# mulns/AccFlow

Hardware: AMD Instinct MI355X
Metric: frame-pairs/s (estimator pair-evals/s), AccFlow(RAFT) 7-frame 480x1024 backward accumulation (higher is better)
Workload: dtype f32 (direct-kernel operands split into 2 fp16 terms - activations kept pre-split in HBM as fp16 hi+lo, 4 B per element; other kernels 3 bf16 terms; f32 accumulate); 1 GPU; AccFlow(RAFT) 7-frame 480x1024, 12 GRU iters, 1 sequence(s)/GPU/step (BASELINE.json configs[2]; configs[3] when n_gpus=8); parallelism=1 rank, no process group: no collective runs, weights=deterministic random init (no checkpoints offline)

## Files before the change

accflow_amd/_lib.py:

```python
import ctypes
import os
import threading

_HERE = os.path.dirname(os.path.abspath(__file__))
LIB_PATH = os.environ.get("ACCFLOW_HIP_LIB") or os.path.join(_HERE, "lib", "libaccflow_hip.so")

ABI_VERSION = 20
c_f = ctypes.c_void_p
c_ll = ctypes.c_longlong
c_i = ctypes.c_int


class ConvSrc(ctypes.Structure):
    _fields_ = [
        ("ptr", c_f), ("bs", c_ll),
        ("C", c_i), ("Hs", c_i), ("Ws", c_i),
        ("step", c_i), ("oy", c_i), ("ox", c_i),
        ("KH", c_i), ("KW", c_i), ("padH", c_i), ("padW", c_i),
        ("reserved", c_i),
    ]


MAX_SRC = 4


class ConvDesc(ctypes.Structure):
    _fields_ = [
        ("in0", c_f), ("in1", c_f),
        ("in0_bs", c_ll), ("in1_bs", c_ll),
        ("C0", c_i), ("C1", c_i),
        ("B", c_i), ("H", c_i), ("W", c_i),
        ("OH", c_i), ("OW", c_i),
        ("KH", c_i), ("KW", c_i), ("stride", c_i), ("padH", c_i), ("padW", c_i),
        ("Cout", c_i),
        ("wpack", c_f), ("ktab", c_f),
        ("Kpad", c_i), ("CoutPad", c_i),
        ("bias", c_f),
        ("out", c_f), ("out_bs", c_ll),
        ("act", c_i), ("epi", c_i),
        ("e0", c_f), ("e0_bs", c_ll),
        ("e1", c_f), ("e1_bs", c_ll),
        ("out2", c_f), ("out2_bs", c_ll),
        ("offset", c_f), ("offset_bs", c_ll),
        ("dmask", c_f), ("dmask_bs", c_ll),
        ("wsplit", c_f), ("mode", c_i),
        ("wpatch", c_f),
        ("wsplit_bs", c_ll),
        ("kws", c_f), ("kws_elems", c_ll),
        ("wpatch16", c_f), ("guard", c_f),
        ("wscale16", c_f), ("wsplit16", c_f), 
        ("stats", c_f), ("stat_slots", c_i), ("pre", c_f), ("pre_bs", c_ll), ("in_norm", c_f), ("acc_scale", ctypes.c_float),
        ("in_fmt", c_i), ("out16", c_f), ("out16_bs", c_ll),
        ("cb", c_i), ("out_cbs", c_ll), ("e0_cbs", c_ll), ("out16_cbs", c_ll),
        ("nsrc", c_i), ("src", ConvSrc * MAX_SRC),
        ("e0_fmt", c_i),
        ("tg_w16", c_f), ("tg_scale", c_f), ("tg_out", c_f), ("tg_out_bs", c_ll), ("tg_out_ps", c_ll),
        ("tg_rows", c_i), ("tg_coutpad", c_i),
        ("split_c0", c_i), ("p32", c_i),
    ]


SIGNATURES = {
    "accflow_abi_version": [],
    "accflow_conv_desc_bytes": [],
    "accflow_conv_src_bytes": [],
    "accflow_s16_item_words": [c_i, c_i, c_i],
    "accflow_to_s16_f32": [c_f, c_ll, c_f, c_ll, c_f, c_i, c_i, c_i, c_f],
    "accflow_conv_kpad": [c_i, c_i, c_i],
    "accflow_conv_coutpad": [c_i],
    "accflow_conv_pack_f32": [c_f, c_f, c_i, c_i, c_i, c_i, c_i, c_i, c_f, c_f, c_f],
    "accflow_conv_pack_bf16s": [c_f, c_f, c_i, c_i, c_i, c_i, c_f, c_f],
    "accflow_conv_patch_elems": [c_i, c_i, c_i, c_i],
    "accflow_conv_pack_patch": [c_f, c_f, c_i, c_i, c_i, c_i, c_f, c_f],
    "accflow_conv_pack_patch16": [c_f, c_f, c_i, c_i, c_i, c_i, c_f, c_f, c_f],
    "accflow_conv_pack_split16": [c_f, c_f, c_i, c_i, c_i, c_i, c_f, c_f, c_f],
    "accflow_conv_multi_pack_elems": [c_i, c_i, ctypes.POINTER(c_i), ctypes.POINTER(c_i), ctypes.POINTER(c_i)],
    "accflow_conv_pack_multi16": [ctypes.POINTER(c_f), c_f, c_i, c_i, ctypes.POINTER(c_i), ctypes.POINTER(c_i), ctypes.POINTER(c_i),
                                  c_f, c_f, c_f],
    "accflow_conv2d_f32": [ctypes.POINTER(ConvDesc), c_f],
    "accflow_conv_stat_slots": [ctypes.POINTER(ConvDesc)],
    "accflow_conv_in_norm_supported": [ctypes.POINTER(ConvDesc)],
    "accflow_conv_plan_query": [ctypes.POINTER(ConvDesc), ctypes.POINTER(c_i), c_i],
    "accflow_conv_gru16_supported": [],
    "accflow_instance_stats_finalize_f32": [c_f, c_i, c_f, c_i, c_i, ctypes.c_float, c_f],
    "accflow_instance_norm_apply_f32": [c_f, c_f, c_i, c_f, c_f, c_f, c_i, c_i, c_i, ctypes.c_float, c_i, c_f],
    "accflow_instance_norm_apply_s16_f32": [c_f, c_f, c_i, c_f, c_f, c_f, c_f, c_ll, c_f, c_i, c_i, c_i, ctypes.c_float, c_i, c_f],
    "accflow_instance_norm_apply_s16res_f32": [c_f, c_f, c_i, c_f, c_f, c_ll, c_f, c_f, c_ll, c_f, c_i, c_i, c_i, ctypes.c_float, c_f],
    "accflow_instance_stats_finalize_sub_f32": [c_f, c_i, c_i, c_i, c_f, c_i, c_i, ctypes.c_float, c_f],
    "accflow_instance_norm_apply_s16proj_f32": [c_f, c_f, c_i, c_f, c_ll, c_f, c_i, c_i, c_i, c_f, c_f, c_ll, c_f, c_i, c_i, c_i,
                                                ctypes.c_float, c_f],
    "accflow_get_occ_s16": [c_f, c_ll, c_f, c_ll, c_f, c_ll, c_f, c_ll, c_f, c_i, c_i, c_i, c_i, c_i, c_f],
    "accflow_blend_s16": [c_f, c_f, c_f, c_f, c_ll, c_f, c_i, c_i, c_i, c_f],
    "accflow_deform_columns_s16": [c_f, c_ll, c_f, c_ll, c_f, c_ll, c_i, c_f, c_ll, c_f, c_i, c_i, c_i, c_i, c_i, c_i, c_i, c_i, c_f],
    "accflow_corr_volume_f32": [c_f, c_f, c_f, c_f, c_f, c_f, c_i, c_i, c_i, c_i, c_f],
    "accflow_corr_volume_ws_bytes": [c_i, c_i, c_i],
    "accflow_corr_volume_split_f32": [c_f, c_f, c_f, c_f, c_f, c_f, c_f, c_i, c_i, c_i, c_i, c_i, c_f],
    "accflow_corr_lookup_f32": [c_f, c_f, c_f, c_f, c_f, c_f, c_ll, c_i, c_i, c_i, c_f],
    "accflow_corr_disp_supported": [c_i, c_i],
    "accflow_corr_disp_level_elems": [c_i, c_i, c_i],
    "accflow_corr_volume_disp_f32": [c_f, c_f, c_f, c_f, c_f, c_f, c_f, c_i, c_f, c_i, c_i, c_i, c_i, c_f],
    "accflow_corr_pack_bytes": [c_i, c_i, c_i],
    "accflow_corr_pack_f32": [c_f, c_f, c_i, c_f, c_i, c_i, c_i, c_i, c_f],
    "accflow_corr_volume_disp_packed_f32": [c_f, c_i, ctypes.POINTER(c_i), ctypes.POINTER(c_i), c_f, c_f, c_f, c_f, c_i, c_f, c_i, c_i, c_i,
                                            c_i, c_f],
    "accflow_corr_disp_pool_f32": [c_f, c_f, c_f, c_f, c_i, c_i, c_i, c_f],
    "accflow_corr_lookup_disp_f32": [c_f, c_f, c_f, c_f, c_f, c_f, c_ll, c_i, c_i, c_i, c_f],
    "accflow_corr_lookup_disp_s16": [c_f, c_f, c_f, c_f, c_f, c_f, c_ll, c_f, c_i, c_i, c_i, c_f],
    "accflow_corr_alt_pyramid_elems": [c_i, c_i, c_i],
    "accflow_corr_alt_pyramid_f32": [c_f, c_f, c_i, c_i, c_i, c_i, c_f],
    "accflow_corr_lookup_alt_f32": [c_f, c_i, c_f, c_f, c_f, c_ll, c_i, c_i, c_i, c_i, c_f],
    "accflow_corr_lookup_alt_s16": [c_f, c_i, c_f, c_f, c_f, c_ll, c_f, c_i, c_i, c_i, c_i, c_f],
    "accflow_corr_lookup_convc1_kpad": [],
    "accflow_corr_lookup_convc1_s16": [c_f, c_f, c_f, c_f, c_f, c_f, c_f, c_f, c_f, c_ll, c_f, c_ll, c_i, c_f, c_i, c_i, c_i, c_i, c_f],
    "accflow_flow_from_coords_s16": [c_f, c_f, c_ll, c_f, c_ll, c_f, c_ll, c_f, c_ll, c_i, c_f, c_i, c_i, c_i, c_i, c_f],
    "accflow_convex_upsample_f32": [c_f, c_ll, c_f, c_ll, c_f, c_i, c_i, c_i, c_f],
    "accflow_backwarp_f32": [c_f, c_ll, c_f, c_ll, c_f, c_ll, c_i, c_i, c_i, c_i, c_f],
    "accflow_compose_flow_f32": [c_f, c_ll, c_f, c_ll, c_f, c_ll, c_i, c_i, c_i, c_f],
    "accflow_get_occ_f32": [c_f, c_ll, c_f, c_ll, c_f, c_ll, c_f, c_ll, c_i, c_i, c_i, c_i, c_i, c_f],
    "accflow_downflow8_f32": [c_f, c_f, c_i, c_i, c_i, c_i, c_f],
    "accflow_forward_interpolate_f32": [c_f, c_f, c_i, c_i, c_i, c_f],
    "accflow_instance_norm_f32": [c_f, c_f, c_f, c_i, c_i, c_i, ctypes.c_float, c_i, c_f],
    "accflow_split_tanh_relu_f32": [c_f, c_f, c_ll, c_f, c_ll, c_i, c_i, c_i, c_i, c_f],
    "accflow_split_tanh_relu_idx_f32": [c_f, c_i, ctypes.POINTER(c_i), c_f, c_ll, c_f, c_ll, c_i, c_i, c_i, c_i, c_f],
    "accflow_coords_grid_f32": [c_f, c_f, c_i, c_i, c_i, c_f],
    "accflow_flow_from_coords_f32": [c_f, c_f, c_ll, c_f, c_ll, c_f, c_i, c_i, c_i, c_i, c_f],
    "accflow_deform_columns_f32": [c_f, c_ll, c_f, c_ll, c_f, c_ll, c_f, c_i, c_i, c_i, c_i, c_i, c_i, c_i, c_i, c_f],
    "accflow_conv_pack_all_f32": [c_f, c_f, c_i, c_i, c_i, c_i, c_i, c_i, c_i, c_f, c_f, c_f, c_f, c_f, c_f, c_f, c_f],
    "accflow_tap_sum_f32": [c_f, c_f, c_f, c_ll, c_f, c_ll, c_i, c_i, c_i, c_i, c_i, c_i, c_i, c_i, c_i, c_i, c_f],
    "accflow_tap_sum_parts_f32": [c_f, c_i, c_ll, c_ll, c_f, c_f, c_ll, c_f, c_ll, c_i, c_i, c_i, c_i, c_i, c_i, c_i, c_i, c_i, c_i, c_f],
    "accflow_blend_f32": [c_f, c_f, c_f, c_f, c_i, c_i, c_i, c_f],
    "accflow_activation_f32": [c_f, c_ll, c_i, c_i, c_i, c_i, c_f],
    "accflow_copy_f32": [c_f, c_ll, c_f, c_ll, c_i, c_i, c_i, c_f],
    "accflow_gma_attention_f32": [c_f, c_f, c_i, c_i, c_i, ctypes.c_float, c_f],
    "accflow_gma_attention_ws_bytes": [c_i, c_i, c_i],
    "accflow_gma_attention_t_f32": [c_f, c_f, c_f, c_i, c_i, c_i, c_i, c_i, ctypes.c_float, c_f],
    "accflow_gma_aggregate_ws_bytes": [c_i, c_i, c_i],
    "accflow_gma_attention_s16_ws_bytes": [c_i, c_i, c_i],
    "accflow_gma_attention_s16": [c_f, c_f, c_f, c_f, c_i, c_i, c_i, c_i, ctypes.c_float, c_f],
    "accflow_gma_aggregate_s16_ws_bytes": [c_i, c_i, c_i],
    "accflow_gma_aggregate_s16": [c_f, c_f, c_f, c_ll, c_f, c_f, c_ll, c_f, c_ll, c_f, c_f, c_i, c_i, c_i, c_i, c_f],
    "accflow_gma_attention_alt_ws_bytes": [c_i, c_i, c_i],
    "accflow_gma_attention_alt": [c_f, c_f, c_f, c_f, c_f, c_f, c_i, c_i, c_i, c_i, ctypes.c_float, c_f],
    "accflow_gma_aggregate_alt_ws_bytes": [c_i, c_i, c_i],
    "accflow_gma_aggregate_alt": [c_f, c_f, c_f, c_f, c_f, c_ll, c_f, c_f, c_ll, c_f, c_ll, c_f, c_f, c_i, c_i, c_i, c_i, c_f],
    "accflow_gma_aggregate_t_f32": [c_f, c_f, c_f, c_f, c_f, c_ll, c_f, c_i, c_f, c_i, c_i, c_i, c_i, c_f],
    "accflow_gma_aggregate_f32": [c_f, c_f, c_f, c_f, c_f, c_ll, c_i, c_i, c_i, c_f],
    "accflow_act_backward_f32": [c_f, c_ll, c_f, c_ll, c_f, c_ll, c_i, c_ll, c_i, c_f],
    "accflow_add_f32": [c_f, c_ll, c_f, c_ll, c_i, c_ll, c_f],
    "accflow_l1_grad_f32": [c_f, c_f, c_f, c_ll, ctypes.c_float, c_f],
    "accflow_dilate_f32": [c_f, c_ll, c_f, c_i, c_i, c_i, c_i, c_i, c_i, c_i, c_f],
    "accflow_blend_backward_f32": [c_f, c_f, c_f, c_f, c_f, c_f, c_f, c_i, c_i, c_i, c_f],
    "accflow_convex_upsample_backward_f32": [c_f, c_f, c_f, c_f, c_f, c_i, c_i, c_i, c_f],
    "accflow_conv_wgrad_f32": [c_f, c_ll, c_f, c_ll, c_f, c_f, c_i, c_i, c_i, c_i, c_i, c_i, c_i, c_i, c_i, c_i, c_f],
    "accflow_deform_conv_backward_f32": [c_f, c_ll, c_f, c_ll, c_f, c_ll, c_f, c_f, c_ll, c_f, c_f, c_i, c_i, c_i, c_i, c_i, c_i, c_i,
                                         c_i, c_f],
}

_lock = threading.Lock()
_lib = None


def _promote_hip_runtime():
    import torch
    cand = os.path.join(os.path.dirname(torch.__file__), "lib", "libamdhip64.so")
    if os.path.exists(cand):
        ctypes.CDLL(cand, mode=ctypes.RTLD_GLOBAL)
    else:
        ctypes.CDLL("libamdhip64.so", mode=ctypes.RTLD_GLOBAL)


def load():
    global _lib
    if _lib is not None:
        return _lib
    with _lock:
        if _lib is not None:
            return _lib
        if not os.path.exists(LIB_PATH):
            raise RuntimeError(
                "accflow_amd: %s not found - run `python -m accflow_amd.build` (hipcc, gfx950). "
                "There is no non-HIP fallback." % LIB_PATH)
        _promote_hip_runtime()
        lib = ctypes.CDLL(LIB_PATH)
        for name, argtypes in SIGNATURES.items():
            fn = getattr(lib, name)
            fn.argtypes = argtypes
            fn.restype = ctypes.c_longlong if name in ("accflow_conv_patch_elems", "accflow_conv_multi_pack_elems", "accflow_corr_pack_bytes", "accflow_corr_volume_ws_bytes",
                                                    "accflow_gma_aggregate_ws_bytes", "accflow_gma_attention_ws_bytes", "accflow_gma_aggregate_s16_ws_bytes", "accflow_gma_attention_s16_ws_bytes", "accflow_gma_attention_alt_ws_bytes", "accflow_gma_aggregate_alt_ws_bytes", "accflow_corr_disp_level_elems", "accflow_corr_alt_pyramid_elems",
                                                    "accflow_s16_item_words") else ctypes.c_int
        if lib.accflow_abi_version() != ABI_VERSION:
            raise RuntimeError("accflow_amd: ABI version mismatch")
        if (lib.accflow_conv_desc_bytes() != ctypes.sizeof(ConvDesc) or lib.accflow_conv_src_bytes() != ctypes.sizeof(ConvSrc)):
            raise RuntimeError("accflow_amd: accflow_conv_desc is %d / %d bytes in the library, %d / %d in _lib.py's mirror" % (
                lib.accflow_conv_desc_bytes(), lib.accflow_conv_src_bytes(), ctypes.sizeof(ConvDesc), ctypes.sizeof(ConvSrc)))
        _lib = lib
    return _lib
```

accflow_amd/csrc/misc.hip:

```cpp
#include "common.h"

namespace {

__device__ __forceinline__ double block_sum(double v, double* red) {
#pragma unroll
  for (int o = 32; o > 0; o >>= 1) v += __shfl_xor(v, o, 64);
  const int lane = threadIdx.x & 63, wave = threadIdx.x >> 6, nw = blockDim.x >> 6;
  __syncthreads();
  if (lane == 0) red[wave] = v;
  __syncthreads();
  double t = 0.0;
  for (int i = 0; i < nw; ++i) t += red[i];
  return t;
}

__global__ __launch_bounds__(512) void instance_norm_kernel(const float* x, const float* res,
                                                            float* out, int HW, float eps, int mode) {
  __shared__ double red[8];
  const long long base = (long long)blockIdx.x * HW;
  const float* p = x + base;
  const bool vec = (HW & 3) == 0;
  double s = 0.0;
  if (vec) {
    const float4* p4 = reinterpret_cast<const float4*>(p);
// ... 112 lines not shown
      for (int k = 0; k < 4; ++k) o[k] = fmaxf(o[k], 0.0f);
    if (mode == 2) {
      const float4 r = *reinterpret_cast<const float4*>(res + i4);
      o[0] = fmaxf(r.x + o[0], 0.0f); o[1] = fmaxf(r.y + o[1], 0.0f); o[2] = fmaxf(r.z + o[2], 0.0f); o[3] = fmaxf(r.w + o[3], 0.0f);
    }
    *reinterpret_cast<float4*>(out + i4) = make_float4(o[0], o[1], o[2], o[3]);
  } else {
    for (long long i = i4; i < i4 + 4 && i < total; ++i) {
      const long long plane = i / HW;
      float v = (x[i] - meanrstd[2 * plane]) * meanrstd[2 * plane + 1];
      if (mode >= 1) v = fmaxf(v, 0.0f);
      if (mode == 2) v = fmaxf(res[i] + v, 0.0f);
      out[i] = v;
    }
  }
}

__global__ void split_tanh_relu_kernel(const float* __restrict__ cnet, float* __restrict__ net, long long net_bs,
                                       float* __restrict__ inp, long long inp_bs, int B, int hd, int cd, int HW) {
  const long long per = (long long)(hd + cd) * HW;
  const long long g = (long long)blockIdx.x * blockDim.x + threadIdx.x;
  if (g >= B * per) return;
  const int b = (int)(g / per);
  const long long r = g - b * per;
  const int c = (int)(r / HW), pix = (int)(r - (long long)c * HW);
  const float v = cnet[g];
  if (c < hd) net[b * net_bs + (long long)c * HW + pix] = tanhf(v);
  else inp[b * inp_bs + (long long)(c - hd) * HW + pix] = fmaxf(v, 0.0f);
}

struct split_idx { int v[64]; };
__global__ void split_tanh_relu_idx_kernel(const float* __restrict__ cnet, split_idx idx, float* __restrict__ net,
                                           long long net_bs, float* __restrict__ inp, long long inp_bs, int B, int hd, int cd,
                                           int HW) {
  const long long per = (long long)(hd + cd) * HW;
  const long long g = (long long)blockIdx.x * blockDim.x + threadIdx.x;
  if (g >= B * per) return;
  const int b = (int)(g / per);
  const long long r = g - b * per;
  const int c = (int)(r / HW), pix = (int)(r - (long long)c * HW);
  const float v = cnet[(long long)idx.v[b] * per + r];
  if (c < hd) net[b * net_bs + (long long)c * HW + pix] = tanhf(v);
  else inp[b * inp_bs + (long long)(c - hd) * HW + pix] = fmaxf(v, 0.0f);
}

__global__ void coords_grid_kernel(float* __restrict__ coords, const float* __restrict__ flow_init, int B, int H8,
                                   int W8) {
  const int P = H8 * W8;
  const long long g = (long long)blockIdx.x * blockDim.x + threadIdx.x;
  if (g >= (long long)B * 2 * P) return;
  const int pix = (int)(g % P), ch = (int)((g / P) & 1);
  const int y = pix / W8, x = pix - y * W8;
  float v = ch == 0 ? (float)x : (float)y;
  if (flow_init) v += flow_init[g];
  coords[g] = v;
}

__global__ void flow_from_coords_kernel(const float* __restrict__ coords1, float* __restrict__ dst0,
                                        long long dst0_bs, float* __restrict__ dst1, long long dst1_bs,
                                        float* __restrict__ stack, int B, int H8, int W8, int is_flow) {
  const int P = H8 * W8;
  const long long g = (long long)blockIdx.x * blockDim.x + threadIdx.x;
  if (g >= (long long)B * 2 * P) return;
  const int b = (int)(g / (2 * P));
  const int r = (int)(g - (long long)b * 2 * P);
  const int ch = r / P, pix = r - ch * P;
  const int y = pix / W8, x = pix - y * W8;
  const float v = is_flow ? coords1[g] : coords1[g] - (ch == 0 ? (float)x : (float)y);
  if (dst0) dst0[b * dst0_bs + r] = v;
  if (dst1) dst1[b * dst1_bs + r] = v;
  if (stack) {
    float* s = stack + (long long)b * 16 * P + pix;
#pragma unroll
    for (int ky = 0; ky < 7; ++ky) {
      const int ys = y + ky - 3;
      const bool ok = (unsigned)ys < (unsigned)H8;
      const float c = ok ? coords1[g + (long long)(ky - 3) * W8] : 0.0f;
      const float u = (ok && !is_flow) ? c - (ch == 0 ? (float)x : (float)ys) : c;
      s[(long long)(ch * 7 + ky) * P] = u;
    }
    s[(long long)(14 + ch) * P] = 0.0f;
  }
}

__global__ __launch_bounds__(256) void flow_from_coords_s16_kernel(const float* __restrict__ coords1, float* __restrict__ dst0,
                                                                   long long dst0_bs, float* __restrict__ dst1, long long dst1_bs,
                                                                   mu32x4* __restrict__ stack, long long stack_bs,
                                                                   unsigned* __restrict__ motion, long long motion_bs, int motion_ch,
                                                                   int* guard, int B, int H8, int W8, int is_flow) {
  const int P = H8 * W8;
  const long long g = (long long)blockIdx.x * 256 + threadIdx.x;
  if (g >= (long long)B * P) return;
  const int b = (int)(g / P), pix = (int)(g - (long long)b * P);
  const int y = pix / W8, x = pix - y * W8;
  const float* c = coords1 + (long long)b * 2 * P + pix;
  float st[16];
#pragma unroll
  for (int ch = 0; ch < 2; ++ch)
#pragma unroll
    for (int ky = 0; ky < 7; ++ky) {
      const int ys = y + ky - 3;
      const bool ok = (unsigned)ys < (unsigned)H8;
      const float cv = ok ? c[(long long)ch * P + (long long)(ky - 3) * W8] : 0.0f;
      st[ch * 7 + ky] = (ok && !is_flow) ? cv - (ch == 0 ? (float)x : (float)ys) : cv;
    }
  st[14] = 0.0f; st[15] = 0.0f;
  const float fx = st[3], fy = st[10];
  if (dst0) { dst0[b * dst0_bs + pix] = fx; dst0[b * dst0_bs + P + pix] = fy; }
  if (dst1) { dst1[b * dst1_bs + pix] = fx; dst1[b * dst1_bs + P + pix] = fy; }
  bool bad = false;
  if (stack) {
    mu32x4* sb = stack + (b * stack_bs) / 4;
#pragma unroll
    for (int o = 0; o < 2; ++o) {
      float v[8];
#pragma unroll
      for (int j = 0; j < 8; ++j) v[j] = st[o * 8 + j];
      mu32x4 hi, lo;
      s16_split8(v, hi, lo, bad);
      sb[((long long)(o * 2 + 0)) * P + pix] = hi;
      sb[((long long)(o * 2 + 1)) * P + pix] = lo;
    }
  }
  if (motion) {
    float v[8] = {fx, fy, 0.0f, 0.0f, 0.0f, 0.0f, 0.0f, 0.0f};
    mu32x4 hi, lo;
    s16_split8(v, hi, lo, bad);
    const int oct = motion_ch >> 3, word = (motion_ch & 7) >> 1;
    unsigned* mb = motion + b * motion_bs;
    mb[(((long long)(oct * 2 + 0)) * P + pix) * 4 + word] = hi[0];
    mb[(((long long)(oct * 2 + 1)) * P + pix) * 4 + word] = lo[0];
  }
  if (bad && guard) atomicOr(guard, 1);
}

__global__ __launch_bounds__(256) void to_s16_kernel(const float* __restrict__ src, long long src_bs, mu32x4* __restrict__ dst,
                                                     long long dst_bs, int* guard, int B, int C, int HW) {
  const int O = (C + 7) >> 3;
  const long long g = (long long)blockIdx.x * 256 + threadIdx.x;
  if (g >= (long long)B * O * HW) return;
  const int pix = (int)(g % HW), o = (int)((g / HW) % O), b = (int)(g / ((long long)HW * O));
  float v[8];
#pragma unroll
  for (int j = 0; j < 8; ++j) v[j] = (o * 8 + j < C) ? src[b * src_bs + (long long)(o * 8 + j) * HW + pix] : 0.0f;
  mu32x4 hi, lo;
  bool bad = false;
  s16_split8(v, hi, lo, bad);
  mu32x4* d = dst + (b * dst_bs) / 4;
  d[(long long)(o * 2 + 0) * HW + pix] = hi;
  d[(long long)(o * 2 + 1) * HW + pix] = lo;
  if (bad && guard) atomicOr(guard, 1);
}

__global__ __launch_bounds__(256) void instance_norm_apply_s16_kernel(const float* __restrict__ x, const float* __restrict__ meanrstd,
                                                                      const float* __restrict__ res, float* __restrict__ out,
                                                                      mu32x4* __restrict__ dst, long long dst_bs, int* guard,
                                                                      int B, int C, int HW, int mode) {
  const int O = (C + 7) >> 3;
  const long long g = (long long)blockIdx.x * 256 + threadIdx.x;
  if (g >= (long long)B * O * HW) return;
  const int pix = (int)(g % HW), o = (int)((g / HW) % O), b = (int)(g / ((long long)HW * O));
  float v[8];
#pragma unroll
  for (int j = 0; j < 8; ++j) {
    const int c = o * 8 + j;
    v[j] = 0.0f;
    if (c < C) {
      const long long plane = (long long)b * C + c, e = plane * HW + pix;
      float t = (x[e] - meanrstd[2 * plane]) * meanrstd[2 * plane + 1];
      if (mode >= 1) t = fmaxf(t, 0.0f);
      if (mode == 2) t = fmaxf(res[e] + t, 0.0f);
      if (out) out[e] = t;
      v[j] = t;
    }
  }
  mu32x4 hi, lo;
  bool bad = false;
  s16_split8(v, hi, lo, bad);
  mu32x4* d = dst + (b * dst_bs) / 4;
  d[(long long)(o * 2 + 0) * HW + pix] = hi;
  d[(long long)(o * 2 + 1) * HW + pix] = lo;
  if (bad && guard) atomicOr(guard, 1);
}

__global__ __launch_bounds__(256) void instance_norm_apply_s16res_kernel(const float* __restrict__ x, const float* __restrict__ meanrstd,
                                                                         const mu32x4* __restrict__ res, long long res_bs,
                                                                         float* __restrict__ out, mu32x4* __restrict__ dst,
                                                                         long long dst_bs, int* guard, int B, int C, int HW) {
  const int O = (C + 7) >> 3;
  const long long g = (long long)blockIdx.x * 256 + threadIdx.x;
  if (g >= (long long)B * O * HW) return;
  const int pix = (int)(g % HW), o = (int)((g / HW) % O), b = (int)(g / ((long long)HW * O));
  const mu32x4* rp = res + (b * res_bs) / 4;
  const mu32x4 rh = rp[(long long)(o * 2 + 0) * HW + pix], rl = rp[(long long)(o * 2 + 1) * HW + pix];
  const unsigned hw[4] = {rh.x, rh.y, rh.z, rh.w}, lw[4] = {rl.x, rl.y, rl.z, rl.w};
  float v[8];
#pragma unroll
  for (int j = 0; j < 8; ++j) {
    const int c = o * 8 + j;
    v[j] = 0.0f;
    if (c < C) {
      const long long plane = (long long)b * C + c, e = plane * HW + pix;
      const _Float16 hh = __builtin_bit_cast(_Float16, (unsigned short)((hw[j >> 1] >> (16 * (j & 1))) & 0xFFFFu));
      const _Float16 ll = __builtin_bit_cast(_Float16, (unsigned short)((lw[j >> 1] >> (16 * (j & 1))) & 0xFFFFu));
      const float r = ((float)hh + (float)ll) * (1.0f / (float)(1 << ACCFLOW_F16_ASHIFT));
      float t = fmaxf((x[e] - meanrstd[2 * plane]) * meanrstd[2 * plane + 1], 0.0f);
      t = fmaxf(r + t, 0.0f);
      if (out) out[e] = t;
      v[j] = t;
    }
  }
  mu32x4 hi, lo;
  bool bad = false;
  s16_split8(v, hi, lo, bad);
  mu32x4* d = dst + (b * dst_bs) / 4;
  d[(long long)(o * 2 + 0) * HW + pix] = hi;
  d[(long long)(o * 2 + 1) * HW + pix] = lo;
  if (bad && guard) atomicOr(guard, 1);
}

__global__ __launch_bounds__(256) void instance_norm_apply_s16proj_kernel(const float* __restrict__ x, const float* __restrict__ mr2,
                                                                          const float* __restrict__ res, long long res_bs,
                                                                          const float* __restrict__ mr3, mu32x4* __restrict__ dst,
                                                                          long long dst_bs, int* guard, int B, int C, int HW) {
  const int O = (C + 7) >> 3;
  const long long g = (long long)blockIdx.x * 256 + threadIdx.x;
  if (g >= (long long)B * O * HW) return;
  const int pix = (int)(g % HW), o = (int)((g / HW) % O), b = (int)(g / ((long long)HW * O));
  float v[8];
#pragma unroll
  for (int j = 0; j < 8; ++j) {
    const int c = o * 8 + j;
    v[j] = 0.0f;
    if (c < C) {
      const long long plane = (long long)b * C + c;
      const float t = fmaxf((x[plane * HW + pix] - mr2[2 * plane]) * mr2[2 * plane + 1], 0.0f);
      const float r = (res[b * res_bs + (long long)c * HW + pix] - mr3[2 * plane]) * mr3[2 * plane + 1];
      v[j] = fmaxf(r + t, 0.0f);
    }
  }
  mu32x4 hi, lo;
  bool bad = false;
  s16_split8(v, hi, lo, bad);
  mu32x4* d = dst + (b * dst_bs) / 4;
  d[(long long)(o * 2 + 0) * HW + pix] = hi;
  d[(long long)(o * 2 + 1) * HW + pix] = lo;
  if (bad && guard) atomicOr(guard, 1);
}

__global__ void blend_kernel(const float* __restrict__ f1, const float* __restrict__ f2, const float* __restrict__ m,
                             float* __restrict__ out, int B, int C, int HW) {
  const long long g = (long long)blockIdx.x * blockDim.x + threadIdx.x;
  if (g >= (long long)B * C * HW) return;
  const int b = (int)(g / ((long long)C * HW));
  const int pix = (int)(g % HW);
  const float mm = m[(long long)b * HW + pix];
  out[g] = f1[g] * mm + (1.0f - mm) * f2[g];
}

__global__ __launch_bounds__(256) void blend_s16_kernel(const float* __restrict__ f1, const float* __restrict__ f2,
                                                        const float* __restrict__ m, mu32x4* __restrict__ dst, long long dst_bs,
                                                        int* guard, int B, int C, int HW) {
  const int O = (C + 7) >> 3;
  const long long g = (long long)blockIdx.x * 256 + threadIdx.x;
  if (g >= (long long)B * O * HW) return;
  const int pix = (int)(g % HW), o = (int)((g / HW) % O), b = (int)(g / ((long long)HW * O));
  const float mm = m[(long long)b * HW + pix];
  float v[8];
#pragma unroll
  for (int j = 0; j < 8; ++j) {
    const int c = o * 8 + j;
    const long long e = ((long long)b * C + c) * HW + pix;
    v[j] = c < C ? f1[e] * mm + (1.0f - mm) * f2[e] : 0.0f;
  }
  mu32x4 hi, lo;
  bool bad = false;
  s16_split8(v, hi, lo, bad);
  mu32x4* d = dst + (b * dst_bs) / 4;
  d[(long long)(o * 2 + 0) * HW + pix] = hi;
  d[(long long)(o * 2 + 1) * HW + pix] = lo;
  if (bad && guard) atomicOr(guard, 1);
}

__global__ void copy_kernel(const float* __restrict__ src, long long src_bs, float* __restrict__ dst, long long dst_bs,
                            int B, long long per) {
  const long long g = (long long)blockIdx.x * blockDim.x + threadIdx.x;
  if (g >= B * per) return;
  const int b = (int)(g / per);
  const long long r = g - b * per;
  dst[b * dst_bs + r] = src[b * src_bs + r];
}

__global__ void act_kernel(float* __restrict__ x, long long x_bs, int B, long long per, int act) {
  const long long g = (long long)blockIdx.x * blockDim.x + threadIdx.x;
  if (g >= B * per) return;
  const int b = (int)(g / per);
  const long long r = g - b * per;
  x[b * x_bs + r] = apply_act(x[b * x_bs + r], act);
}

}

extern "C" int accflow_activation_f32(float* x, long long x_bs, int B, int C, int HW, int act, void* stream) {
  if (!x || B <= 0 || C <= 0 || HW <= 0) return 1;
  const long long per = (long long)C * HW;
  hipLaunchKernelGGL(act_kernel, dim3(cdiv(B * per, 256)), dim3(256), 0, as_stream(stream), x, x_bs, B, per, act);
  ACCFLOW_RETURN_LAUNCH_STATUS();
}

extern "C" int accflow_instance_norm_f32(const float* x, const float* res, float* out, int B, int C, int HW, float eps,
                                         int mode, void* stream) {
  if (!x || !out || B <= 0 || C <= 0 || HW <= 0 || mode < 0 || mode > 2 || (mode == 2 && !res)) return 1;
  hipLaunchKernelGGL(instance_norm_kernel, dim3((unsigned)((long long)B * C)), dim3(512), 0, as_stream(stream), x, res,
                     out, HW, eps, mode);
  ACCFLOW_RETURN_LAUNCH_STATUS();
}

extern "C" int accflow_instance_stats_finalize_f32(const float* stats, int slots, float* meanrstd, int B, int C, float eps,
                                                   void* stream) {
  if (!stats || !meanrstd || slots <= 0 || B <= 0 || C <= 0) return 1;
  launch_finalize(stats, slots, C, 0, meanrstd, B, C, eps, as_stream(stream));
  ACCFLOW_RETURN_LAUNCH_STATUS();
}

extern "C" int accflow_instance_stats_finalize_sub_f32(const float* stats, int slots, int Ctot, int c0, float* meanrstd, int B,
                                                       int C, float eps, void* stream) {
  if (!stats || !meanrstd || slots <= 0 || B <= 0 || C <= 0 || c0 < 0 || c0 + C > Ctot) return 1;
  launch_finalize(stats, slots, Ctot, c0, meanrstd, B, C, eps, as_stream(stream));
  ACCFLOW_RETURN_LAUNCH_STATUS();
}

extern "C" int accflow_instance_norm_apply_s16proj_f32(const float* x, const float* stats, int slots, const float* res,
                                                       long long res_bs, const float* res_stats, int res_slots, int res_ctot,
                                                       int res_c0, float* meanrstd, void* out16, long long out16_bs, int* guard,
                                                       int B, int C, int HW, float eps, void* stream) {
  if (!x || !stats || !res || !res_stats || !meanrstd || !out16 || slots <= 0 || res_slots <= 0 || B <= 0 || C <= 0 || HW <= 0 ||
      res_c0 < 0 || res_c0 + C > res_ctot)
    return 1;
  hipStream_t st = as_stream(stream);
  float* mr3 = meanrstd + 2LL * B * C;
  launch_finalize(stats, slots, C, 0, meanrstd, B, C, eps, st, res_stats, res_slots, res_ctot, res_c0, mr3);
  const long long n = (long long)B * ((C + 7) / 8) * HW;
  hipLaunchKernelGGL(instance_norm_apply_s16proj_kernel, dim3(cdiv(n, 256)), dim3(256), 0, st, x, meanrstd, res, res_bs, mr3,
                     reinterpret_cast<mu32x4*>(out16), out16_bs, guard, B, C, HW);
  ACCFLOW_RETURN_LAUNCH_STATUS();
}

extern "C" int accflow_instance_norm_apply_f32(const float* x, const float* stats, int slots, float* meanrstd,
                                               const float* res, float* out, int B, int C, int HW, float eps, int mode,
                                               void* stream) {
  if (!x || !stats || !meanrstd || !out || slots <= 0 || B <= 0 || C <= 0 || HW <= 0 || mode < 0 || mode > 2 ||
      (mode == 2 && !res))
    return 1;
  const long long total = (long long)B * C * HW;
  launch_finalize(stats, slots, C, 0, meanrstd, B, C, eps, as_stream(stream));
  hipLaunchKernelGGL(instance_norm_apply_kernel, dim3(cdiv(cdiv(total, 4), 256)), dim3(256), 0, as_stream(stream), x,
                     meanrstd, res, out, HW, total, mode);
  ACCFLOW_RETURN_LAUNCH_STATUS();
}

extern "C" int accflow_instance_norm_apply_s16_f32(const float* x, const float* stats, int slots, float* meanrstd,
                                                   const float* res, float* out, void* out16, long long out16_bs, int* guard,
                                                   int B, int C, int HW, float eps, int mode, void* stream) {
  if (!x || !stats || !meanrstd || !out16 || slots <= 0 || B <= 0 || C <= 0 || HW <= 0 || mode < 0 || mode > 2 ||
      (mode == 2 && !res))
    return 1;
  launch_finalize(stats, slots, C, 0, meanrstd, B, C, eps, as_stream(stream));
  const long long n = (long long)B * ((C + 7) / 8) * HW;
  hipLaunchKernelGGL(instance_norm_apply_s16_kernel, dim3(cdiv(n, 256)), dim3(256), 0, as_stream(stream), x, meanrstd, res,
                     out, reinterpret_cast<mu32x4*>(out16), out16_bs, guard, B, C, HW, mode);
  ACCFLOW_RETURN_LAUNCH_STATUS();
}

extern "C" int accflow_instance_norm_apply_s16res_f32(const float* x, const float* stats, int slots, float* meanrstd,
                                                      const void* res16, long long res16_bs, float* out, void* out16,
                                                      long long out16_bs, int* guard, int B, int C, int HW, float eps,
                                                      void* stream) {
  if (!x || !stats || !meanrstd || !res16 || !out16 || slots <= 0 || B <= 0 || C <= 0 || HW <= 0) return 1;
  launch_finalize(stats, slots, C, 0, meanrstd, B, C, eps, as_stream(stream));
  const long long n = (long long)B * ((C + 7) / 8) * HW;
  hipLaunchKernelGGL(instance_norm_apply_s16res_kernel, dim3(cdiv(n, 256)), dim3(256), 0, as_stream(stream), x, meanrstd,
                     reinterpret_cast<const mu32x4*>(res16), res16_bs, out, reinterpret_cast<mu32x4*>(out16), out16_bs, guard,
                     B, C, HW);
  ACCFLOW_RETURN_LAUNCH_STATUS();
}

extern "C" int accflow_split_tanh_relu_f32(const float* cnet, float* net, long long net_bs, float* inp,
                                           long long inp_bs, int B, int hd, int cd, int HW, void* stream) {
  if (!cnet || !net || !inp || B <= 0 || hd <= 0 || cd <= 0 || HW <= 0) return 1;
  const long long n = (long long)B * (hd + cd) * HW;
  hipLaunchKernelGGL(split_tanh_relu_kernel, dim3(cdiv(n, 256)), dim3(256), 0, as_stream(stream), cnet, net, net_bs,
                     inp, inp_bs, B, hd, cd, HW);
  ACCFLOW_RETURN_LAUNCH_STATUS();
}

extern "C" int accflow_split_tanh_relu_idx_f32(const float* cnet, int n_items, const int* idx, float* net, long long net_bs,
                                               float* inp, long long inp_bs, int B, int hd, int cd, int HW, void* stream) {
  if (!cnet || !idx || !net || !inp || n_items <= 0 || B <= 0 || hd <= 0 || cd <= 0 || HW <= 0) return 1;
  for (int b = 0; b < B; ++b)
    if (idx[b] < 0 || idx[b] >= n_items) return 1;
  for (int b0 = 0; b0 < B; b0 += 64) {
    const int nb = B - b0 < 64 ? B - b0 : 64;
    split_idx a;
    for (int k = 0; k < 64; ++k) a.v[k] = k < nb ? idx[b0 + k] : 0;
    const long long n = (long long)nb * (hd + cd) * HW;
    hipLaunchKernelGGL(split_tanh_relu_idx_kernel, dim3(cdiv(n, 256)), dim3(256), 0, as_stream(stream), cnet, a,
                       net + b0 * net_bs, net_bs, inp + b0 * inp_bs, inp_bs, nb, hd, cd, HW);
  }
  ACCFLOW_RETURN_LAUNCH_STATUS();
}

extern "C" int accflow_coords_grid_f32(float* coords, const float* flow_init, int B, int H8, int W8, void* stream) {
  if (!coords || B <= 0 || H8 <= 0 || W8 <= 0) return 1;
  const long long n = (long long)B * 2 * H8 * W8;
  hipLaunchKernelGGL(coords_grid_kernel, dim3(cdiv(n, 256)), dim3(256), 0, as_stream(stream), coords, flow_init, B, H8,
                     W8);
  ACCFLOW_RETURN_LAUNCH_STATUS();
}

extern "C" int accflow_flow_from_coords_f32(const float* coords1, float* dst0, long long dst0_bs, float* dst1,
                                            long long dst1_bs, float* stack16, int is_flow, int B, int H8, int W8,
                                            void* stream) {
  if (!coords1 || (!dst0 && !dst1 && !stack16) || B <= 0 || H8 <= 0 || W8 <= 0) return 1;
  const long long n = (long long)B * 2 * H8 * W8;
  hipLaunchKernelGGL(flow_from_coords_kernel, dim3(cdiv(n, 256)), dim3(256), 0, as_stream(stream), coords1, dst0,
                     dst0_bs, dst1, dst1_bs, stack16, B, H8, W8, is_flow);
  ACCFLOW_RETURN_LAUNCH_STATUS();
}

extern "C" int accflow_flow_from_coords_s16(const float* coords1, float* dst0, long long dst0_bs, float* dst1,
                                            long long dst1_bs, void* stack16, long long stack16_bs, void* motion16,
                                            long long motion16_bs, int motion_ch, int* guard, int is_flow, int B, int H8,
                                            int W8, void* stream) {
  if (!coords1 || (!dst0 && !dst1 && !stack16 && !motion16) || B <= 0 || H8 <= 0 || W8 <= 0 || motion_ch < 0 || (motion_ch & 1))
    return 1;
  const long long n = (long long)B * H8 * W8;
  hipLaunchKernelGGL(flow_from_coords_s16_kernel, dim3(cdiv(n, 256)), dim3(256), 0, as_stream(stream), coords1, dst0, dst0_bs,
                     dst1, dst1_bs, reinterpret_cast<mu32x4*>(stack16), stack16_bs, reinterpret_cast<unsigned*>(motion16),
                     motion16_bs, motion_ch, guard, B, H8, W8, is_flow);
  ACCFLOW_RETURN_LAUNCH_STATUS();
}

extern "C" int accflow_to_s16_f32(const float* src, long long src_bs, void* dst16, long long dst16_bs, int* guard, int B,
                                  int C, int HW, void* stream) {
  if (!src || !dst16 || B <= 0 || C <= 0 || HW <= 0) return 1;
  const long long n = (long long)B * ((C + 7) / 8) * HW;
  hipLaunchKernelGGL(to_s16_kernel, dim3(cdiv(n, 256)), dim3(256), 0, as_stream(stream), src, src_bs,
                     reinterpret_cast<mu32x4*>(dst16), dst16_bs, guard, B, C, HW);
  ACCFLOW_RETURN_LAUNCH_STATUS();
}

extern "C" int accflow_blend_f32(const float* f1, const float* f2, const float* m, float* out, int B, int C, int HW,
                                 void* stream) {
  if (!f1 || !f2 || !m || !out || B <= 0 || C <= 0 || HW <= 0) return 1;
  const long long n = (long long)B * C * HW;
  hipLaunchKernelGGL(blend_kernel, dim3(cdiv(n, 256)), dim3(256), 0, as_stream(stream), f1, f2, m, out, B, C, HW);
  ACCFLOW_RETURN_LAUNCH_STATUS();
}

extern "C" int accflow_blend_s16(const float* f1, const float* f2, const float* m, void* out16, long long out16_bs, int* guard,
                                 int B, int C, int HW, void* stream) {
  if (!f1 || !f2 || !m || !out16 || B <= 0 || C <= 0 || HW <= 0) return 1;
  const long long n = (long long)B * ((C + 7) / 8) * HW;
  hipLaunchKernelGGL(blend_s16_kernel, dim3(cdiv(n, 256)), dim3(256), 0, as_stream(stream), f1, f2, m,
                     reinterpret_cast<mu32x4*>(out16), out16_bs, guard, B, C, HW);
  ACCFLOW_RETURN_LAUNCH_STATUS();
}

extern "C" int accflow_copy_f32(const float* src, long long src_bs, float* dst, long long dst_bs, int B, int C, int HW,
                                void* stream) {
  if (!src || !dst || B <= 0 || C <= 0 || HW <= 0) return 1;
  const long long per = (long long)C * HW;
  hipLaunchKernelGGL(copy_kernel, dim3(cdiv(B * per, 256)), dim3(256), 0, as_stream(stream), src, src_bs, dst, dst_bs,
                     B, per);
  ACCFLOW_RETURN_LAUNCH_STATUS();
}

__global__ __launch_bounds__(256) void tap_sum_kernel(const float* __restrict__ z, const float* __restrict__ bias,
                                                      const float* __restrict__ e0, long long e0_bs, float* __restrict__ out,
                                                      long long out_bs, int B, int Cout, int H, int W, int KH, int KW,
                                                      int padH, int padW, int act, int epi, int nparts, long long part_stride,
                                                      long long z_bs) {
  const long long n = (long long)B * Cout * H * W;
  const long long i = (long long)blockIdx.x * 256 + threadIdx.x;
  if (i >= n) return;
  const int x = (int)(i % W), y = (int)((i / W) % H);
  const int co = (int)((i / ((long long)W * H)) % Cout), b = (int)(i / ((long long)W * H * Cout));
  const int HW = H * W;
  const float* zb = z + (long long)b * z_bs;
  float v = 0.0f;
  for (int ky = 0; ky < KH; ++ky) {
    const int yy = y + ky - padH;
    if ((unsigned)yy >= (unsigned)H) continue;
    for (int kx = 0; kx < KW; ++kx) {
      const int xx = x + kx - padW;
      if ((unsigned)xx >= (unsigned)W) continue;
      const float* zp = zb + (long long)((ky * KW + kx) * Cout + co) * HW + yy * W + xx;
      float t = zp[0];
      for (int p = 1; p < nparts; ++p) t += zp[p * part_stride];
      v += t;
    }
  }
  if (bias) v += bias[co];
  v = apply_act(v, act);
  const long long o = (long long)co * HW + y * W + x;
  if (epi == ACCFLOW_EPI_ACCUM) v += e0[b * e0_bs + o];
  else if (epi == ACCFLOW_EPI_RES_RELU) v = fmaxf(e0[b * e0_bs + o] + v, 0.0f);
  out[b * out_bs + o] = v;
}

extern "C" int accflow_tap_sum_f32(const float* z, const float* bias, const float* e0, long long e0_bs, float* out,
                                   long long out_bs, int B, int Cout, int H, int W, int KH, int KW, int padH, int padW,
                                   int act, int epi, void* stream) {
  if (!z || !out || B <= 0 || Cout <= 0 || H <= 0 || W <= 0 || KH <= 0 || KW <= 0) return 1;
  if (epi != ACCFLOW_EPI_STORE && epi != ACCFLOW_EPI_ACCUM && epi != ACCFLOW_EPI_RES_RELU) return 1;
  if (epi != ACCFLOW_EPI_STORE && !e0) return 1;
  const long long n = (long long)B * Cout * H * W;
  hipLaunchKernelGGL(tap_sum_kernel, dim3(cdiv(n, 256)), dim3(256), 0, as_stream(stream), z, bias, e0, e0_bs, out, out_bs, B,
                     Cout, H, W, KH, KW, padH, padW, act, epi, 1, 0LL, (long long)KH * KW * Cout * H * W);
  ACCFLOW_RETURN_LAUNCH_STATUS();
}

extern "C" int accflow_tap_sum_parts_f32(const float* z, int nparts, long long part_stride, long long z_bs, const float* bias,
                                         const float* e0, long long e0_bs, float* out, long long out_bs, int B, int Cout, int H,
                                         int W, int KH, int KW, int padH, int padW, int act, int epi, void* stream) {
  if (!z || !out || B <= 0 || Cout <= 0 || H <= 0 || W <= 0 || KH <= 0 || KW <= 0 || nparts < 1 || nparts > 8) return 1;
  if (z_bs < (long long)KH * KW * Cout * H * W || (nparts > 1 && part_stride <= 0)) return 1;
  if (epi != ACCFLOW_EPI_STORE && epi != ACCFLOW_EPI_ACCUM && epi != ACCFLOW_EPI_RES_RELU) return 1;
  if (epi != ACCFLOW_EPI_STORE && !e0) return 1;
  const long long n = (long long)B * Cout * H * W;
  hipLaunchKernelGGL(tap_sum_kernel, dim3(cdiv(n, 256)), dim3(256), 0, as_stream(stream), z, bias, e0, e0_bs, out, out_bs, B,
                     Cout, H, W, KH, KW, padH, padW, act, epi, nparts, part_stride, z_bs);
  ACCFLOW_RETURN_LAUNCH_STATUS();
}

extern "C" int accflow_abi_version(void) { return ACCFLOW_ABI_VERSION; }
extern "C" int accflow_conv_desc_bytes(void) { return (int)sizeof(accflow_conv_desc); }
extern "C" int accflow_conv_src_bytes(void) { return (int)sizeof(accflow_conv_src); }
```

accflow_amd/csrc/sampling.hip:

```cpp
#include "common.h"

namespace {

__global__ __launch_bounds__(256) void convex_upsample_kernel(const float* __restrict__ flow, long long flow_bs,
                                                              const float* __restrict__ mask, long long mask_bs,
                                                              float* __restrict__ out, int B, int H8, int W8) {
  const int P = H8 * W8;
  const long long gp = (long long)blockIdx.x * blockDim.x + threadIdx.x;
  if (gp >= (long long)B * P) return;
  const int b = (int)(gp / P), pix = (int)(gp - (long long)b * P);
  const int h = pix / W8, w = pix - h * W8;
  const float* fl = flow + b * flow_bs;
  float f0[9], f1[9];
#pragma unroll
  for (int k = 0; k < 9; ++k) {
    const int yy = h + k / 3 - 1, xx = w + k % 3 - 1;
    const bool ok = (unsigned)yy < (unsigned)H8 && (unsigned)xx < (unsigned)W8;
    f0[k] = ok ? 8.0f * fl[yy * W8 + xx] : 0.0f;
    f1[k] = ok ? 8.0f * fl[P + yy * W8 + xx] : 0.0f;
  }
  const float* mk = mask + b * mask_bs + pix;
  const int W = 8 * W8;
  float* o0 = out + ((long long)(b * 2 + 0) * (8 * H8) + 8 * h) * W + 8 * w;
  float* o1 = out + ((long long)(b * 2 + 1) * (8 * H8) + 8 * h) * W + 8 * w;
#pragma unroll 1
  for (int a = 0; a < 8; ++a) {
    float r0[8], r1[8];
#pragma unroll
    for (int bb = 0; bb < 8; ++bb) {
      float m[9];
      float mx = -INFINITY;
#pragma unroll
      for (int k = 0; k < 9; ++k) {
        m[k] = mk[(long long)(k * 64 + a * 8 + bb) * P];
        mx = fmaxf(mx, m[k]);
      }
      float s = 0.0f;
#pragma unroll
      for (int k = 0; k < 9; ++k) {
        m[k] = expf(m[k] - mx);
        s += m[k];
      }
      float u0 = 0.0f, u1 = 0.0f;
#pragma unroll
      for (int k = 0; k < 9; ++k) {
        const float wk = m[k] / s;
        u0 += wk * f0[k];
        u1 += wk * f1[k];
      }
      r0[bb] = u0;
      r1[bb] = u1;
    }
    float4* q0 = reinterpret_cast<float4*>(o0 + (long long)a * W);
    float4* q1 = reinterpret_cast<float4*>(o1 + (long long)a * W);
    q0[0] = make_float4(r0[0], r0[1], r0[2], r0[3]);
    q0[1] = make_float4(r0[4], r0[5], r0[6], r0[7]);
    q1[0] = make_float4(r1[0], r1[1], r1[2], r1[3]);
    q1[1] = make_float4(r1[4], r1[5], r1[6], r1[7]);
  }
}

struct WarpTaps {
  int o00, o01, o10, o11;
  float w00, w01, w10, w11;
};

__device__ __forceinline__ WarpTaps make_taps(float sx, float sy, int H, int W) {
  sx = fminf(fmaxf(sx, -1.0e6f), 1.0e6f);
  sy = fminf(fmaxf(sy, -1.0e6f), 1.0e6f);
  const float fx0 = floorf(sx), fy0 = floorf(sy);
  const int x0 = (int)fx0, y0 = (int)fy0;
  const float ax = sx - fx0, ay = sy - fy0;
  const bool xin0 = (unsigned)x0 < (unsigned)W, xin1 = (unsigned)(x0 + 1) < (unsigned)W;
  const bool yin0 = (unsigned)y0 < (unsigned)H, yin1 = (unsigned)(y0 + 1) < (unsigned)H;
  WarpTaps t;
  t.o00 = (xin0 && yin0) ? y0 * W + x0 : 0;
  t.o01 = (xin1 && yin0) ? y0 * W + x0 + 1 : 0;
  t.o10 = (xin0 && yin1) ? (y0 + 1) * W + x0 : 0;
  t.o11 = (xin1 && yin1) ? (y0 + 1) * W + x0 + 1 : 0;
  t.w00 = (xin0 && yin0) ? (1.0f - ax) * (1.0f - ay) : 0.0f;
  t.w01 = (xin1 && yin0) ? ax * (1.0f - ay) : 0.0f;
  t.w10 = (xin0 && yin1) ? (1.0f - ax) * ay : 0.0f;
  t.w11 = (xin1 && yin1) ? ax * ay : 0.0f;
  return t;
}
__device__ __forceinline__ float tap_sample(const float* __restrict__ plane, const WarpTaps& t) {
  return plane[t.o00] * t.w00 + plane[t.o01] * t.w01 + plane[t.o10] * t.w10 + plane[t.o11] * t.w11;
}

constexpr int WARP_CCHUNK = 16;

template <bool ADD>
__global__ __launch_bounds__(256) void backwarp_kernel(const float* __restrict__ img, long long img_bs,
                                                       const float* __restrict__ flow, long long flow_bs,
                                                       float* __restrict__ out, long long out_bs, int B, int C, int H,
                                                       int W) {
  const int HW = H * W;
  const long long gp = (long long)blockIdx.x * blockDim.x + threadIdx.x;
  if (gp >= (long long)B * HW) return;
  const int b = (int)(gp / HW), pix = (int)(gp - (long long)b * HW);
  const int y = pix / W, x = pix - y * W;
  const float u = flow[b * flow_bs + pix], v0 = flow[b * flow_bs + HW + pix];
  const WarpTaps t = make_taps((float)x + u, (float)y + v0, H, W);
  const int c0 = blockIdx.y * WARP_CCHUNK, c1 = min(C, c0 + WARP_CCHUNK);
  for (int c = c0; c < c1; ++c) {
    float v = tap_sample(img + b * img_bs + (long long)c * HW, t);
    if constexpr (ADD) v += c == 0 ? u : v0;
    out[b * out_bs + (long long)c * HW + pix] = v;
  }
}

template <bool BINARY>
__global__ __launch_bounds__(256) void get_occ_kernel(const float* __restrict__ flow, long long flow_bs,
                                                      const float* __restrict__ i1, long long i1_bs,
                                                      const float* __restrict__ i2, long long i2_bs,
                                                      float* __restrict__ out, long long out_bs, int B, int C, int H,
                                                      int W) {
  const int HW = H * W;
  const long long gp = (long long)blockIdx.x * blockDim.x + threadIdx.x;
  if (gp >= (long long)B * HW) return;
  const int b = (int)(gp / HW), pix = (int)(gp - (long long)b * HW);
  const int y = pix / W, x = pix - y * W;
  const float u = flow[b * flow_bs + pix], v = flow[b * flow_bs + HW + pix];
  const WarpTaps t = make_taps((float)x + u, (float)y + v, H, W);
  if constexpr (BINARY) {
    const int cper = (C + 3) / 4;
    float q[4];
#pragma unroll
    for (int k = 0; k < 4; ++k) {
      float s = 0.0f;
      for (int c = k * cper; c < min(C, (k + 1) * cper); ++c) {
        const float wv = tap_sample(i2 + b * i2_bs + (long long)c * HW, t);
        s += fabsf(i1[b * i1_bs + (long long)c * HW + pix] - wv);
      }
      q[k] = s;
    }
    const float tot = (q[0] + q[1]) + (q[2] + q[3]);
    out[b * out_bs + pix] = (tot / (float)C <= 1.0f) ? 1.0f : 0.0f;
  } else {
    const int c0 = blockIdx.y * WARP_CCHUNK, c1 = min(C, c0 + WARP_CCHUNK);
    for (int c = c0; c < c1; ++c) {
      const float wv = tap_sample(i2 + b * i2_bs + (long long)c * HW, t);
      out[b * out_bs + (long long)c * HW + pix] = fabsf(i1[b * i1_bs + (long long)c * HW + pix] - wv);
    }
  }
}

template <bool BINARY>
__global__ __launch_bounds__(256) void get_occ_s16_kernel(const float* __restrict__ flow, long long flow_bs,
                                                          const float* __restrict__ i1, long long i1_bs,
                                                          const float* __restrict__ i2, long long i2_bs,
                                                          mu32x4* __restrict__ dst, long long dst_bs, int* guard, int B, int C,
                                                          int H, int W) {
  const int HW = H * W;
  const long long gp = (long long)blockIdx.x * blockDim.x + threadIdx.x;
  if (gp >= (long long)B * HW) return;
  const int b = (int)(gp / HW), pix = (int)(gp - (long long)b * HW);
  const int y = pix / W, x = pix - y * W;
  const float u = flow[b * flow_bs + pix], v = flow[b * flow_bs + HW + pix];
  const WarpTaps t = make_taps((float)x + u, (float)y + v, H, W);
  float val[8] = {0.0f, 0.0f, 0.0f, 0.0f, 0.0f, 0.0f, 0.0f, 0.0f};
  const int o = BINARY ? 0 : blockIdx.y;
  if constexpr (BINARY) {
    const int cper = (C + 3) / 4;
    float q[4];
#pragma unroll
    for (int k = 0; k < 4; ++k) {
      float s = 0.0f;
      for (int c = k * cper; c < min(C, (k + 1) * cper); ++c) {
        const float wv = tap_sample(i2 + b * i2_bs + (long long)c * HW, t);
        s += fabsf(i1[b * i1_bs + (long long)c * HW + pix] - wv);
      }
      q[k] = s;
    }
    const float tot = (q[0] + q[1]) + (q[2] + q[3]);
    val[0] = (tot / (float)C <= 1.0f) ? 1.0f : 0.0f;
  } else {
#pragma unroll
    for (int j = 0; j < 8; ++j) {
      const int c = o * 8 + j;
      if (c < C) val[j] = fabsf(i1[b * i1_bs + (long long)c * HW + pix] - tap_sample(i2 + b * i2_bs + (long long)c * HW, t));
    }
  }
  mu32x4 hi, lo;
  bool bad = false;
  s16_split8(val, hi, lo, bad);
  mu32x4* d = dst + (b * dst_bs) / 4;
  d[(long long)(o * 2 + 0) * HW + pix] = hi;
  d[(long long)(o * 2 + 1) * HW + pix] = lo;
  if (bad && guard) atomicOr(guard, 1);
}

__global__ __launch_bounds__(256) void downflow8_kernel(const float* __restrict__ flow, float* __restrict__ out,
                                                        int BC, int H, int W) {
  const int H8 = H / 8, W8 = W / 8, P = H8 * W8;
  const long long g = (long long)blockIdx.x * blockDim.x + threadIdx.x;
  if (g >= (long long)BC * P) return;
  const int bc = (int)(g / P), pix = (int)(g - (long long)bc * P);
  const int y = pix / W8, x = pix - y * W8;
  const float sy_scale = H8 > 1 ? (float)(H - 1) / (float)(H8 - 1) : 0.0f;
  const float sx_scale = W8 > 1 ? (float)(W - 1) / (float)(W8 - 1) : 0.0f;
  const float sy = sy_scale * (float)y, sx = sx_scale * (float)x;
  const int y0 = (int)sy, x0 = (int)sx;
  const int yp = y0 < H - 1 ? 1 : 0, xp = x0 < W - 1 ? 1 : 0;
  const float ly = sy - (float)y0, lx = sx - (float)x0;
  const float hy = 1.0f - ly, hx = 1.0f - lx;
  const float* p = flow + (long long)bc * H * W + (long long)y0 * W + x0;
  const float v = hy * (hx * p[0] + lx * p[xp]) + ly * (hx * p[(long long)yp * W] + lx * p[(long long)yp * W + xp]);
  out[g] = v / 8.0f;
}

}

extern "C" int accflow_convex_upsample_f32(const float* flow, long long flow_bs, const float* mask, long long mask_bs,
                                           float* out, int B, int H8, int W8, void* stream) {
  if (!flow || !mask || !out || B <= 0 || H8 <= 0 || W8 <= 0) return 1;
  const long long np = (long long)B * H8 * W8;
  hipLaunchKernelGGL(convex_upsample_kernel, dim3(cdiv(np, 256)), dim3(256), 0, as_stream(stream), flow, flow_bs,
                     mask, mask_bs, out, B, H8, W8);
  ACCFLOW_RETURN_LAUNCH_STATUS();
}

template <bool S16OUT>
__global__ __launch_bounds__(256) void get_occ_binary4_kernel(const float* __restrict__ flow, long long flow_bs,
                                                              const float* __restrict__ i1, long long i1_bs,
                                                              const float* __restrict__ i2, long long i2_bs,
                                                              float* __restrict__ out, long long out_bs, int B, int C, int H,
                                                              int W) {
  __shared__ float part[4][64];
  const int HW = H * W;
  const int lane = threadIdx.x & 63, wave = threadIdx.x >> 6;
  const long long gp = (long long)blockIdx.x * 64 + lane;
  const bool live = gp < (long long)B * HW;
  const int b = live ? (int)(gp / HW) : 0, pix = live ? (int)(gp - (long long)b * HW) : 0;
  const int y = pix / W, x = pix - y * W;
  const float u = flow[b * flow_bs + pix], v = flow[b * flow_bs + HW + pix];
  const WarpTaps t = make_taps((float)x + u, (float)y + v, H, W);
  const int cper = (C + 3) / 4, cbeg = wave * cper, cend = min(C, cbeg + cper);
  float s = 0.0f;
  for (int c = cbeg; c < cend; ++c) {
    const float wv = tap_sample(i2 + b * i2_bs + (long long)c * HW, t);
    s += fabsf(i1[b * i1_bs + (long long)c * HW + pix] - wv);
  }
  part[wave][lane] = s;
  __syncthreads();
  if (wave == 0 && live) {
    const float tot = (part[0][lane] + part[1][lane]) + (part[2][lane] + part[3][lane]);
    const float bit = (tot / (float)C <= 1.0f) ? 1.0f : 0.0f;
    if constexpr (S16OUT) {
      const float val[8] = {bit, 0.0f, 0.0f, 0.0f, 0.0f, 0.0f, 0.0f, 0.0f};
      mu32x4 hi, lo;
      bool bad = false;
      s16_split8(val, hi, lo, bad);
      mu32x4* d = reinterpret_cast<mu32x4*>(out) + (b * out_bs) / 4;
      d[pix] = hi;
      d[(long long)HW + pix] = lo;
    } else {
      out[b * out_bs + pix] = bit;
    }
  }
}

extern "C" int accflow_backwarp_f32(const float* img, long long img_bs, const float* flow, long long flow_bs,
                                    float* out, long long out_bs, int B, int C, int H, int W, void* stream) {
  if (!img || !flow || !out || B <= 0 || C <= 0 || H <= 0 || W <= 0) return 1;
  const long long np = (long long)B * H * W;
  hipLaunchKernelGGL(backwarp_kernel<false>, dim3(cdiv(np, 256), cdiv(C, WARP_CCHUNK)), dim3(256), 0, as_stream(stream),
                     img, img_bs, flow, flow_bs, out, out_bs, B, C, H, W);
  ACCFLOW_RETURN_LAUNCH_STATUS();
}

extern "C" int accflow_compose_flow_f32(const float* step, long long step_bs, const float* acc, long long acc_bs,
                                        float* out, long long out_bs, int B, int H, int W, void* stream) {
  if (!step || !acc || !out || B <= 0 || H <= 0 || W <= 0) return 1;
  const long long np = (long long)B * H * W;
  hipLaunchKernelGGL(backwarp_kernel<true>, dim3(cdiv(np, 256), 1), dim3(256), 0, as_stream(stream), acc, acc_bs, step,
                     step_bs, out, out_bs, B, 2, H, W);
  ACCFLOW_RETURN_LAUNCH_STATUS();
}

extern "C" int accflow_get_occ_f32(const float* flow, long long flow_bs, const float* i1, long long i1_bs,
                                   const float* i2, long long i2_bs, float* out, long long out_bs, int B, int C, int H,
                                   int W, int binary, void* stream) {
  if (!flow || !i1 || !i2 || !out || B <= 0 || C <= 0 || H <= 0 || W <= 0) return 1;
  const long long np = (long long)B * H * W;
  if (binary && np < (1 << 17))
    hipLaunchKernelGGL((get_occ_binary4_kernel<false>), dim3(cdiv(np, 64)), dim3(256), 0, as_stream(stream), flow, flow_bs, i1,
                       i1_bs, i2, i2_bs, out, out_bs, B, C, H, W);
  else if (binary)
    hipLaunchKernelGGL((get_occ_kernel<true>), dim3(cdiv(np, 256)), dim3(256), 0, as_stream(stream), flow, flow_bs,
                       i1, i1_bs, i2, i2_bs, out, out_bs, B, C, H, W);
  else
    hipLaunchKernelGGL((get_occ_kernel<false>), dim3(cdiv(np, 256), cdiv(C, WARP_CCHUNK)), dim3(256), 0,
                       as_stream(stream), flow, flow_bs, i1, i1_bs, i2, i2_bs, out, out_bs, B, C, H, W);
  ACCFLOW_RETURN_LAUNCH_STATUS();
}

extern "C" int accflow_get_occ_s16(const float* flow, long long flow_bs, const float* i1, long long i1_bs, const float* i2,
                                   long long i2_bs, void* out16, long long out16_bs, int* guard, int B, int C, int H, int W,
                                   int binary, void* stream) {
  if (!flow || !i1 || !i2 || !out16 || B <= 0 || C <= 0 || H <= 0 || W <= 0) return 1;
  const long long np = (long long)B * H * W;
  mu32x4* d = reinterpret_cast<mu32x4*>(out16);
  if (binary && np < (1 << 17))
    hipLaunchKernelGGL((get_occ_binary4_kernel<true>), dim3(cdiv(np, 64)), dim3(256), 0, as_stream(stream), flow, flow_bs, i1,
                       i1_bs, i2, i2_bs, reinterpret_cast<float*>(out16), out16_bs, B, C, H, W);
  else if (binary)
    hipLaunchKernelGGL((get_occ_s16_kernel<true>), dim3(cdiv(np, 256)), dim3(256), 0, as_stream(stream), flow, flow_bs, i1, i1_bs,
                       i2, i2_bs, d, out16_bs, guard, B, C, H, W);
  else
    hipLaunchKernelGGL((get_occ_s16_kernel<false>), dim3(cdiv(np, 256), cdiv(C, 8)), dim3(256), 0, as_stream(stream), flow,
                       flow_bs, i1, i1_bs, i2, i2_bs, d, out16_bs, guard, B, C, H, W);
  ACCFLOW_RETURN_LAUNCH_STATUS();
}

extern "C" int accflow_downflow8_f32(const float* flow, float* out, int B, int C, int H, int W, void* stream) {
  if (!flow || !out || B <= 0 || C <= 0 || H < 8 || W < 8 || (H % 8) || (W % 8)) return 1;
  const long long n = (long long)B * C * (H / 8) * (W / 8);
  hipLaunchKernelGGL(downflow8_kernel, dim3(cdiv(n, 256)), dim3(256), 0, as_stream(stream), flow, out, B * C, H, W);
  ACCFLOW_RETURN_LAUNCH_STATUS();
}

namespace {
__global__ __launch_bounds__(256) void deform_columns_kernel(const float* __restrict__ x, long long x_bs,
                                                             const float* __restrict__ off, long long off_bs,
                                                             const float* __restrict__ msk, long long msk_bs,
                                                             float* __restrict__ cols, int B, int C, int H, int W, int KH,
                                                             int KW, int padH, int padW) {
  const int HW = H * W, T = KH * KW;
  const long long i = (long long)blockIdx.x * 256 + threadIdx.x;
  if (i >= (long long)B * T * HW) return;
  const int p = (int)(i % HW), tap = (int)((i / HW) % T), b = (int)(i / ((long long)HW * T));
  const int y = p / W, xx = p - y * W, ky = tap / KW, kx = tap - ky * KW;
  const float dy = off[b * off_bs + (long long)(2 * tap) * HW + p], dx = off[b * off_bs + (long long)(2 * tap + 1) * HW + p];
  const float m = msk[b * msk_bs + (long long)tap * HW + p];
  const float h = (float)(y - padH + ky) + dy, w = (float)(xx - padW + kx) + dx;
  const bool inside = h > -1.0f && h < (float)H && w > -1.0f && w < (float)W;
  const float fh = floorf(h), fw = floorf(w);
  const int hl = (int)fh, wl = (int)fw, hh = hl + 1, wh = wl + 1;
  const float lh = h - fh, lw = w - fw, uh = 1.0f - lh, uw = 1.0f - lw;
  const bool o1 = inside && hl >= 0 && wl >= 0, o2 = inside && hl >= 0 && wh <= W - 1;
  const bool o3 = inside && hh <= H - 1 && wl >= 0, o4 = inside && hh <= H - 1 && wh <= W - 1;
  const int i1 = o1 ? hl * W + wl : 0, i2 = o2 ? hl * W + wh : 0, i3 = o3 ? hh * W + wl : 0, i4 = o4 ? hh * W + wh : 0;
  const float* src = x + b * x_bs;
  float* dst = cols + ((long long)b * T * C + (long long)tap * C) * HW + p;
  const int cper = (C + gridDim.y - 1) / gridDim.y, cbeg = blockIdx.y * cper, cend = min(C, cbeg + cper);
  for (int c = cbeg; c < cend; ++c) {
    const float* plane = src + (long long)c * HW;
    const float v1 = o1 ? plane[i1] : 0.0f, v2 = o2 ? plane[i2] : 0.0f, v3 = o3 ? plane[i3] : 0.0f, v4 = o4 ? plane[i4] : 0.0f;
    dst[(long long)c * HW] = inside ? m * (uh * uw * v1 + uh * lw * v2 + lh * uw * v3 + lh * lw * v4) : 0.0f;
  }
}

template <bool LOGIT>
__global__ __launch_bounds__(256) void deform_columns_s16_kernel(const float* __restrict__ x, long long x_bs,
                                                                 const float* __restrict__ off, long long off_bs,
                                                                 const float* __restrict__ msk, long long msk_bs,
                                                                 mu32x4* __restrict__ cols, long long cols_bs, int* guard, int B,
                                                                 int C, int H, int W, int KH, int KW, int padH, int padW) {
  const int HW = H * W, T = KH * KW;
  const long long i = (long long)blockIdx.x * 256 + threadIdx.x;
  if (i >= (long long)B * T * HW) return;
  const int p = (int)(i % HW), tap = (int)((i / HW) % T), b = (int)(i / ((long long)HW * T));
  const int y = p / W, xx = p - y * W, ky = tap / KW, kx = tap - ky * KW;
  const float dy = off[b * off_bs + (long long)(2 * tap) * HW + p], dx = off[b * off_bs + (long long)(2 * tap + 1) * HW + p];
  float m = msk[b * msk_bs + (long long)tap * HW + p];
  if constexpr (LOGIT) m = sigmoidf_(m);
  const float h = (float)(y - padH + ky) + dy, w = (float)(xx - padW + kx) + dx;
  const bool inside = h > -1.0f && h < (float)H && w > -1.0f && w < (float)W;
  const float fh = floorf(h), fw = floorf(w);
  const int hl = (int)fh, wl = (int)fw, hh = hl + 1, wh = wl + 1;
  const float lh = h - fh, lw = w - fw, uh = 1.0f - lh, uw = 1.0f - lw;
  const bool o1 = inside && hl >= 0 && wl >= 0, o2 = inside && hl >= 0 && wh <= W - 1;
  const bool o3 = inside && hh <= H - 1 && wl >= 0, o4 = inside && hh <= H - 1 && wh <= W - 1;
  const int i1 = o1 ? hl * W + wl : 0, i2 = o2 ? hl * W + wh : 0, i3 = o3 ? hh * W + wl : 0, i4 = o4 ? hh * W + wh : 0;
  const float* src = x + b * x_bs;
  const int OC = C >> 3;
  const int oper = (OC + gridDim.y - 1) / gridDim.y, obeg = blockIdx.y * oper, oend = min(OC, obeg + oper);
  mu32x4* d = cols + (b * cols_bs) / 4;
  bool bad = false;
  for (int o = obeg; o < oend; ++o) {
    float v[8];
#pragma unroll
    for (int j = 0; j < 8; ++j) {
      const float* plane = src + (long long)(o * 8 + j) * HW;
      const float v1 = o1 ? plane[i1] : 0.0f, v2 = o2 ? plane[i2] : 0.0f, v3 = o3 ? plane[i3] : 0.0f, v4 = o4 ? plane[i4] : 0.0f;
      v[j] = inside ? m * (uh * uw * v1 + uh * lw * v2 + lh * uw * v3 + lh * lw * v4) : 0.0f;
    }
    mu32x4 hi, lo;
    s16_split8(v, hi, lo, bad);
    const long long oct = (long long)tap * OC + o;
    d[(oct * 2 + 0) * HW + p] = hi;
    d[(oct * 2 + 1) * HW + p] = lo;
  }
  if (bad && guard) atomicOr(guard, 1);
}
}

extern "C" int accflow_deform_columns_s16(const float* x, long long x_bs, const float* offset, long long offset_bs,
                                          const float* dmask, long long dmask_bs, int mask_is_logit, void* cols16,
                                          long long cols16_bs, int* guard, int B, int C, int H, int W, int KH, int KW, int padH,
                                          int padW, void* stream) {
  if (!x || !offset || !dmask || !cols16 || B <= 0 || C <= 0 || (C & 7) || H <= 0 || W <= 0 || KH <= 0 || KW <= 0) return 1;
  const long long n = (long long)B * KH * KW * H * W;
  const int chunks = n < (1 << 18) ? (C >= 64 ? 8 : 1) : (n < (1 << 20) ? 2 : 1);
  mu32x4* d = reinterpret_cast<mu32x4*>(cols16);
  if (mask_is_logit)
    hipLaunchKernelGGL((deform_columns_s16_kernel<true>), dim3(cdiv(n, 256), chunks), dim3(256), 0, as_stream(stream), x, x_bs,
                       offset, offset_bs, dmask, dmask_bs, d, cols16_bs, guard, B, C, H, W, KH, KW, padH, padW);
  else
    hipLaunchKernelGGL((deform_columns_s16_kernel<false>), dim3(cdiv(n, 256), chunks), dim3(256), 0, as_stream(stream), x, x_bs,
                       offset, offset_bs, dmask, dmask_bs, d, cols16_bs, guard, B, C, H, W, KH, KW, padH, padW);
  ACCFLOW_RETURN_LAUNCH_STATUS();
}

extern "C" int accflow_deform_columns_f32(const float* x, long long x_bs, const float* offset, long long offset_bs,
                                          const float* dmask, long long dmask_bs, float* cols, int B, int C, int H, int W,
                                          int KH, int KW, int padH, int padW, void* stream) {
  if (!x || !offset || !dmask || !cols || B <= 0 || C <= 0 || H <= 0 || W <= 0 || KH <= 0 || KW <= 0) return 1;
  const long long n = (long long)B * KH * KW * H * W;
  const int chunks = n < (1 << 18) ? (C >= 64 ? 8 : 1) : (n < (1 << 20) ? 2 : 1);
  hipLaunchKernelGGL(deform_columns_kernel, dim3(cdiv(n, 256), chunks), dim3(256), 0, as_stream(stream), x, x_bs, offset, offset_bs,
                     dmask, dmask_bs, cols, B, C, H, W, KH, KW, padH, padW);
  ACCFLOW_RETURN_LAUNCH_STATUS();
}
```

accflow_amd/networks/AccFlow_.py:

```python
import math

import torch
import torch.nn as nn

from .. import ops
from ._packs import PackCache, require_cuda, span
from .modules import ZeroConv2d
from .raft.extractor import BasicEncoder

import contextlib
import threading
import os

USE_S16_CHAIN = os.environ.get("ACCFLOW_S16_CHAIN", "1") == "1"
CONTEXT_SIDE_STREAM = os.environ.get("ACCFLOW_CONTEXT_STREAM", "1") == "1"
USE_CHAIN_HOIST = os.environ.get("ACCFLOW_CHAIN_HOIST", "auto")
_CHAIN_TLS = threading.local()


PIPELINE_CHAIN_KSPLIT = os.environ.get("ACCFLOW_PIPELINE_CHAIN_KSPLIT", "0") == "1"


@contextlib.contextmanager
def chain_in_pipeline():
    prev = (getattr(_CHAIN_TLS, "pipelined", False), getattr(_CHAIN_TLS, "no_ksplit", False))
    _CHAIN_TLS.pipelined, _CHAIN_TLS.no_ksplit = True, not PIPELINE_CHAIN_KSPLIT
    try:
        yield
    finally:
        _CHAIN_TLS.pipelined, _CHAIN_TLS.no_ksplit = prev


@contextlib.contextmanager
def pipeline_chain_arithmetic():
    prev = getattr(_CHAIN_TLS, "no_ksplit", False)
    _CHAIN_TLS.no_ksplit = not PIPELINE_CHAIN_KSPLIT
    try:
        yield
    finally:
        _CHAIN_TLS.no_ksplit = prev


def _hoist_now():
    if USE_CHAIN_HOIST == "auto":
        return not getattr(_CHAIN_TLS, "pipelined", False)
    return USE_CHAIN_HOIST == "1" or USE_CHAIN_HOIST is True
USE_CHAIN_DEFER_UP = os.environ.get("ACCFLOW_CHAIN_DEFER_UP", "1") == "1"
_CTX_STREAMS = {}


def _context_stream(device):
    key = str(device)
    if key not in _CTX_STREAMS:
        _CTX_STREAMS[key] = torch.cuda.Stream(device=device)
    return _CTX_STREAMS[key]


class FlowDecoder(nn.Module):
    def __init__(self, cin=128):
        super().__init__()
        self.flow = nn.Sequential(nn.Conv2d(cin, cin * 2, 3, 1, 1), nn.ReLU(True), nn.Conv2d(cin * 2, 2, 3, 1, 1))
        self.mask = nn.Sequential(nn.Conv2d(cin, cin * 2, 3, 1, 1), nn.ReLU(True), nn.Conv2d(cin * 2, 64 * 9, 1, 1, 0))
        self._packs = PackCache()

    def upsample_flow(self, flow, mask):
        require_cuda(flow, mask)
        return ops.convex_upsample(flow.float(), mask.float())

    @torch.no_grad()
    @ops.range_guarded
    def forward(self, x):
        require_cuda(x)
        pk = self._packs
        if ops.s16_active() and USE_S16_CHAIN:
            return self._forward16(ops.to_s16(x.float()))
        t = ops.conv2d(pk.conv("f0", self.flow[0]), x, act=ops.ACT_RELU)
        flow_small = ops.conv2d(pk.conv("f2", self.flow[2]), t)
        t = ops.conv2d(pk.conv("m0", self.mask[0]), x, act=ops.ACT_RELU, out=t)
        mask = ops.conv2d(pk.conv("m2", self.mask[2]), t)
        return flow_small, ops.convex_upsample(flow_small, mask)


    def _forward16(self, x16):
        pk = self._packs
        B, _, h, w = x16.shape
        c2 = self.flow[0].out_channels
        t16 = ops.S16.empty(B, 2 * c2, h, w, x16.device)
        ops.conv2d_multi(pk.multi_cat("fm0", [self.flow[0], self.mask[0]]), [x16], act=ops.ACT_RELU, out16=t16, fp32_out=False)
        flow_small = ops.conv2d(pk.conv("f2", self.flow[2]), t16.channels(0, c2))
        mask = ops.conv2d_multi(pk.multi("m2m", self.mask[2]), [t16.channels(c2, 2 * c2)])
        return flow_small, ops.convex_upsample(flow_small, mask)

    def flow16(self, x16, out=None):
        pk = self._packs
        B, _, h, w = x16.shape
        t16 = ops.S16.empty(B, self.flow[0].out_channels, h, w, x16.device)
        ops.conv2d_multi(pk.multi("f0m", self.flow[0]), [x16], act=ops.ACT_RELU, out16=t16, fp32_out=False)
        return ops.conv2d(pk.conv("f2", self.flow[2]), t16, out=out)

    def upsample16(self, x16, flow_small):
        pk = self._packs
        B, _, h, w = x16.shape
        t16 = ops.S16.empty(B, self.mask[0].out_channels, h, w, x16.device)
        ops.conv2d_multi(pk.multi("m0m", self.mask[0]), [x16], act=ops.ACT_RELU, out16=t16, fp32_out=False)
        mask = ops.conv2d_multi(pk.multi("m2m", self.mask[2]), [t16])
        return ops.convex_upsample(flow_small, mask)


class FlowEncoder(nn.Module):
    def __init__(self, c=128):
        super().__init__()
        self.conv1 = nn.Conv2d(2, c, 7, stride=1, padding=3)
        self.conv2 = nn.Conv2d(c, c * 2, 3, stride=1, padding=1)
        self.conv3 = nn.Conv2d(c * 2, c, 1, stride=1, padding=0)
        self.relu = nn.ReLU(True)
        self._packs = PackCache()

    @torch.no_grad()
    @ops.range_guarded
    def forward(self, x):
        is_list = isinstance(x, (tuple, list))
        if is_list:
            batch_dim = x[0].shape[0]
            x = torch.cat(x, dim=0)
        require_cuda(x)
        pk = self._packs
        if ops.s16_active() and USE_S16_CHAIN:
            x = self.encode16(x.float().contiguous())[0]
        else:
            x = ops.conv2d(pk.conv("1", self.conv1), x.float().contiguous(), act=ops.ACT_RELU)
            x = ops.conv2d(pk.conv("2", self.conv2), x, act=ops.ACT_RELU)
            x = ops.conv2d(pk.conv("3", self.conv3), x)
        if is_list:
            x = torch.split(x, batch_dim, dim=0)
        return x

    def encode16(self, flows):
        pk = self._packs
        B, _, h, w = flows.shape
        dev = flows.device
        c = self.conv1.out_channels
        stack16 = ops.S16.empty(B, 16, h, w, dev)
        ops.flow_from_coords_s16(flows, None, None, stack16, None, 0, is_flow=True)
        a16 = ops.S16.empty(B, c, h, w, dev)
        ops.conv2d(pk.conv("1s", self.conv1, rows_as_channels=True), stack16, act=ops.ACT_RELU, out16=a16, fp32_out=False)
        b16 = ops.S16.empty(B, 2 * c, h, w, dev)
        ops.conv2d_multi(pk.multi("2m", self.conv2), [a16], act=ops.ACT_RELU, out16=b16, fp32_out=False)
        o16 = ops.S16.empty(B, c, h, w, dev)
        out = ops.conv2d_multi(pk.multi("3m", self.conv3), [b16], out16=o16)
        return out, o16


class DeformConv2d(nn.Module):

    def __init__(self, in_channels, out_channels, kernel_size=3, stride=1, padding=1):
        super().__init__()
        if (kernel_size, stride, padding) != (3, 1, 1):
            raise NotImplementedError("AccPlus uses DeformConv2d(c, c, 3, 1, 1) (AccFlow_.py:83)")
        self.in_channels, self.out_channels = in_channels, out_channels
        self.kernel_size, self.stride, self.padding = (3, 3), (1, 1), (1, 1)
        self.weight = nn.Parameter(torch.empty(out_channels, in_channels, 3, 3))
        self.bias = nn.Parameter(torch.empty(out_channels))
        nn.init.kaiming_uniform_(self.weight, a=math.sqrt(5))
        bound = 1 / math.sqrt(in_channels * 9)
        nn.init.uniform_(self.bias, -bound, bound)


class AccPlus(nn.Module):
    def __init__(self, c=128):
        super().__init__()
        self.conv1 = nn.Sequential(nn.Conv2d(c * 2 + 1, c * 2, 3, 1, 1), nn.ReLU(True), nn.Conv2d(c * 2, c, 3, 1, 1))
        self.conv2 = nn.Sequential(nn.Conv2d(c * 2, c * 2, 3, 1, 1), nn.ReLU(True), nn.Conv2d(c * 2, c, 3, 1, 1),
                                   nn.ReLU(True), ZeroConv2d(c, 3 ** 3))
        self.dconv = DeformConv2d(c, c, 3, 1, 1)
        self.conv3 = nn.Sequential(nn.Conv2d(c * 2 + 1, c * 2, 3, 1, 1), nn.ReLU(True), nn.Conv2d(c * 2, c, 3, 1, 1))
        self.conv4 = nn.Sequential(nn.Conv2d(c * 4, c * 2, 3, 1, 1), nn.ReLU(True), nn.Conv2d(c * 2, c, 3, 1, 1),
                                   nn.ReLU(True), nn.Conv2d(c, c, 1, 1, 0))
        self.c = c
        self._packs = PackCache()

    @torch.no_grad()
    @ops.range_guarded
    def forward(self, df, f, o, c):
        require_cuda(df, f, o, c)
        if ops.s16_active() and USE_S16_CHAIN:
            return self.forward16(ops.to_s16(df.float()), f.float().contiguous(), ops.to_s16(f.float()), ops.to_s16(o.float()),
                                  ops.to_s16(c.float()))
        pk, C = self._packs, self.c
        B, _, h, w = df.shape
        dev = df.device

        def buf(ch):
            return torch.empty((B, ch, h, w), dtype=torch.float32, device=dev)

        A, E, G, X2 = buf(2 * C + 1), buf(2 * C + 1), buf(4 * C), buf(2 * C)
        ops.copy_into(df.float(), A[:, :C]); ops.copy_into(f.float(), A[:, C:2 * C]); ops.copy_into(o.float(), A[:, 2 * C:])
        ops.copy_into(c.float(), X2[:, C:]); ops.copy_into(c.float(), G[:, C:2 * C])
        ops.copy_into(df.float(), G[:, 3 * C:]); ops.copy_into(df.float(), E[:, C:2 * C]); ops.copy_into(o.float(), E[:, 2 * C:])
        t = ops.conv2d(pk.conv("1a", self.conv1[0]), A, act=ops.ACT_RELU)
# ... 6 lines not shown
        f_ = ops.conv2d(pk.conv("dc", self.dconv_as_conv(), tap_major=True), A[:, C:2 * C], out=E[:, :C],
                        offset=off, dmask=msk)
        ops.copy_into(f_, G[:, 2 * C:3 * C])
        t = ops.conv2d(pk.conv("3a", self.conv3[0]), E, act=ops.ACT_RELU, out=t)
        ops.conv2d(pk.conv("3b", self.conv3[2]), t, out=G[:, :C])
        t = ops.conv2d(pk.conv("4a", self.conv4[0]), G, act=ops.ACT_RELU, out=t)
        u = ops.conv2d(pk.conv("4b", self.conv4[2]), t, act=ops.ACT_RELU, out=u)
        return ops.conv2d(pk.conv("4c", self.conv4[4]), u)

    def forward16(self, df16, f, f16, o16, c16):
        pk, C = self._packs, self.c
        B, _, h, w = f.shape
        dev = f.device
        R = ops.ACT_RELU

        def s16(ch):
            return ops.S16.empty(B, ch, h, w, dev)

        t16, x16, u16, f_16, y16 = s16(2 * C), s16(C), s16(C), s16(C), s16(C)
        ops.conv2d_multi(pk.multi("1a", self.conv1[0], splits=[C, C, 1]), [df16, f16, o16], act=R, out16=t16, fp32_out=False)
        ops.conv2d_multi(pk.multi("1b", self.conv1[2]), [t16], out16=x16, fp32_out=False)
        ops.conv2d_multi(pk.multi("2a", self.conv2[0], splits=[C, C]), [x16, c16], act=R, out16=t16, fp32_out=False)
        ops.conv2d_multi(pk.multi("2b", self.conv2[2]), [t16], act=R, out16=u16, fp32_out=False)
        zc = self.conv2[4]
        om = ops.conv2d_multi(pk.multi("2z", zc.conv, scale=zc.out_scale, scale_dep=zc.scale), [u16])
        ops.deform_conv2d_s16(pk.conv("dc", self.dconv_as_conv(), tap_major=True), f, om[:, :18], om[:, 18:], f_16,
                              mask_is_logit=True)
        ops.conv2d_multi(pk.multi("3a", self.conv3[0], splits=[C, C, 1]), [f_16, df16, o16], act=R, out16=t16, fp32_out=False)
        ops.conv2d_multi(pk.multi("3b", self.conv3[2]), [t16], out16=y16, fp32_out=False)
        ops.conv2d_multi(pk.multi("4a", self.conv4[0], splits=[C, C, C, C]), [y16, c16, f_16, df16], act=R, out16=t16,
                         fp32_out=False)
        ops.conv2d_multi(pk.multi("4b", self.conv4[2]), [t16], act=R, out16=u16, fp32_out=False)
        return ops.conv2d_multi(pk.multi("4c", self.conv4[4]), [u16])

    def dconv_as_conv(self):
        return _ConvView(self.dconv)


class _ConvView:

    def __init__(self, d):
        self.weight, self.bias, self.stride, self.padding = d.weight, d.bias, d.stride, d.padding


class Blending(nn.Module):
    def __init__(self, c=128):
        super().__init__()
        self.mask = nn.Sequential(nn.Conv2d(c, c * 2, 1, 1, 0), nn.ReLU(True), nn.Conv2d(c * 2, 1, 3, 1, 1), nn.Sigmoid())
        self._packs = PackCache()

    def mask16(self, emap):
        pk = self._packs
        e16 = emap if isinstance(emap, ops.S16) else ops.to_s16(emap.float())
        B, _, h, w = e16.shape
        t16 = ops.S16.empty(B, self.mask[0].out_channels, h, w, e16.device)
        ops.conv2d_multi(pk.multi("0m", self.mask[0]), [e16], act=ops.ACT_RELU, out16=t16, fp32_out=False)
        return ops.conv2d(pk.conv("2", self.mask[2]), t16, act=ops.ACT_SIGMOID)

    @torch.no_grad()
    @ops.range_guarded
    def forward(self, f1, f2, emap):
        require_cuda(f1, f2, emap)
        pk = self._packs
        if ops.s16_active() and USE_S16_CHAIN:
            e16 = ops.to_s16(emap.float())
            B, _, h, w = e16.shape
            t16 = ops.S16.empty(B, self.mask[0].out_channels, h, w, e16.device)
            ops.conv2d_multi(pk.multi("0m", self.mask[0]), [e16], act=ops.ACT_RELU, out16=t16, fp32_out=False)
            t = t16
        else:
            t = ops.conv2d(pk.conv("0", self.mask[0]), emap.float(), act=ops.ACT_RELU)
        m = ops.conv2d(pk.conv("2", self.mask[2]), t, act=ops.ACT_SIGMOID)
        return ops.blend(f1.float().contiguous(), f2.float().contiguous(), m)


def getOcc(F12, I1, I2, binary=True):
    require_cuda(F12, I1, I2)
    return ops.get_occ(F12.float(), I1.float(), I2.float(), binary=binary)


def downflow8(flow, mode="bilinear"):
    if mode != "bilinear":
        raise NotImplementedError("downflow8: bilinear only")
    require_cuda(flow)
    h, w = flow.shape[-2:]
    assert h % 8 == 0 and w % 8 == 0
    return ops.downflow8(flow.float().contiguous())


class AccFlow(nn.Module):

    def __init__(self, ofe: nn.Module, warm_start=False, warm_iters=None):
        super().__init__()
        self.warm_start = bool(warm_start)
        self.warm_iters = warm_iters
        self.ofe: nn.Module = ofe
        self.hidden_channel = 128
        self.flow_encoder = FlowEncoder(self.hidden_channel)
        self.flow_decoder = FlowDecoder(self.hidden_channel)
        self.context = BasicEncoder(3, output_dim=self.hidden_channel, norm_fn="none")
        self.accplus = AccPlus(self.hidden_channel)
        self.blending = Blending(self.hidden_channel)
        self.mixed_precision = True

    def _fuse(self, dflow, flow_ini, F2n, c1, c2, cn, c1_16=None, defer=None):
        if c1_16 is not None and ops.s16_active() and USE_S16_CHAIN:
            N = dflow.shape[0]
            feats, feats16 = self.flow_encoder.encode16(torch.cat([flow_ini, dflow, F2n], dim=0).float().contiguous())
            f_ini, f = feats[:N], feats[2 * N:]
            h, w = dflow.shape[2:]
            o16 = ops.get_occ(dflow.float(), c1, c2, binary=True, out16=ops.S16.empty(N, 1, h, w, dflow.device))
            f_acc = self.accplus.forward16(feats16.batch(N, 2 * N), f, feats16.batch(2 * N, 3 * N), o16, c1_16)
            e16 = ops.get_occ(flow_ini.float(), c1, cn, binary=False, out16=ops.S16.empty(N, c1.shape[1], h, w, dflow.device))
            m = self.blending.mask16(e16)
            x16 = defer[0] if defer is not None else ops.S16.empty(N, f_acc.shape[1], h, w, dflow.device)
            ops.blend(f_ini.contiguous(), f_acc, m, out16=x16)
            if defer is not None:
                return self.flow_decoder.flow16(x16, out=defer[1]), None
            return self.flow_decoder._forward16(x16)
        f_ini, df, f = self.flow_encoder([flow_ini, dflow, F2n])
        o = getOcc(dflow, c1, c2)
        f_acc = self.accplus(df, f, o, c1)
        emap = getOcc(flow_ini, c1, cn, binary=False)
        f_fuse = self.blending(f_ini, f_acc, emap)
        return self.flow_decoder(f_fuse)

    @torch.no_grad()
    @ops.range_guarded
    def iter(self, I1, I2, In, F2n):
        require_cuda(I1, I2, In)
        if F2n is None:
            flows = downflow8(self.ofe(torch.cat([I1, I1, I2]), torch.cat([I2, In, In])))
            dflow, flow_ini, F2n = flows.chunk(3)
        else:
            flows = downflow8(self.ofe(torch.cat([I1, I1]), torch.cat([I2, In])))
            dflow, flow_ini = flows.chunk(2)
        c1, c2, cn = self.context([I1, I2, In])
        out_small, out = self._fuse(dflow.contiguous(), flow_ini.contiguous(), F2n.float().contiguous(), c1, c2, cn)
        return out_small.float(), out.float()

    @staticmethod
    def pair_schedule(n_frames):
        pairs = []
        for i in range(2, n_frames):
            pairs += [(i, i - 1), (i, 0)]
            if i == 2:
                pairs.append((1, 0))
        return pairs

    @torch.no_grad()
    def estimate_small(self, images, pairs, flow_init=None, iters=None, features=None):
        iters = getattr(self, "ofe_iters", 12) if iters is None else iters
        if hasattr(self.ofe, "estimate_pairs"):
            flows = self.ofe.estimate_pairs(images, pairs, iters=iters, flow_init=flow_init, features=features)
        else:
            flows = self.ofe(torch.cat([images[i] for i, _ in pairs]), torch.cat([images[j] for _, j in pairs]),
                             iters=iters, flow_init=flow_init)
        return downflow8(flows)

    def context_async(self, images):
        dev = images[0].device
        main = torch.cuda.current_stream(dev)
        side = _context_stream(dev)
        side.wait_stream(main)
        guarded = ops.current_mode() == ops.CONV_F16X3 and not ops.inside_guard()
        with torch.cuda.stream(side):
            flag = torch.zeros(1, dtype=torch.int32, device=dev) if guarded else None
            with (ops.guard_scope(flag) if guarded else contextlib.nullcontext()):
                ctx = self.context([im.float().contiguous() for im in images], want16=True)
        return (side, ctx, flag, images)

    def context_join(self, handle):
        side, ctx, flag, images = handle
        main = torch.cuda.current_stream(ctx[0][0].device)
        main.wait_stream(side)
        if flag is not None and int(flag.item()):
            ops.note_guard_trip("AccFlow.context")
            with ops.conv_mode(ops.CONV_BF16X6):
                return self.context([im.float().contiguous() for im in images], want16=True)
        for t in ctx[0]:
            t.record_stream(main)
        if ctx[1] is not None:
            for t in ctx[1]:
                t.data.record_stream(main)
        return ctx

    @torch.no_grad()
    @ops.range_guarded
    def fuse_chain(self, images, by_pair, ctx=None):
        if ctx is None:
            ctx = self.context([im.float().contiguous() for im in images], want16=True)
        if getattr(_CHAIN_TLS, "no_ksplit", False):
            with ops.ksplit_scope(False):
                return self._fuse_chain(images, by_pair, ctx)
        return self._fuse_chain(images, by_pair, ctx)

    def _fuse_chain(self, images, by_pair, ctx):
        n = len(images)
        ctx, ctx16 = ctx
        outs, F2n = [], by_pair[(1, 0)]
        if ctx16 is not None and ops.s16_active() and USE_S16_CHAIN and _hoist_now() and n > 3:
            return self._fuse_chain_hoisted(n, by_pair, ctx, ctx16)
        defer = ctx16 is not None and ops.s16_active() and USE_S16_CHAIN and USE_CHAIN_DEFER_UP and n > 3
        if defer:
            N, _, h, w = F2n.shape
            x16_all = ops.S16.empty((n - 2) * N, self.hidden_channel, h, w, F2n.device)
            small_all = torch.empty(((n - 2) * N, 2, h, w), dtype=torch.float32, device=F2n.device)
        for i in range(2, n):
            k0, k1 = (i - 2) * F2n.shape[0], (i - 1) * F2n.shape[0]
            F2n, up = self._fuse(by_pair[(i, i - 1)].contiguous(), by_pair[(i, 0)].contiguous(), F2n.contiguous(),
                                 ctx[i], ctx[i - 1], ctx[0], c1_16=ctx16[i] if ctx16 is not None else None,
                                 defer=(x16_all.batch(k0, k1), small_all[k0:k1]) if defer else None)
            outs.append(up)
        if defer:
            outs = list(self.flow_decoder.upsample16(x16_all, small_all).split(N, dim=0))
        return outs

    def _fuse_chain_hoisted(self, n, by_pair, ctx, ctx16):
        steps = list(range(2, n))
        N = by_pair[(1, 0)].shape[0]
        K = len(steps) * N
        flow_ini = torch.cat([by_pair[(i, 0)] for i in steps], dim=0).float().contiguous()
        dflow = torch.cat([by_pair[(i, i - 1)] for i in steps], dim=0).float().contiguous()
        feats, feats16 = self.flow_encoder.encode16(torch.cat([flow_ini, dflow], dim=0))
        f_ini, df16 = feats[:K], feats16.batch(K, 2 * K)
        c1 = span([ctx[i] for i in steps])
        c2 = span([ctx[i - 1] for i in steps])
        cn = ctx[0].expand(len(steps), -1, -1, -1) if N == 1 else ctx[0].repeat(len(steps), 1, 1, 1)
        h, w = dflow.shape[2:]
        o16 = ops.get_occ(dflow, c1, c2, binary=True, out16=ops.S16.empty(K, 1, h, w, dflow.device))
        m = self.blending.mask16(ops.get_occ(flow_ini, c1, cn, binary=False, out16=ops.S16.empty(K, c1.shape[1], h, w, dflow.device)))
        outs, F2n = [], by_pair[(1, 0)]
        defer = USE_CHAIN_DEFER_UP
        if defer:
            _, _, h, w = F2n.shape
            x16_all = ops.S16.empty(K, self.hidden_channel, h, w, F2n.device)
            small_all = torch.empty((K, 2, h, w), dtype=torch.float32, device=F2n.device)
        for k, i in enumerate(steps):
            k0, k1 = k * N, (k + 1) * N
            f, f16 = self.flow_encoder.encode16(F2n.float().contiguous())
            f_acc = self.accplus.forward16(df16.batch(k0, k1), f, f16, o16.batch(k0, k1), ctx16[i])
            if defer:
                F2n = self.flow_decoder.flow16(ops.blend(f_ini[k0:k1], f_acc, m[k0:k1], out16=x16_all.batch(k0, k1)),
                                               out=small_all[k0:k1])
            else:
                F2n, up = self.flow_decoder(ops.blend(f_ini[k0:k1], f_acc, m[k0:k1]))
                outs.append(up)
        if defer:
            outs = list(self.flow_decoder.upsample16(x16_all, small_all).split(N, dim=0))
        return outs

    @torch.no_grad()
    @ops.range_guarded
    def forward_warm(self, images):
        images = list(images)
        require_cuda(*images)
        n = len(images)
        if n < 3:
            return []
        N = images[0].shape[0]
        feats = {}
        adjacent = [(i, i - 1) for i in range(1, n)]
        small = self.estimate_small(images, adjacent, features=feats)
        adj = {p: small[k * N:(k + 1) * N] for k, p in enumerate(adjacent)}
        ctx = self.context([im.float().contiguous() for im in images])
        outs, F2n = [], adj[(1, 0)]
        for i in range(2, n):
            dflow = adj[(i, i - 1)].contiguous()
            seed = ops.compose_flow(dflow, F2n.contiguous())
            flow_ini = self.estimate_small(images, [(i, 0)], flow_init=seed, iters=self.warm_iters, features=feats)
            F2n, up = self._fuse(dflow, flow_ini.contiguous(), F2n.contiguous(), ctx[i], ctx[i - 1], ctx[0])
            outs.append(up)
        return outs

    @staticmethod
    def stack_frames(images):
        images = [im.float() for im in images]
        if len({tuple(im.shape) for im in images}) != 1:
            return images
        whole = span([im.contiguous() for im in images])
        return list(whole.split(images[0].shape[0], dim=0))

    @torch.no_grad()
    def forward(self, images, test_mode=False):
        images = list(images)
        require_cuda(*images)
        if len(images) < 3:
            return []
        if self.warm_start:
            return self.forward_warm(images)
        images = self.stack_frames(images)
        N = images[0].shape[0]
        pairs = self.pair_schedule(len(images))

        def run():
            handle = self.context_async(images) if CONTEXT_SIDE_STREAM else None
            small = self.estimate_small(images, pairs)
            ctx = self.context_join(handle) if handle is not None else None
            return self.fuse_chain(images, {p: small[k * N:(k + 1) * N] for k, p in enumerate(pairs)}, ctx=ctx)

        out, tripped = ops.optimistic(run, images[0].device)
        return run() if tripped else out

    @torch.no_grad()
    def forward_pair_sharded_stream(self, sequences, group=None, on_result=None):
        import itertools
# ... 80 lines not shown
```

accflow_amd/networks/_packs.py:

```python
import torch

from .. import ops


def _sig(tensors):
    return tuple((t.data_ptr(), t._version, str(t.device)) for t in tensors if t is not None)


def bn_fold(bn, conv_bias):
    inv = torch.rsqrt(bn.running_var.float() + bn.eps)
    scale = bn.weight.float() * inv if bn.weight is not None else inv
    bias = (conv_bias.float() if conv_bias is not None else 0.0) - bn.running_mean.float()
    bias = bias * scale
    if bn.bias is not None:
        bias = bias + bn.bias.float()
    return scale, bias


def _mark_ready(device):
    if device.type != "cuda":
        return None
    if torch.cuda.is_current_stream_capturing():
        return None
    st = torch.cuda.current_stream(device)
    ev = torch.cuda.Event()
    ev.record(st)
    return [ev, st.cuda_stream, device]


def _wait_ready(entry):
    r = entry[2]
    if r is None:
        return
    if r[0].query():
        entry[2] = None
        return
    cur = torch.cuda.current_stream(r[2])
    if cur.cuda_stream != r[1]:
        cur.wait_event(r[0])


class PackCache:
    def __init__(self):
        self._store = {}

    def clear(self):
        self._store.clear()

    def conv(self, key, conv, bn=None, scale=None, const_scale=None, C0=None, tap_major=False, rows_as_channels=False,
             scale_dep=None, lookup88=False, lookup_fused=False):
        deps = [conv.weight, conv.bias, scale_dep if scale_dep is not None else (None if callable(scale) else scale)]
        if callable(scale) and scale_dep is None:
            raise ValueError("PackCache.conv: a callable scale needs scale_dep (the parameter it derives from)")
        if bn is not None:
            deps += [bn.weight, bn.bias, bn.running_mean, bn.running_var]
        sig = _sig(deps) + (const_scale, C0, tap_major, rows_as_channels, lookup88, lookup_fused)
        key = (key, str(conv.weight.device))
        hit = self._store.get(key)
        if hit is not None and hit[0] == sig:
            _wait_ready(hit)
            return hit[1]
        with torch.no_grad():
            w, b = conv.weight, conv.bias
            sc = None
            if bn is not None:
                sc, b = bn_fold(bn, b)
            if scale is not None:
                s = (scale() if callable(scale) else scale).reshape(-1).float()
                sc = s if sc is None else sc * s
                b = b * s if b is not None else None
            if const_scale is not None:
                cs = torch.full((w.shape[0],), float(const_scale), dtype=torch.float32, device=w.device)
                sc = cs if sc is None else sc * cs
                b = b * float(const_scale) if b is not None else None
            padding = conv.padding
            if lookup88:
                co, ci, kh, kw = w.shape
                if (ci, kh, kw) != (324, 1, 1):
                    raise ValueError("lookup88: a 1x1 convolution over 4 x 81 correlation channels")
                w4 = w.float().reshape(co, 4, 9, 9).transpose(2, 3)
                w2 = torch.zeros((co, 4, 88), dtype=torch.float32, device=w.device)
                w2[:, :, :81] = w4.reshape(co, 4, 81)
                w = w2.reshape(co, 352, 1, 1)
            if lookup_fused:
                w = ops.lookup_fused_weight(w)
            if rows_as_channels:
                co, ci, kh, kw = w.shape
                w2 = torch.zeros((co, 16, 1, kw), dtype=torch.float32, device=w.device)
                w2[:, :ci * kh, 0] = w.float().reshape(co, ci * kh, kw)
                w, padding = w2, (0, conv.padding[1])
            pk = ops.PackedConv(w, b, stride=conv.stride, padding=padding, scale=sc, C0=C0,
                                tap_major=tap_major)
        self._store[key] = [sig, pk, _mark_ready(conv.weight.device)]
        return pk

    def multi(self, key, conv, bn=None, scale=None, scale_dep=None, splits=None, strided=False, in_ranges=None, with_bias=True):
        deps = [conv.weight, conv.bias, scale_dep if scale_dep is not None else (None if callable(scale) else scale)]
        if callable(scale) and scale_dep is None:
            raise ValueError("PackCache.multi: a callable scale needs scale_dep (the parameter it derives from)")
        if bn is not None:
            deps += [bn.weight, bn.bias, bn.running_mean, bn.running_var]
        sig = _sig(deps) + (tuple(splits) if splits else None, bool(strided), tuple(in_ranges) if in_ranges else None, bool(with_bias))
        key = (key, str(conv.weight.device))
        hit = self._store.get(key)
        if hit is not None and hit[0] == sig:
            _wait_ready(hit)
            return hit[1]
        with torch.no_grad():
            w, b = conv.weight.float(), (conv.bias if with_bias else None)
            if in_ranges:
                if splits or strided or bn is not None:
                    raise ValueError("PackCache.multi: in_ranges stands alone (it defines the sources)")
                w = torch.cat([w[:, a:b_] for a, b_ in in_ranges], dim=1).contiguous()
                splits = [b_ - a for a, b_ in in_ranges]
            sc = None
            if bn is not None:
                sc, b = bn_fold(bn, b)
            if scale is not None:
                s = (scale() if callable(scale) else scale).reshape(-1).float()
                sc = s if sc is None else sc * s
                b = b * s if b is not None else None
            stride = conv.stride[0] if isinstance(conv.stride, (tuple, list)) else conv.stride
            if strided:
                if stride != 2:
                    raise ValueError("PackCache.multi: strided=True is for stride-2 convolutions")
                pk = ops.PackedMulti.from_strided(w, b, conv.padding, scale=sc)
            else:
                if stride != 1:
                    raise ValueError("PackCache.multi: a stride-%d convolution needs strided=True" % stride)
                pk = ops.PackedMulti.from_cat(w, b, list(splits) if splits else [w.shape[1]], conv.padding, scale=sc)
        self._store[key] = [sig, pk, _mark_ready(conv.weight.device)]
        return pk

    def multi_proj(self, key, conv, proj, bn=None, bn_proj=None):
        deps = [conv.weight, conv.bias, proj.weight, proj.bias]
        for b_ in (bn, bn_proj):
            if b_ is not None:
                deps += [b_.weight, b_.bias, b_.running_mean, b_.running_var]
        sig = _sig(deps) + (bn is not None, bn_proj is not None)
        key = (key, str(conv.weight.device))
        hit = self._store.get(key)
        if hit is not None and hit[0] == sig:
            _wait_ready(hit)
            return hit[1]
        with torch.no_grad():
            sc, b = (None, conv.bias) if bn is None else bn_fold(bn, conv.bias)
            scp, bp = (None, proj.bias) if bn_proj is None else bn_fold(bn_proj, proj.bias)
            pk = ops.PackedMulti.from_strided_with_projection(conv.weight.float(), b, conv.padding, proj.weight.float(), bp,
                                                              scale=sc, scale_proj=scp)
        self._store[key] = [sig, pk, _mark_ready(conv.weight.device)]
        return pk

    def multi_cat(self, key, convs):
        deps = []
        for c in convs:
            deps += [c.weight, c.bias]
        sig = _sig(deps)
        key = (key, str(convs[0].weight.device))
        hit = self._store.get(key)
        if hit is not None and hit[0] == sig:
            _wait_ready(hit)
            return hit[1]
        with torch.no_grad():
            w = torch.cat([c.weight.float() for c in convs], dim=0).contiguous()
            b = torch.cat([c.bias.float() for c in convs], dim=0).contiguous()
            pk = ops.PackedMulti.from_cat(w, b, [w.shape[1]], convs[0].padding)
        self._store[key] = [sig, pk, _mark_ready(convs[0].weight.device)]
        return pk

    def conv_cat(self, key, convs, C0=None, in_slices=None, with_bias=True):
        deps = []
        for c in convs:
            deps += [c.weight, c.bias]
        sig = _sig(deps) + (C0, tuple(in_slices) if in_slices else None, with_bias)
        key = (key, str(convs[0].weight.device))
        hit = self._store.get(key)
        if hit is not None and hit[0] == sig:
            _wait_ready(hit)
            return hit[1]
        with torch.no_grad():
            w = torch.cat([c.weight.float() for c in convs], dim=0)
            if in_slices:
                w = torch.cat([w[:, a:b] for a, b in in_slices], dim=1)
            w = w.contiguous()
            b = torch.cat([c.bias.float() for c in convs], dim=0).contiguous() if with_bias else None
            pk = ops.PackedConv(w, b, stride=convs[0].stride, padding=convs[0].padding, C0=C0)
        self._store[key] = [sig, pk, _mark_ready(convs[0].weight.device)]
        return pk


def span(items):
    items = list(items)
    if len(items) == 1:
        return items[0]
    t0 = items[0]
    off, ok = t0.storage_offset(), True
    for t in items:
        ok &= (t.untyped_storage().data_ptr() == t0.untyped_storage().data_ptr() and t.storage_offset() == off
               and t.dtype == t0.dtype and t.stride() == t0.stride() and t.shape[1:] == t0.shape[1:] and t.is_contiguous())
        off += t.shape[0] * (t.stride(0) if t.dim() else 0)
    if ok:
        B = sum(t.shape[0] for t in items)
        return t0.as_strided((B,) + tuple(t0.shape[1:]), t0.stride(), t0.storage_offset())
    return torch.cat(items, dim=0)


def require_cuda(*tensors):
    for t in tensors:
        if not t.is_cuda:
            raise RuntimeError(
                "accflow_amd: this module runs only on an MI355X through libaccflow_hip (got a %s tensor); "
                "there is no CPU path in the product - the CPU restatement lives in oracle/ for tests." % t.device)
```

accflow_amd/networks/gma/gma.py:

```python
import os

import torch.nn as nn

from ... import ops
from ..raft.extractor import BasicEncoder
from ..raft.raft import RAFT
from .modules import Attention
from .update import GMAUpdateBlock

SHARE_ATTENTION = os.environ.get("ACCFLOW_GMA_SHARE_ATTENTION", "1") != "0"
ALTERNATE_ATTENTION = os.environ.get("ACCFLOW_ALTERNATE_ATTENTION", "0") == "1"


class RAFTGMA(RAFT):
    KEEP_CONTEXT_RUNS = True

    def __init__(self, args):
        nn.Module.__init__(self)
        self.args = args
        self.hidden_dim = hdim = 128
        self.context_dim = cdim = 128
        args.corr_levels = 4
        args.corr_radius = 4
        if "dropout" not in self.args:
            self.args.dropout = 0
        if "alternate_attention" not in self.args:
            self.args.alternate_attention = False
        self.fnet = BasicEncoder(output_dim=256, norm_fn="instance", dropout=args.dropout)
        self.cnet = BasicEncoder(output_dim=hdim + cdim, norm_fn="batch", dropout=args.dropout)
        self.update_block = GMAUpdateBlock(self.args, hidden_dim=hdim)
        self.att = Attention(args=self.args, dim=cdim, heads=self.args.num_heads, max_pos_size=160, dim_head=cdim)

    def _x_dim(self):
        return 384

    def _alternate_attention(self):
        return ALTERNATE_ATTENTION or bool(getattr(self.args, "alternate_attention", False))

    def _prepack(self):
        super()._prepack()
        self.att._packs.conv("qk", self.att.to_qk)

    def _prepare_context(self, ws, cnet_feat, ids=None):
        super()._prepare_context(ws, cnet_feat)
        fast = ops.current_mode() != ops.CONV_F32
        inp = ws.inp.contiguous()
        if not fast:
            ws.attention = self.att(inp)
            return
        runs = None
        if ids is not None and SHARE_ATTENTION and len(set(ids)) < len(ids):
            slot, reps, runs = {}, [], []
            for b, key in enumerate(ids):
                if key not in slot:
                    slot[key] = len(reps)
                    reps.append(b)
                if runs and runs[-1][0] == slot[key]:
                    runs[-1][2] = b + 1
                else:
                    runs.append([slot[key], b, b + 1])
            inp = inp[reps].contiguous()
        if self._alternate_attention() and ops.s16_active():
            ws.attention = self.att.forward_alt(inp, runs=runs)
            return
        ws.attention = self.att.forward_t(inp, runs=runs)

    def _iteration(self, ws, corr_fn, coords1, last):
        self._lookup_and_flow(ws, corr_fn, coords1)
        return self.update_block.step(ws, coords1, want_mask=last, attention=ws.attention)
```

accflow_amd/networks/gma/update.py:

```python
import torch
import torch.nn as nn

from ... import ops
from .._packs import PackCache, require_cuda
from ..raft.update import BasicMotionEncoder, BasicUpdateBlock, FlowHead, SepConvGRU, UpdateWorkspace
from .modules import Aggregate


class GMAUpdateBlock(BasicUpdateBlock):
    def __init__(self, args, hidden_dim=128):
        nn.Module.__init__(self)
        self.args = args
        self.encoder = BasicMotionEncoder(args)
        self.gru = SepConvGRU(hidden_dim=hidden_dim, input_dim=128 + hidden_dim + hidden_dim)
        self.flow_head = FlowHead(hidden_dim, hidden_dim=256)
        self.mask = nn.Sequential(nn.Conv2d(128, 256, 3, padding=1), nn.ReLU(inplace=True),
                                  nn.Conv2d(256, 64 * 9, 1, padding=0))
        self.aggregator = Aggregate(args=self.args, dim=128, dim_head=128, heads=self.args.num_heads)
        self._packs = PackCache()

    def prepack(self):
        super().prepack()
        self.aggregator._packs.conv("v", self.aggregator.to_v)

    def aggregate(self, ws, attention):
        hd = ws.hidden
        mg = ws.hx[:, hd + 256:hd + 384]
        if ws.s16 and (getattr(attention, "attn16", None) is not None or getattr(attention, "alt", None) is not None):
            self.aggregator.forward_ws(attention, ws, None, ws.x16.channels(128, 256))
            return
        self.aggregator(attention, ws.motion.contiguous(), out=mg)
        if ws.s16:
            ops.to_s16(mg, ws.x16.channels(128, 256))

    def step(self, ws, coords1, want_mask, attention=None):
        self.motion_encoder(ws)
        self.aggregate(ws, attention)
        self.gru_step(ws)
        self.flow_delta(ws, coords1=coords1)
        return self.up_mask(ws) if want_mask else None

    @torch.no_grad()
    @ops.range_guarded
    def forward(self, net, inp, corr, flow, attention):
        require_cuda(net, inp, corr, flow, attention)
        B, _, h, w = net.shape
        ws = UpdateWorkspace(B, h, w, net.device, x_dim=384)
        ops.copy_into(net.float(), ws.net)
        ops.copy_into(inp.float(), ws.inp)
        ops.copy_into(corr.float(), ws.corr)
        ws.fill_s16_inputs(flow.float().contiguous(), is_flow=True)
        if not ws.s16:
            ops.flow_from_coords(flow.float().contiguous(), dst0=ws.flow, dst1=ws.motion_flow, stack16=ws.flow16, is_flow=True)
        self.motion_encoder(ws)
        self.aggregate(ws, attention)
        self.gru_step(ws)
        delta = self.flow_delta(ws)
        mask = self.up_mask(ws)
        return ws.net32(), mask, delta
```

accflow_amd/networks/raft/raft.py:

```python
import argparse

import torch
import torch.nn as nn

from ... import ops
from .._packs import require_cuda
from . import corr as _corr
from .corr import AlternateCorrBlock, CorrBlock
from .extractor import BasicEncoder
from . import update as _update
from .update import BasicUpdateBlock, UpdateWorkspace


import os

N_STREAMS = max(1, int(os.environ.get("ACCFLOW_STREAMS", "2")))
PROFILE_STANDALONE_LOOKUP = False
USE_CORR_PACKS = os.environ.get("ACCFLOW_CORR_PACKS", "1") == "1"
ALTERNATE_CORR = os.environ.get("ACCFLOW_ALTERNATE_CORR", "0") == "1"
_STREAMS = {}


ENCODER_STREAMS = int(os.environ.get("ACCFLOW_ENCODER_STREAMS", "2"))
GROUP_STREAM_PRIORITY = int(os.environ.get("ACCFLOW_GROUP_PRIORITY", "-1"))


def _side_streams(device, n):
    key = (str(device), n)
    if key not in _STREAMS:
        _STREAMS[key] = [torch.cuda.Stream(device=device, priority=GROUP_STREAM_PRIORITY) for _ in range(n)]
    return _STREAMS[key]


class RAFT(nn.Module):
    KEEP_CONTEXT_RUNS = False

    def __init__(self, args):
        super().__init__()
        self.args = args
        if getattr(args, "small", False):
            raise NotImplementedError("RAFT-small is not reachable from networks.build_flow_estimator "
                                      "(networks/__init__.py:8 fixes small=False)")
        self.hidden_dim = hdim = 128
        self.context_dim = cdim = 128
        args.corr_levels = 4
        args.corr_radius = 4
        if "dropout" not in self.args:
            self.args.dropout = 0
        if "alternate_corr" not in self.args:
            self.args.alternate_corr = False
        self.fnet = BasicEncoder(output_dim=256, norm_fn="instance", dropout=args.dropout)
        self.cnet = BasicEncoder(output_dim=hdim + cdim, norm_fn="batch", dropout=args.dropout)
        self.update_block = BasicUpdateBlock(self.args, hidden_dim=hdim)

    def freeze_bn(self):
        for m in self.modules():
            if isinstance(m, nn.BatchNorm2d):
                m.eval()

    def initialize_flow(self, img):
        N, _, H, W = img.shape
        return (ops.coords_grid(N, H // 8, W // 8, img.device), ops.coords_grid(N, H // 8, W // 8, img.device))

    def upsample_flow(self, flow, mask):
        require_cuda(flow, mask)
        return ops.convex_upsample(flow.float(), mask.float())

    def _x_dim(self):
        return 256

    def _alternate(self):
        return ALTERNATE_CORR or bool(getattr(self.args, "alternate_corr", False))

    def _prepack(self):
        self.update_block.prepack()

    def _prepare_context(self, ws, cnet_feat, ids=None):
        if isinstance(cnet_feat, tuple):
            ops.split_tanh_relu_indexed(cnet_feat[0], cnet_feat[1], ws.net, ws.inp, self.hidden_dim, self.context_dim)
        else:
            ops.split_tanh_relu(cnet_feat, ws.net, ws.inp, self.hidden_dim, self.context_dim)
        if ws.s16:
            ops.to_s16(ws.net, ws.h16)

    def _lookup_and_flow(self, ws, corr_fn, coords1):
        if ws.s16 and corr_fn.supports_s16():
            ub = self.update_block
            if _update.FUSE_LOOKUP and ub.encoder.convc1.out_channels == 256 and isinstance(corr_fn, CorrBlock):
                if PROFILE_STANDALONE_LOOKUP and ops.profiler.ACTIVE is not None:
                    corr_fn.lookup_s16(coords1, ws.corr16)
                corr_fn.lookup_convc1(coords1, ub._packs.conv("c1f", ub.encoder.convc1, lookup_fused=True), ws.c1_16,
                                      cache=(ws.descs, "lookup"))
                ws.c1_fused = True
            else:
                corr_fn.lookup_s16(coords1, ws.corr16, cache=(ws.descs, "lookup"))
            ops.flow_from_coords_s16(coords1, ws.flow, ws.motion_flow if ws.x_dim > 256 else None, ws.stack16, ws.motion16, 126,
                                     cache=(ws.descs, "flow"))
            return
        if ws.s16:
            corr_fn(coords1, out=ws.corr)
            ws.fill_s16_inputs(coords1, is_flow=False)
            return
        corr_fn(coords1, out=ws.corr)
        ops.flow_from_coords(coords1, dst0=ws.flow, dst1=ws.motion_flow, stack16=ws.flow16)

    def _iteration(self, ws, corr_fn, coords1, last):
        self._lookup_and_flow(ws, corr_fn, coords1)
        return self.update_block.step(ws, coords1, want_mask=last)

    @classmethod
    def _group_cuts(cls, B, n_groups, flip=False, ctx_ids=None):
        flip = flip and not cls.KEEP_CONTEXT_RUNS
        cuts = [(g * B + (n_groups - 1 if flip else 0)) // n_groups for g in range(n_groups + 1)]
        if ctx_ids is not None and cls.KEEP_CONTEXT_RUNS:
            for g in range(1, n_groups):
                while cuts[g] < cuts[g + 1] - 1 and ctx_ids[cuts[g]] == ctx_ids[cuts[g] - 1]:
                    cuts[g] += 1
        return cuts

    def _refine(self, fmap1, fmap2, cnet_feat, iters, flow_init, packed=None, ctx_ids=None, ready=None, return_low=False):
        if iters < 1:
            raise ValueError("iters must be >= 1")
        indexed = isinstance(cnet_feat, tuple)
        B = len(cnet_feat[1]) if indexed else cnet_feat.shape[0]
        dev = (cnet_feat[0] if indexed else cnet_feat).device
        _, _, h, w = (cnet_feat[0] if indexed else cnet_feat).shape
        self._prepack()
        n_groups = N_STREAMS if B >= 4 else 1
        ctx_ready, flip = None, False
        if isinstance(ready, tuple):
            ready, ctx_ready, flip = ready
        cuts = self._group_cuts(B, n_groups, flip, ctx_ids)
        bounds = list(zip(cuts[:-1], cuts[1:]))
        main = torch.cuda.current_stream()
        streams = [main] if n_groups == 1 else _side_streams(dev, n_groups)
        out_all = torch.empty((B, 2, 8 * h, 8 * w), dtype=torch.float32, device=dev)
        low_all = torch.empty((B, 2, h, w), dtype=torch.float32, device=dev) if return_low else None
        forked = None
        if ctx_ready is not None:
            forked = torch.cuda.Event()
            forked.record(main)
        state = []
        early = ready is not None and packed is not None and n_groups > 1
        for (b0, b1), st in zip(bounds, streams):
            if st != main:
                if early:
                    st.wait_event(ready)
                else:
                    st.wait_stream(main)
            with torch.cuda.stream(st):
                if packed is not None and isinstance(packed[0], ops.AltPyramid):
                    corr_fn = AlternateCorrBlock.from_frames(packed[0], packed[1][b0:b1], packed[2][b0:b1])
                elif packed is not None:
                    corr_fn = CorrBlock.from_packs(packed[0], packed[1][b0:b1], packed[2][b0:b1])
                else:
                    block = AlternateCorrBlock if self._alternate() else CorrBlock
                    corr_fn = block(fmap1[b0:b1], fmap2[b0:b1], radius=self.args.corr_radius)
                if early and ctx_ready is not None:
                    st.wait_event(ctx_ready)
                elif early:
                    st.wait_stream(main)
                ws = UpdateWorkspace(b1 - b0, h, w, dev, hidden=self.hidden_dim, x_dim=self._x_dim())
                self._prepare_context(ws, (cnet_feat[0], cnet_feat[1][b0:b1]) if indexed else cnet_feat[b0:b1],
                                      ctx_ids[b0:b1] if ctx_ids is not None else None)
                fi = flow_init[b0:b1] if flow_init is not None else None
                coords1 = ops.coords_grid(b1 - b0, h, w, dev, flow_init=fi)
            state.append((st, corr_fn, ws, coords1))
        masks = [None] * n_groups
        for itr in range(iters):
            for g, (st, corr_fn, ws, coords1) in enumerate(state):
                with torch.cuda.stream(st):
                    masks[g] = self._iteration(ws, corr_fn, coords1, last=(itr == iters - 1))
        for g, (st, corr_fn, ws, coords1) in enumerate(state):
            with torch.cuda.stream(st):
                if forked is not None and early:
                    st.wait_event(forked)
                ops.flow_from_coords(coords1, dst0=ws.flow)
                ops.convex_upsample(ws.flow, masks[g], out=out_all[bounds[g][0]:bounds[g][1]])
                if return_low:
                    low_all[bounds[g][0]:bounds[g][1]].copy_(ws.flow)
            if st != main:
                main.wait_stream(st)
        return (out_all, low_all) if return_low else out_all

    @torch.no_grad()
    def forward(self, image1, image2, iters=12, flow_init=None):
        require_cuda(image1, image2)
        image1 = image1.float().contiguous()
        image2 = image2.float().contiguous()

        def run():
            fmap1, fmap2 = self.fnet([image1, image2])
            cnet_feat = self.cnet(image1)
            return self._refine_guarded(fmap1.contiguous(), fmap2.contiguous(), cnet_feat, iters, flow_init)

        out, tripped = ops.optimistic(run, image1.device)
        return run() if tripped else out

    def _refine_guarded(self, *args, **kwargs):
        dev = next(self.parameters()).device
        return ops.with_range_guard(lambda: self._refine(*args, **kwargs), dev, name="%s.refine" % type(self).__name__)

    @torch.no_grad()
    def encode_frames(self, frames, fnet_ids, cnet_ids, features=None, after_fmap=None):
        feats = features if features is not None else {}
        if feats.get("mode") != ops.current_mode():
            feats.clear()
            feats.update({"fmap": {}, "cnet": {}, "mode": ops.current_mode()})
        jobs = [(key, enc, [f for f in sorted(set(ids)) if f not in feats[key]])
                for key, enc, ids in (("fmap", self.fnet, fnet_ids), ("cnet", self.cnet, cnet_ids))]
        dev = frames[0].device
        side = None
        if (ENCODER_STREAMS in (1, 3) and N_STREAMS > 1 and all(todo for _, _, todo in jobs)
                and (ops.current_mode() != ops.CONV_F16X3 or ops.inside_guard())):
            main = torch.cuda.current_stream(dev)
            side = _side_streams(dev, N_STREAMS)[-1]
            side.wait_stream(main)
        for key, enc, todo in jobs:
            if todo:
                if side is not None and key == "cnet":
                    with torch.cuda.stream(side):
                        outs = enc([frames[f].float().contiguous() for f in todo])
                else:
                    outs = enc([frames[f].float().contiguous() for f in todo])
                base = getattr(outs[0], "_base", None)
                whole = not feats[key] and base is not None and base.shape[0] == len(todo) * outs[0].shape[0]
                feats[key + "_base"] = (base, {f: k for k, f in enumerate(todo)}) if whole else None
                if key == "fmap":
                    feats.pop("corr_packs", None)
                feats[key].update(zip(todo, outs))
            if key == "fmap" and after_fmap is not None:
                after_fmap(feats)
        if side is not None:
            main.wait_stream(side)
            base = feats.get("cnet_base")
            for t in ([base[0]] if base is not None else []) + list(feats["cnet"].values()):
                t.record_stream(main)
        return feats

    @torch.no_grad()
    def estimate_pairs(self, frames, pairs, iters=12, flow_init=None, features=None, return_low=False):
        require_cuda(*frames)
        N = frames[0].shape[0]
        feats = self.encode_pairs(frames, pairs, features)
        ready = feats.pop("fmap_event", None)
        home = feats.pop("refine_at_home", None)
        if ready is not None and home is not None and flow_init is None:
            ready = (ready, home[0], home[1])
        return self._estimate_encoded(frames, pairs, feats, ready, iters, flow_init, return_low)

    @torch.no_grad()
    def estimate_video(self, frames, iters=12, warm_start=True, pairs=None, features=None):
        require_cuda(*frames)
        if pairs is None:
            pairs = [(t, t + 1) for t in range(len(frames) - 1)]
        pairs = list(pairs)
        if not pairs:
            raise ValueError("estimate_video: needs at least two frames (one pair)")
        first, rest = (int(iters[0]), int(iters[1])) if isinstance(iters, (tuple, list)) else (iters, iters)
        feats = self.encode_pairs(frames, pairs, features)
        if not warm_start:
            return self.estimate_pairs(frames, pairs, first, features=feats, return_low=True)
        ups, lows = [], []
        for k, pair in enumerate(pairs):
            seed = ops.forward_interpolate(lows[-1]) if lows else None
            up, low = self.estimate_pairs(frames, [pair], first if k == 0 else rest, flow_init=seed, features=feats,
                                          return_low=True)
            ups.append(up)
            lows.append(low)
        return torch.cat(ups, dim=0), torch.cat(lows, dim=0)

    def _packs_usable(self, feats, pairs):
        fb = feats.get("fmap_base")
        return (fb is not None and USE_CORR_PACKS and not self._alternate() and _corr.LAYOUT == "disp" and all(f in fb[1] for p in pairs for f in p)
                and ops.corr_packs_supported(fb[0].shape[1], fb[0].shape[2], fb[0].shape[3]))

    @torch.no_grad()
    def encode_pairs(self, frames, pairs, features=None):
        def after_fmap(feats):
            if (ENCODER_STREAMS not in (2, 3) or N_STREAMS < 2 or not self._packs_usable(feats, pairs)
                    or not (ops.current_mode() != ops.CONV_F16X3 or ops.inside_guard())):
                return
            cp = feats.get("corr_packs")
            if cp is not None and cp.mode == ops.current_mode() and "fmap_event" in feats:
                return
            if cp is None or cp.mode != ops.current_mode():
                feats["corr_packs"] = ops.corr_pack(feats["fmap_base"][0])
            ev = torch.cuda.Event()
            ev.record(torch.cuda.current_stream(frames[0].device))
            feats["fmap_event"] = ev

        feats = self.encode_frames(frames, {i for p in pairs for i in p}, {i for i, _ in pairs}, features, after_fmap=after_fmap)
        self._prepack()
        return feats

    def _estimate_encoded(self, frames, pairs, feats, ready, iters, flow_init, return_low=False):
        N = frames[0].shape[0]
        cb = feats.get("cnet_base")
        if cb is not None and all(i in cb[1] for i, _ in pairs):
            cfeat = (cb[0], [cb[1][i] * N + n for i, _ in pairs for n in range(N)])
            n_items, hw8 = len(cfeat[1]), tuple(cb[0].shape[2:])
        else:
            cfeat = torch.cat([feats["cnet"][i] for i, _ in pairs], dim=0)
            n_items, hw8 = cfeat.shape[0], tuple(cfeat.shape[2:])
        assert n_items == N * len(pairs)
        if flow_init is not None:
            require_cuda(flow_init)
            if tuple(flow_init.shape) != (n_items, 2) + hw8:
                raise RuntimeError("estimate_pairs: flow_init must be (len(pairs)*N, 2, H/8, W/8)")
        ctx_ids = [(i, n) for i, _ in pairs for n in range(N)]
        fb = feats.get("fmap_base")
        if self._alternate() and fb is not None and all(f in fb[1] for p in pairs for f in p):
            idx1 = [fb[1][i] * N + n for i, _ in pairs for n in range(N)]
            idx2 = [fb[1][j] * N + n for _, j in pairs for n in range(N)]

            def refine_alt():
                pyr = ops.corr_alt_pyramid(fb[0])
                return self._refine(None, None, cfeat, iters, flow_init, packed=(pyr, idx1, idx2), ctx_ids=ctx_ids,
                                    return_low=return_low)

            return ops.with_range_guard(refine_alt, frames[0].device, name="%s.refine" % type(self).__name__)
        if self._packs_usable(feats, pairs):
            idx1 = [fb[1][i] * N + n for i, _ in pairs for n in range(N)]
            idx2 = [fb[1][j] * N + n for _, j in pairs for n in range(N)]

            first = [ready]

            def refine_packed():
                ev = first.pop() if first else None
                cp = feats.get("corr_packs")
                if cp is None or cp.mode != ops.current_mode():
                    cp, ev = ops.corr_pack(fb[0]), None
                    feats["corr_packs"] = cp
                return self._refine(None, None, cfeat, iters, flow_init, packed=(cp, idx1, idx2), ctx_ids=ctx_ids, ready=ev,
                                    return_low=return_low)

            return ops.with_range_guard(refine_packed, frames[0].device, name="%s.refine" % type(self).__name__)
        fmap1 = torch.cat([feats["fmap"][i] for i, _ in pairs], dim=0)
        fmap2 = torch.cat([feats["fmap"][j] for _, j in pairs], dim=0)
        return self._refine_guarded(fmap1, fmap2, cfeat, iters, flow_init, ctx_ids=ctx_ids, return_low=return_low)


def default_args():
    return argparse.Namespace(small=False, mixed_precision=True)
```

accflow_amd/networks/raft/update.py:

```python
import torch
import torch.nn as nn

import os

from ... import ops
from .._packs import PackCache, require_cuda

FUSE_LOOKUP = os.environ.get("ACCFLOW_FUSE_LOOKUP", "1") == "1"
USE_H16_STATE = os.environ.get("ACCFLOW_H16_STATE", "1") == "1"


def h16_state_supported():
    return not ops.S16_VIA_MULTI and ops.conv_gru16_supported()


class FlowHead(nn.Module):
    def __init__(self, input_dim=128, hidden_dim=256):
        super().__init__()
        self.conv1 = nn.Conv2d(input_dim, hidden_dim, 3, padding=1)
        self.conv2 = nn.Conv2d(hidden_dim, 2, 3, padding=1)
        self.relu = nn.ReLU(inplace=True)


class SepConvGRU(nn.Module):
    def __init__(self, hidden_dim=128, input_dim=192 + 128):
        super().__init__()
        cin = hidden_dim + input_dim
        for suffix, ks, pad in (("1", (1, 5), (0, 2)), ("2", (5, 1), (2, 0))):
            for gate in "zrq":
                setattr(self, "conv%s%s" % (gate, suffix), nn.Conv2d(cin, hidden_dim, ks, padding=pad))
        self.hidden_dim = hidden_dim
        self.input_dim = input_dim


class BasicMotionEncoder(nn.Module):
    def __init__(self, args):
        super().__init__()
        cor_planes = args.corr_levels * (2 * args.corr_radius + 1) ** 2
        self.convc1 = nn.Conv2d(cor_planes, 256, 1, padding=0)
        self.convc2 = nn.Conv2d(256, 192, 3, padding=1)
        self.convf1 = nn.Conv2d(2, 128, 7, padding=3)
        self.convf2 = nn.Conv2d(128, 64, 3, padding=1)
        self.conv = nn.Conv2d(64 + 192, 128 - 2, 3, padding=1)


class UpdateWorkspace:

    def __init__(self, B, h, w, device, hidden=128, x_dim=256):
        def buf(c):
            return torch.empty((B, c, h, w), dtype=torch.float32, device=device)
        self.B, self.h, self.w, self.hidden, self.x_dim = B, h, w, hidden, x_dim
        self._buf = buf
        self.s16 = bool(ops.s16_active())
        self.net_in_h16 = False
        self.c1_fused = False
        self.descs = {}
        self.hx = buf(hidden + x_dim)
        self.net = self.hx[:, :hidden]
        self.inp = self.hx[:, hidden:hidden + 128]
        self.motion = self.hx[:, hidden + 128:hidden + 256]
        self.motion_conv = self.hx[:, hidden + 128:hidden + 254]
        self.motion_flow = self.hx[:, hidden + 254:hidden + 256]
        self.x = self.hx[:, hidden:]
        self.z = buf(hidden)
        self.flow = buf(2)
        self._corr = None
        if not self.s16:
            self.rh = buf(hidden)
            self.flow16 = buf(16)
            self.c1 = buf(256)
            self.corflo = buf(256)
            self.f1 = buf(128)
            self.head = buf(256)
        self.mask = None
        self.gru_pre = None
        if self.s16:
            def s(c, zero=False):
                return ops.S16.empty(B, c, h, w, device, zero=zero)
            self._corr16 = None
            self.stack16 = s(16)
            self.c1_16, self.corflo16, self.f1_16, self.head16 = s(256), s(256), s(128), s(256)
            self.h16, self.rh16 = s(hidden), s(hidden)
            self.net_in_h16 = USE_H16_STATE and h16_state_supported()
            self.x16 = s(x_dim - 128)
            self.motion16 = self.x16.channels(0, 128)


def _fill_s16_inputs(ws, flow_or_coords, is_flow):
    if not ws.s16:
        return
    B, h, w = ws.B, ws.h, ws.w
    c = ws.corr.view(B, 4, 9, 9, h, w).transpose(2, 3).reshape(B, 4, 81, h, w)
    c88 = torch.zeros((B, 4, 88, h, w), dtype=torch.float32, device=ws.corr.device)
    c88[:, :, :81] = c
    ops.to_s16(c88.view(B, 352, h, w), ws.corr16)
    ops.to_s16(ws.net, ws.h16)
    ops.flow_from_coords_s16(flow_or_coords, ws.flow, ws.motion_flow, ws.stack16, ws.motion16, 126, is_flow=is_flow)


UpdateWorkspace.fill_s16_inputs = _fill_s16_inputs


def _ws_corr(ws):
    if ws._corr is None:
        ws._corr = ws._buf(324)
    return ws._corr


UpdateWorkspace.corr = property(_ws_corr)


def _ws_corr16(ws):
    if ws._corr16 is None:
        ws._corr16 = ops.S16.empty(ws.B, ops.LOOKUP_S16_CHANNELS, ws.h, ws.w, ws.hx.device)
    return ws._corr16


UpdateWorkspace.corr16 = property(_ws_corr16)


def _ws_net32(ws):
    return ws.h16.to_float() if (ws.s16 and ws.net_in_h16) else ws.net.contiguous()


UpdateWorkspace.net32 = _ws_net32


class BasicUpdateBlock(nn.Module):
    def __init__(self, args, hidden_dim=128, input_dim=128):
        super().__init__()
        self.args = args
        self.encoder = BasicMotionEncoder(args)
        self.gru = SepConvGRU(hidden_dim=hidden_dim, input_dim=128 + hidden_dim)
        self.flow_head = FlowHead(hidden_dim, hidden_dim=256)
        self.mask = nn.Sequential(nn.Conv2d(128, 256, 3, padding=1), nn.ReLU(inplace=True),
                                  nn.Conv2d(256, 64 * 9, 1, padding=0))
        self._packs = PackCache()

    def prepack(self):
        pk, e, g, f = self._packs, self.encoder, self.gru, self.flow_head
        pk.conv("c1", e.convc1); pk.conv("c2", e.convc2); pk.conv("f1s", e.convf1, rows_as_channels=True)
        if ops.s16_active():
            pk.conv("c1s", e.convc1, lookup88=True)
            if FUSE_LOOKUP:
                pk.conv("c1f", e.convc1, lookup_fused=True)
        pk.conv("f2", e.convf2)
        pk.conv("cf", e.conv)
        for s in ("1", "2"):
            self._gru_packs(s)
        pk.conv("fh1", f.conv1); pk.conv("fh2", f.conv2)
        pk.conv("m0", self.mask[0]); pk.conv("m2", self.mask[2], const_scale=0.25)

    def motion_encoder(self, ws):
        pk, e = self._packs, self.encoder
        if ws.s16:
            R, D = ops.ACT_RELU, ws.descs
            fused = ws.c1_fused
            if "c2" in D:
                for k in ("c2", "f1", "f2", "cf") if fused else ("c1", "c2", "f1", "f2", "cf"):
                    ops.conv2d(None, None, cache=(D, k))
                return
            if not fused:
                ops.conv2d(pk.conv("c1s", e.convc1, lookup88=True), ws.corr16, out16=ws.c1_16, act=R, fp32_out=False,
                           algo_cin=324, cache=(D, "c1"))
            ops.conv2d(pk.conv("c2", e.convc2), ws.c1_16, out16=ws.corflo16.channels(0, 192), act=R, fp32_out=False,
                       cache=(D, "c2"))
            ops.conv2d(pk.conv("f1s", e.convf1, rows_as_channels=True), ws.stack16, out16=ws.f1_16, act=R, fp32_out=False,
                       algo_cin=2 * 7, cache=(D, "f1"))
            ops.conv2d(pk.conv("f2", e.convf2), ws.f1_16, out16=ws.corflo16.channels(192, 256), act=R, fp32_out=False,
                       cache=(D, "f2"))
            want32 = ws.x_dim > 256
            ops.conv2d(pk.conv("cf", e.conv), ws.corflo16, out16=ws.motion16.channels(0, 126), act=R, fp32_out=want32,
                       out=ws.motion_conv if want32 else None, cache=(D, "cf"))
            return
        ops.conv2d(pk.conv("c1", e.convc1), ws.corr, out=ws.c1, act=ops.ACT_RELU)
        ops.conv2d(pk.conv("c2", e.convc2), ws.c1, out=ws.corflo[:, :192], act=ops.ACT_RELU)
        ops.conv2d(pk.conv("f1s", e.convf1, rows_as_channels=True), ws.flow16, out=ws.f1, act=ops.ACT_RELU, algo_cin=2 * 7)
        ops.conv2d(pk.conv("f2", e.convf2), ws.f1, out=ws.corflo[:, 192:], act=ops.ACT_RELU)
        ops.conv2d(pk.conv("cf", e.conv), ws.corflo, out=ws.motion_conv, act=ops.ACT_RELU)

    def _gru_packs(self, s):
        pk, g, hd = self._packs, self.gru, self.gru.hidden_dim
        cin = hd + g.input_dim
        var, ctx = [(0, hd), (hd + 128, cin)], [(hd, hd + 128)]
        zr = [getattr(g, "convz" + s), getattr(g, "convr" + s)]
        q = [getattr(g, "convq" + s)]
        return (pk.conv_cat("zr%sv" % s, zr, C0=hd, in_slices=var), pk.conv_cat("zr%sc" % s, zr, in_slices=ctx, with_bias=False),
                pk.conv_cat("q%sv" % s, q, C0=hd, in_slices=var), pk.conv_cat("q%sc" % s, q, in_slices=ctx, with_bias=False))

    def gru_context(self, ws):
        B, h, w, hd = ws.B, ws.h, ws.w, ws.hidden
        ws.gru_pre = {}
        inp = ops.to_s16(ws.inp) if ws.s16 else ws.inp
        p32 = ws.s16 and ws.net_in_h16
        for s in ("1", "2"):
            _, zrc, _, qc = self._gru_packs(s)
            ws.gru_pre["zr" + s] = ops.conv2d(zrc, inp, algo_cin=0, p32_out=p32)
            ws.gru_pre["q" + s] = ops.conv2d(qc, inp, algo_cin=0, p32_out=p32)

    def gru_step(self, ws):
        if getattr(ws, "gru_pre", None) is None:
            self.gru_context(ws)
        rest = ws.hx[:, ws.hidden + 128:]
        cin = ws.hidden + ws.x_dim
        if ws.s16:
            D = ws.descs
            if "zr1" in D:
                for k in ("zr1", "q1", "zr2", "q2"):
                    ops.conv2d(None, None, cache=(D, k))
                return
            h16s = ws.net_in_h16
            for s in ("1", "2"):
                zrv, _, qv, _ = self._gru_packs(s)
                ops.conv2d(zrv, ws.h16, in1=ws.x16, out=ws.z, act=ops.ACT_SIGMOID, epi=ops.EPI_GRU_ZR, e0=ws.h16 if h16s else ws.net,
                           out16=ws.rh16, fp32_out=False, pre=ws.gru_pre["zr" + s], algo_cin=cin, cache=(D, "zr" + s))
                ops.conv2d(qv, ws.rh16, in1=ws.x16, out=None if h16s else ws.net, act=ops.ACT_TANH, epi=ops.EPI_GRU_Q,
                           e0=ws.h16 if h16s else ws.net, e1=ws.z, out16=ws.h16, fp32_out=not h16s,
                           pre=ws.gru_pre["q" + s], algo_cin=cin, cache=(D, "q" + s))
            return
        for s in ("1", "2"):
            zrv, _, qv, _ = self._gru_packs(s)
            ops.conv2d(zrv, ws.net, in1=rest, out=ws.z, act=ops.ACT_SIGMOID, epi=ops.EPI_GRU_ZR, e0=ws.net, out2=ws.rh,
                       pre=ws.gru_pre["zr" + s], algo_cin=cin)
            ops.conv2d(qv, ws.rh, in1=rest, out=ws.net, act=ops.ACT_TANH, epi=ops.EPI_GRU_Q, e0=ws.net, e1=ws.z,
                       pre=ws.gru_pre["q" + s], algo_cin=cin)

    def flow_delta(self, ws, coords1=None, out=None):
        pk, f = self._packs, self.flow_head
        if ws.s16:
            D = ws.descs
            if coords1 is not None and ops.profiler.ACTIVE is None and "fh12" in D and D["fh12"][1] is coords1:
                return ops.conv2d_tapgemm(None, None, None, cache=(D, "fh12"))
            p1, p2 = pk.conv("fh1", f.conv1), pk.conv("fh2", f.conv2)
            if ops.tapgemm_eligible(p1, p2, ws.h16):
                if coords1 is not None:
                    return ops.conv2d_tapgemm(p1, p2, ws.h16, out=coords1, epi=ops.EPI_ACCUM, e0=coords1, cache=(D, "fh12"))
                return ops.conv2d_tapgemm(p1, p2, ws.h16, out=out)
            ops.conv2d(p1, ws.h16, out16=ws.head16, act=ops.ACT_RELU, fp32_out=False, cache=(ws.descs, "fh1"))
            if coords1 is not None:
                return ops.conv2d(pk.conv("fh2", f.conv2), ws.head16, out=coords1, epi=ops.EPI_ACCUM, e0=coords1)
            return ops.conv2d(pk.conv("fh2", f.conv2), ws.head16, out=out)
        ops.conv2d(pk.conv("fh1", f.conv1), ws.net, out=ws.head, act=ops.ACT_RELU)
        if coords1 is not None:
            return ops.conv2d(pk.conv("fh2", f.conv2), ws.head, out=coords1, epi=ops.EPI_ACCUM, e0=coords1)
        return ops.conv2d(pk.conv("fh2", f.conv2), ws.head, out=out)

    def up_mask(self, ws):
        pk = self._packs
        if ws.mask is None:
            ws.mask = torch.empty((ws.B, 576, ws.h, ws.w), dtype=torch.float32, device=ws.hx.device)
        if ws.s16:
            ops.conv2d(pk.conv("m0", self.mask[0]), ws.h16, out16=ws.head16, act=ops.ACT_RELU, fp32_out=False)
            return ops.conv2d(pk.conv("m2", self.mask[2], const_scale=0.25), ws.head16, out=ws.mask)
        ops.conv2d(pk.conv("m0", self.mask[0]), ws.net, out=ws.head, act=ops.ACT_RELU)
        return ops.conv2d(pk.conv("m2", self.mask[2], const_scale=0.25), ws.head, out=ws.mask)

    def step(self, ws, coords1, want_mask):
        self.motion_encoder(ws)
        self.gru_step(ws)
        self.flow_delta(ws, coords1=coords1)
        return self.up_mask(ws) if want_mask else None

    @torch.no_grad()
    @ops.range_guarded
    def forward(self, net, inp, corr, flow, upsample=True):
        require_cuda(net, inp, corr, flow)
        B, _, h, w = net.shape
        ws = UpdateWorkspace(B, h, w, net.device)
        ops.copy_into(net.float(), ws.net)
        ops.copy_into(inp.float(), ws.inp)
        ops.copy_into(corr.float(), ws.corr)
        ws.fill_s16_inputs(flow.float().contiguous(), is_flow=True)
        if not ws.s16:
            ops.flow_from_coords(flow.float().contiguous(), dst0=ws.flow, dst1=ws.motion_flow, stack16=ws.flow16, is_flow=True)
        self.motion_encoder(ws)
        self.gru_step(ws)
        delta = self.flow_delta(ws)
        mask = self.up_mask(ws)
        return ws.net32(), mask, delta
```

accflow_amd/ops.py:

```python
import contextlib
import ctypes
import functools
import threading

import torch

from . import _lib, profiler
from ._lib import ConvDesc

import os

ACT_NONE, ACT_RELU, ACT_SIGMOID, ACT_TANH = 0, 1, 2, 3
CONV_F32, CONV_BF16X3, CONV_BF16X6, CONV_F16X3 = 0, 2, 3, 4
_MODES = {"f32": CONV_F32, "bf16x3": CONV_BF16X3, "bf16x6": CONV_BF16X6, "f16x3": CONV_F16X3}
CONV_MODE = _MODES[os.environ.get("ACCFLOW_CONV_MODE", "f16x3").lower()]
_tls = threading.local()


USE_PATCH = os.environ.get("ACCFLOW_CONV_PATCH", "1") == "1"


def set_conv_mode(name):
    global CONV_MODE
    CONV_MODE = _MODES[name.lower()]
# ... 1209 lines not shown
    w4 = w.detach().float().reshape(co, 4, 9, 9).transpose(2, 3).reshape(co, 4, 81)
    out = torch.zeros((co, LOOKUP_FUSED_K), dtype=torch.float32, device=w.device)
    out[:, :320] = w4[:, :, :80].reshape(co, 4, 10, 8).permute(0, 2, 1, 3).reshape(co, 320)
    out[:, 320:324] = w4[:, :, 80]
    return out.reshape(co, LOOKUP_FUSED_K, 1, 1)


def corr_lookup_convc1(pyr, coords, pk, out16=None, out=None, act=ACT_RELU, cache=None):
    r = _replay(cache, "accflow_corr_lookup_convc1_s16")
    if r is not None:
        return r
    lib = _lib.load()
    if not isinstance(pyr, DispPyramid):
        raise RuntimeError("corr_lookup_convc1: needs the displaced pyramid")
    if current_mode() != CONV_F16X3 or pk.wpatch16 is None or pk.Cin != LOOKUP_FUSED_K or pk.Cout != 256:
        raise RuntimeError("corr_lookup_convc1: needs the f16x3 mode and the fused pack of a 324 -> 256 1x1 convolution")
    coords = _dense(coords, "coords")
    B, _, H8, W8 = coords.shape
    if (B, H8, W8) != (pyr.B, pyr.H8, pyr.W8) or (out16 is None and out is None):
        raise RuntimeError("corr_lookup_convc1: shape mismatch")
    if out16 is not None and tuple(out16.shape) != (B, pk.Cout, H8, W8):
        raise RuntimeError("corr_lookup_convc1: out16 shape %s" % (out16.shape,))
    out_bs = 0
    if out is not None:
        out_bs = _plane4(out, "out")
        if tuple(out.shape) != (B, pk.Cout, H8, W8):
            raise RuntimeError("corr_lookup_convc1: out shape %s" % (tuple(out.shape),))
    lv = pyr.levels
    tm = profiler.ACTIVE
    t0 = tm.begin() if tm is not None and tm.wants("lookup_convc1") else None
    args = (_p(lv[0]), _p(lv[1]), _p(lv[2]), _p(lv[3]), _p(coords), _p(pk.wpatch16), _p(pk.wscale16),
            _p(pk.bias) if pk.bias is not None else None,
            ctypes.c_void_p(out16.ptr()) if out16 is not None else None, out16.bs if out16 is not None else 0,
            _p(out) if out is not None else None, out_bs, int(act), _p(_guard(coords.device)), B, H8, W8, pk.Cout)
    _check(lib.accflow_corr_lookup_convc1_s16(*args, _stream()), "accflow_corr_lookup_convc1_s16")
    ret = out16 if out16 is not None else out
    if t0 is not None:
        tm.end("lookup_convc1", t0, 2.0 * 324 * pk.Cout * B * H8 * W8, "lookup+convc1 B%d %dx%d" % (B, H8, W8),
               work_exec=2.0 * LOOKUP_FUSED_K * pk.Cout * B * H8 * W8)
    elif cache is not None and tm is None:
        cache[0][cache[1]] = (lib.accflow_corr_lookup_convc1_s16, args, ret, (pyr, coords, pk, out16, out))
    return ret


def flow_from_coords_s16(coords1, dst0, dst1, stack16, motion16, motion_ch, is_flow=False, cache=None):
    if _replay(cache, "accflow_flow_from_coords_s16") is not None:
        return
    lib = _lib.load()
    coords1 = _dense(coords1, "coords1")
    B, _, H8, W8 = coords1.shape
    b0 = _plane4(dst0, "dst0") if dst0 is not None else 0
    b1 = _plane4(dst1, "dst1") if dst1 is not None else 0
    if tuple(stack16.shape) != (B, 16, H8, W8) or motion_ch % 2 or (
            motion16 is not None and (motion16.shape[0] != B or tuple(motion16.shape[2:]) != (H8, W8))):
        raise RuntimeError("flow_from_coords_s16: shape mismatch")
    args = (_p(coords1), _p(dst0), b0, _p(dst1), b1, ctypes.c_void_p(stack16.ptr()), stack16.bs,
            ctypes.c_void_p(motion16.ptr() if motion16 is not None else 0), motion16.bs if motion16 is not None else 0,
            int(motion_ch), _p(_guard(coords1.device)), int(bool(is_flow)), B, H8, W8)
    _check(lib.accflow_flow_from_coords_s16(*args, _stream()), "accflow_flow_from_coords_s16")
    if cache is not None and profiler.ACTIVE is None:
        cache[0][cache[1]] = (lib.accflow_flow_from_coords_s16, args, True, (coords1, dst0, dst1, stack16, motion16))


def _corr_lookup_rowmajor(pyramid, coords, out=None):
    lib = _lib.load()
    coords = _dense(coords, "coords")
    B, _, H8, W8 = coords.shape
    if out is None:
        out = torch.empty((B, 324, H8, W8), dtype=torch.float32, device=coords.device)
    out_bs = _plane4(out, "out")
    for t in pyramid:
        _dense(t, "pyramid level")
    tm = profiler.ACTIVE
    t0 = tm.begin() if tm is not None and tm.wants("corr_lookup") else None
    _check(lib.accflow_corr_lookup_f32(_p(pyramid[0]), _p(pyramid[1]), _p(pyramid[2]), _p(pyramid[3]),
                                       _p(coords), _p(out), out_bs, B, H8, W8, _stream()),
           "accflow_corr_lookup_f32")
    if t0 is not None:
        tm.end("corr_lookup", t0, LOOKUP_BYTES_PER_PX * B * H8 * W8)
    return out


def convex_upsample(flow, mask, out=None):
    lib = _lib.load()
    fbs, mbs = _plane4(flow, "flow"), _plane4(mask, "mask")
    B, _, H8, W8 = flow.shape
    if mask.shape[1] != 576 or mask.shape[2:] != flow.shape[2:]:
        raise RuntimeError("convex_upsample: mask must be (B,576,H8,W8)")
    if out is None:
        out = torch.empty((B, 2, 8 * H8, 8 * W8), dtype=torch.float32, device=flow.device)
    elif tuple(out.shape) != (B, 2, 8 * H8, 8 * W8) or not out.is_contiguous():
        raise RuntimeError("convex_upsample: out must be a contiguous (B,2,8*H8,8*W8) tensor (a batch slice is fine)")
    _check(lib.accflow_convex_upsample_f32(_p(flow), fbs, _p(mask), mbs, _p(out), B, H8, W8, _stream()),
           "accflow_convex_upsample_f32")
    return out


def backwarp(img, flow, out=None):
    lib = _lib.load()
    ibs, fbs = _plane4(img, "image"), _plane4(flow, "flow")
    B, C, H, W = img.shape
    if tuple(flow.shape) != (B, 2, H, W):
        raise RuntimeError("backwarp: flow must be (N,2,H,W) matching image")
    if out is None:
        out = torch.empty((B, C, H, W), dtype=torch.float32, device=img.device)
    obs = _plane4(out, "out")
    _check(lib.accflow_backwarp_f32(_p(img), ibs, _p(flow), fbs, _p(out), obs, B, C, H, W, _stream()),
           "accflow_backwarp_f32")
    return out


def compose_flow(step, acc):
    lib = _lib.load()
    sbs, abs_ = _plane4(step, "step"), _plane4(acc, "acc")
    B, C, H, W = step.shape
    if C != 2 or tuple(acc.shape) != (B, 2, H, W):
        raise RuntimeError("compose_flow: both flows must be (B,2,H,W)")
    out = torch.empty((B, 2, H, W), dtype=torch.float32, device=step.device)
    _check(lib.accflow_compose_flow_f32(_p(step), sbs, _p(acc), abs_, _p(out), 2 * H * W, B, H, W, _stream()),
           "accflow_compose_flow_f32")
    return out


def get_occ(flow, i1, i2, binary=True, out=None, out16=None):
    lib = _lib.load()
    fbs, b1, b2 = _plane4(flow, "flow"), _plane4(i1, "I1"), _plane4(i2, "I2")
    B, C, H, W = i1.shape
    if out16 is not None:
        if tuple(out16.shape) != (B, 1 if binary else C, H, W):
            raise RuntimeError("get_occ: out16 shape %s" % (out16.shape,))
        _check(lib.accflow_get_occ_s16(_p(flow), fbs, _p(i1), b1, _p(i2), b2, ctypes.c_void_p(out16.ptr()), out16.bs,
                                       _p(_guard(i1.device)), B, C, H, W, int(bool(binary)), _stream()), "accflow_get_occ_s16")
        return out16
    if out is None:
        out = torch.empty((B, 1 if binary else C, H, W), dtype=torch.float32, device=i1.device)
    obs = _plane4(out, "out")
    _check(lib.accflow_get_occ_f32(_p(flow), fbs, _p(i1), b1, _p(i2), b2, _p(out), obs, B, C, H, W,
                                   int(bool(binary)), _stream()), "accflow_get_occ_f32")
    return out


def downflow8(flow):
    lib = _lib.load()
    _plane4(flow, "flow")
    flow = _dense(flow, "flow")
    B, C, H, W = flow.shape
    if H % 8 or W % 8:
        raise AssertionError("downflow8: H and W must be multiples of 8")
    out = torch.empty((B, C, H // 8, W // 8), dtype=torch.float32, device=flow.device)
    _check(lib.accflow_downflow8_f32(_p(flow), _p(out), B, C, H, W, _stream()), "accflow_downflow8_f32")
    return out


def forward_interpolate(flow, out=None):
    lib = _lib.load()
    if not (isinstance(flow, torch.Tensor) and flow.is_cuda and flow.is_floating_point() and flow.dim() in (3, 4)
            and flow.shape[-3] == 2):
        raise RuntimeError("forward_interpolate: expected a (B, 2, h, w) or (2, h, w) floating-point CUDA tensor, got %s" % (
            (tuple(flow.shape), flow.dtype, flow.device) if isinstance(flow, torch.Tensor) else type(flow),))
    shape = tuple(flow.shape)
    src = _dense(flow.float().contiguous(), "flow")
    h, w = shape[-2:]
    B = shape[0] if len(shape) == 4 else 1
    if B * h * w == 0:
        raise RuntimeError("forward_interpolate: empty flow %s" % (shape,))
    if out is None:
        out = torch.empty(shape, dtype=torch.float32, device=flow.device)
    else:
        nbytes = 4 * src.numel()
        if (tuple(_dense(out, "out").shape) != shape or out.device != flow.device
                or (out.data_ptr() < src.data_ptr() + nbytes and src.data_ptr() < out.data_ptr() + nbytes)):
            raise RuntimeError("forward_interpolate: out must be a float32 tensor of shape %s on %s that does not overlap flow" % (
                shape, flow.device))
    _check(lib.accflow_forward_interpolate_f32(_p(src), _p(out), B, h, w, _stream()), "accflow_forward_interpolate_f32")
    return out


def instance_stats_finalize(stats, eps=1e-5, c0=0, C=None):
    lib = _lib.load()
    B, Ctot = stats.partial.shape[:2]
    C = Ctot - c0 if C is None else C
    mr = torch.empty((B, C, 2), dtype=torch.float32, device=stats.partial.device)
    _check(lib.accflow_instance_stats_finalize_sub_f32(_p(stats.partial), stats.slots, Ctot, int(c0), _p(mr), B, C, float(eps),
                                                       _stream()), "accflow_instance_stats_finalize_sub_f32")
    return mr


def instance_norm_proj(x, stats, proj, proj_stats, proj_c0, out16, eps=1e-5):
    lib = _lib.load()
    x = _dense(x, "x")
    B, C, H, W = x.shape
    pbs = _plane4(proj, "proj")
    if (tuple(proj.shape) != (B, C, H, W) or tuple(out16.shape) != (B, C, H, W) or tuple(stats.partial.shape[:2]) != (B, C)
            or proj_stats.partial.shape[0] != B or proj_c0 + C > proj_stats.partial.shape[1]):
        raise RuntimeError("instance_norm_proj: shape mismatch")
    mr = torch.empty(4 * B * C, dtype=torch.float32, device=x.device)
    _check(lib.accflow_instance_norm_apply_s16proj_f32(_p(x), _p(stats.partial), stats.slots, _p(proj), pbs, _p(proj_stats.partial),
                                                       proj_stats.slots, proj_stats.partial.shape[1], int(proj_c0), _p(mr),
                                                       ctypes.c_void_p(out16.ptr()), out16.bs, _p(_guard(x.device)), B, C, H * W,
                                                       float(eps), _stream()), "accflow_instance_norm_apply_s16proj_f32")
    return out16


def instance_norm(x, mode, res=None, eps=1e-5, out=None, stats=None, out16=None, fp32_out=True):
    lib = _lib.load()
    x = _dense(x, "x")
    B, C, H, W = x.shape
    if out16 is not None:
        if stats is None or tuple(stats.partial.shape[:2]) != (B, C) or tuple(out16.shape) != (B, C, H, W):
            raise RuntimeError("instance_norm: out16 needs the producing convolution's statistics and a matching S16 tensor")
        o32 = (x if out is None else _dense(out, "out")) if fp32_out else None
        mr = torch.empty(2 * B * C, dtype=torch.float32, device=x.device)
        if isinstance(res, S16):
            if mode != 2 or tuple(res.shape) != (B, C, H, W):
                raise RuntimeError("instance_norm: an S16 residual belongs to mode 2 and must match x")
            _check(lib.accflow_instance_norm_apply_s16res_f32(_p(x), _p(stats.partial), stats.slots, _p(mr),
                                                              ctypes.c_void_p(res.ptr()), res.bs, _p(o32),
                                                              ctypes.c_void_p(out16.ptr()), out16.bs, _p(_guard(x.device)), B, C,
                                                              H * W, float(eps), _stream()), "accflow_instance_norm_apply_s16res_f32")
            return o32 if fp32_out else out16
        if res is not None:
            _dense(res, "res")
        _check(lib.accflow_instance_norm_apply_s16_f32(_p(x), _p(stats.partial), stats.slots, _p(mr), _p(res), _p(o32),
                                                       ctypes.c_void_p(out16.ptr()), out16.bs, _p(_guard(x.device)), B, C, H * W,
                                                       float(eps), int(mode), _stream()), "accflow_instance_norm_apply_s16_f32")
        return o32 if fp32_out else out16
    if out is None:
        out = x
    if res is not None:
        _dense(res, "res")
    if stats is not None:
        if tuple(stats.partial.shape[:2]) != (B, C):
            raise RuntimeError("instance_norm: statistics do not belong to this tensor")
        mr = torch.empty(2 * B * C, dtype=torch.float32, device=x.device)
        _check(lib.accflow_instance_norm_apply_f32(_p(x), _p(stats.partial), stats.slots, _p(mr), _p(res), _p(out), B, C, H * W,
                                                   float(eps), int(mode), _stream()), "accflow_instance_norm_apply_f32")
        return out
    _check(lib.accflow_instance_norm_f32(_p(x), _p(res), _p(out), B, C, H * W, float(eps), int(mode), _stream()),
           "accflow_instance_norm_f32")
    return out


def split_tanh_relu(cnet, net, inp, hd, cd):
    lib = _lib.load()
    cnet = _dense(cnet, "cnet")
    B, _, H, W = cnet.shape
    nbs, ibs = _plane4(net, "net"), _plane4(inp, "inp")
    _check(lib.accflow_split_tanh_relu_f32(_p(cnet), _p(net), nbs, _p(inp), ibs, B, hd, cd, H * W, _stream()),
           "accflow_split_tanh_relu_f32")


def split_tanh_relu_indexed(cnet_items, idx, net, inp, hd, cd):
    lib = _lib.load()
    cnet_items = _dense(cnet_items, "cnet")
    n, _, H, W = cnet_items.shape
    B = len(idx)
    nbs, ibs = _plane4(net, "net"), _plane4(inp, "inp")
    if net.shape[0] != B or inp.shape[0] != B:
        raise RuntimeError("split_tanh_relu_indexed: one index per output item")
    arr = (ctypes.c_int * B)(*idx)
    _check(lib.accflow_split_tanh_relu_idx_f32(_p(cnet_items), n, arr, _p(net), nbs, _p(inp), ibs, B, hd, cd, H * W, _stream()),
           "accflow_split_tanh_relu_idx_f32")


def coords_grid(B, H8, W8, device, flow_init=None):
    lib = _lib.load()
    out = torch.empty((B, 2, H8, W8), dtype=torch.float32, device=device)
    if flow_init is not None:
        flow_init = _dense(flow_init.float().contiguous(), "flow_init")
    _check(lib.accflow_coords_grid_f32(_p(out), _p(flow_init), B, H8, W8, _stream()), "accflow_coords_grid_f32")
    return out


def flow_from_coords(coords1, dst0=None, dst1=None, stack16=None, is_flow=False):
    lib = _lib.load()
    coords1 = _dense(coords1, "coords1")
    B, _, H8, W8 = coords1.shape
    b0 = _plane4(dst0, "dst0") if dst0 is not None else 0
    b1 = _plane4(dst1, "dst1") if dst1 is not None else 0
    if stack16 is not None and tuple(_dense(stack16, "stack16").shape) != (B, 16, H8, W8):
        raise RuntimeError("flow_from_coords: stack16 must be (B, 16, h, w)")
    _check(lib.accflow_flow_from_coords_f32(_p(coords1), _p(dst0), b0, _p(dst1), b1, _p(stack16), int(bool(is_flow)), B, H8, W8,
                                            _stream()),
           "accflow_flow_from_coords_f32")


def blend(f1, f2, m, out16=None):
    lib = _lib.load()
    f1, f2, m = _dense(f1, "f1"), _dense(f2, "f2"), _dense(m, "m")
    B, C, H, W = f1.shape
    if out16 is not None:
        if tuple(out16.shape) != (B, C, H, W):
            raise RuntimeError("blend: out16 shape %s" % (out16.shape,))
        _check(lib.accflow_blend_s16(_p(f1), _p(f2), _p(m), ctypes.c_void_p(out16.ptr()), out16.bs, _p(_guard(f1.device)), B, C,
                                     H * W, _stream()), "accflow_blend_s16")
        return out16
    out = torch.empty_like(f1)
    _check(lib.accflow_blend_f32(_p(f1), _p(f2), _p(m), _p(out), B, C, H * W, _stream()), "accflow_blend_f32")
    return out


def activation_(x, act):
    lib = _lib.load()
    xbs = _plane4(x, "x")
    B, C, H, W = x.shape
    _check(lib.accflow_activation_f32(_p(x), xbs, B, C, H * W, int(act), _stream()), "accflow_activation_f32")
    return x


def copy_into(src, dst):
    lib = _lib.load()
    sbs, dbs = _plane4(src, "src"), _plane4(dst, "dst")
    if src.shape != dst.shape:
        raise RuntimeError("copy_into: shape mismatch")
    B, C, H, W = src.shape
    _check(lib.accflow_copy_f32(_p(src), sbs, _p(dst), dbs, B, C, H * W, _stream()), "accflow_copy_f32")
    return dst


def gma_attention(qk, D, scale):
    lib = _lib.load()
    qk = _dense(qk, "qk")
    B, _, H, W = qk.shape
    P = H * W
    attn = torch.empty((B, 1, P, P), dtype=torch.float32, device=qk.device)
    _check(lib.accflow_gma_attention_f32(_p(qk), _p(attn), B, D, P, float(scale), _stream()),
           "accflow_gma_attention_f32")
    return attn


def gma_aggregate(attn, v, fmap, gamma, out=None):
    lib = _lib.load()
    attn, v, fmap = _dense(attn, "attn"), _dense(v, "v"), _dense(fmap, "fmap")
    gamma = _dense(gamma.detach().float().contiguous(), "gamma")
    B, D, H, W = fmap.shape
    if out is None:
        out = torch.empty_like(fmap)
    obs = _plane4(out, "out")
    _check(lib.accflow_gma_aggregate_f32(_p(attn), _p(v), _p(fmap), _p(gamma), _p(out), obs, B, D, H * W, _stream()),
           "accflow_gma_aggregate_f32")
    return out


def gma_attention_t(qk, D, scale):
    lib = _lib.load()
    qk = _dense(qk, "qk")
    B, _, H, W = qk.shape
    P = H * W
    attn_t = torch.empty((B, P, P), dtype=torch.float32, device=qk.device)
    md = current_mode()
    ws = (torch.empty(lib.accflow_gma_attention_ws_bytes(D, H, W), dtype=torch.uint8, device=qk.device)
          if md != CONV_F32 else None)
    _check(lib.accflow_gma_attention_t_f32(_p(qk), _p(attn_t), _p(ws), md, B, D, H, W, float(scale), _stream()),
           "accflow_gma_attention_t_f32")
    return attn_t


def gma_aggregate_t(attn_t, v, fmap, gamma, out=None, mode=None):
    lib = _lib.load()
    attn_t, v, fmap = _dense(attn_t, "attnT"), _dense(v, "v"), _dense(fmap, "fmap")
    gamma = _dense(gamma.detach().float().contiguous(), "gamma")
    B, D, H, W = fmap.shape
    if out is None:
        out = torch.empty_like(fmap)
    obs = _plane4(out, "out")
    md = current_mode() if mode is None else mode
    ws = torch.empty(lib.accflow_gma_aggregate_ws_bytes(B, D, H * W), dtype=torch.uint8, device=fmap.device)
    guard = _guard(fmap.device) if md == CONV_F16X3 else None
    _check(lib.accflow_gma_aggregate_t_f32(_p(attn_t), _p(v), _p(fmap), _p(gamma), _p(out), obs, _p(ws), md, _p(guard), B, D, H, W,
                                           _stream()), "accflow_gma_aggregate_t_f32")
    return out


def gma_attention_s16(qk, D, scale):
    lib = _lib.load()
    qk = _dense(qk, "qk")
    B, _, H, W = qk.shape
    P = H * W
    attn16 = S16.empty(B, P, H, W, qk.device)
    ws = torch.empty(lib.accflow_gma_attention_s16_ws_bytes(D, H, W), dtype=torch.uint8, device=qk.device)
    _check(lib.accflow_gma_attention_s16(_p(qk), ctypes.c_void_p(attn16.ptr()), _p(ws), _p(_guard(qk.device)), B, D, H, W,
                                         float(scale), _stream()), "accflow_gma_attention_s16")
    return attn16


def gma_aggregate_s16(attn16_item, v, fmap0, fmap_bs, gamma, out0, out_bs, out16_0, out16_bs, n, D, H, W):
    lib = _lib.load()
    v = _dense(v, "v")
    gamma = _dense(gamma.detach().float().contiguous(), "gamma")
    ws = torch.empty(lib.accflow_gma_aggregate_s16_ws_bytes(n, D, H * W), dtype=torch.uint8, device=v.device)
    _check(lib.accflow_gma_aggregate_s16(ctypes.c_void_p(attn16_item), _p(v), ctypes.c_void_p(fmap0), fmap_bs, _p(gamma),
                                         ctypes.c_void_p(out0), out_bs, ctypes.c_void_p(out16_0), out16_bs, _p(ws),
                                         _p(_guard(v.device)), n, D, H, W, _stream()), "accflow_gma_aggregate_s16")


class AltAttention:
    __slots__ = ("packs", "stats", "D", "H", "W")

    def __init__(self, packs, stats, D, H, W):
        self.packs, self.stats, self.D, self.H, self.W = packs, stats, D, H, W

    @property
    def nbytes(self):
        return self.packs.numel() + self.stats.numel() * 4

    def __len__(self):
        return self.packs.shape[1]


def gma_attention_alt(qk, D, scale):
    lib = _lib.load()
    qk = _dense(qk, "qk")
    B, C2, H, W = qk.shape
    if D != 128 or C2 != 2 * D:
        raise RuntimeError("gma_attention_alt: D = 128 only (got D = %d, %d channels)" % (D, C2))
    P = H * W
    pack_bytes = 2 * (D // 8) * lib.accflow_conv_coutpad(P) * 16
# ... 26 lines not shown
```

include/accflow_hip.h:

```cpp
#ifndef ACCFLOW_HIP_H
#define ACCFLOW_HIP_H

#ifdef __cplusplus
extern "C" {
#endif

#define ACCFLOW_ABI_VERSION 20

enum { ACCFLOW_ACT_NONE = 0, ACCFLOW_ACT_RELU = 1, ACCFLOW_ACT_SIGMOID = 2, ACCFLOW_ACT_TANH = 3 };

enum {
  ACCFLOW_EPI_STORE = 0,
  ACCFLOW_EPI_RES_RELU = 1,
  ACCFLOW_EPI_GRU_ZR = 2,
  ACCFLOW_EPI_GRU_Q = 3,
  ACCFLOW_EPI_ACCUM = 4,
  ACCFLOW_EPI_TAPGEMM = 5
};

enum {
  ACCFLOW_CONV_F32 = 0,
  ACCFLOW_CONV_BF16X3 = 2,
  ACCFLOW_CONV_BF16X6 = 3,
  ACCFLOW_CONV_F16X3 = 4
// ... 5 lines not shown
  long long bs;
  int C, Hs, Ws;
  int step, oy, ox;
  int KH, KW, padH, padW;
  int reserved;
} accflow_conv_src;
#define ACCFLOW_CONV_MAX_SRC 4

typedef struct accflow_conv_desc {
  const float* in0;  const float* in1;
  long long in0_bs, in1_bs;
  int C0, C1;
  int B, H, W;
  int OH, OW;
  int KH, KW, stride, padH, padW;
  int Cout;
  const float* wpack;
  const int*   ktab;
  int Kpad, CoutPad;
  const float* bias;
  float* out;  long long out_bs;
  int act, epi;
  const float* e0; long long e0_bs;
  const float* e1; long long e1_bs;
  float* out2; long long out2_bs;
  const float* offset; long long offset_bs;
  const float* dmask;  long long dmask_bs;
  const void* wsplit;
  int mode;
  const void* wpatch;
  long long wsplit_bs;
  float* kws; long long kws_elems;
  const void* wpatch16; int* guard;
  const float* wscale16;
  const void* wsplit16;
  float* stats; int stat_slots;
  const float* pre; long long pre_bs;
  const float* in_norm;
  float acc_scale;
  int in_fmt;
  void* out16; long long out16_bs;
  int cb;
  long long out_cbs, e0_cbs, out16_cbs;
  int nsrc;
  accflow_conv_src src[ACCFLOW_CONV_MAX_SRC];
  int e0_fmt;
  const void* tg_w16; const float* tg_scale;
  float* tg_out; long long tg_out_bs, tg_out_ps;
  int tg_rows, tg_coutpad;
  int split_c0;
  int p32;
} accflow_conv_desc;

long long accflow_s16_item_words(int C, int H, int W);
int accflow_to_s16_f32(const float* src, long long src_bs, void* dst16, long long dst16_bs, int* guard, int B, int C,
                       int HW, void* stream);

int accflow_conv_kpad(int Cin, int KH, int KW);
int accflow_conv_coutpad(int Cout);

int accflow_conv_pack_f32(const float* w, const float* scale, int Cout, int Cin, int KH, int KW,
                          int C0, int tap_major, float* wpack, int* ktab, void* stream);

int accflow_conv_pack_bf16s(const float* w, const float* scale, int Cout, int Cin, int KH, int KW,
                            void* wsplit, void* stream);

long long accflow_conv_patch_elems(int Cout, int Cin, int KH, int KW);
int accflow_conv_pack_patch(const float* w, const float* scale, int Cout, int Cin, int KH, int KW,
                            void* wpatch, void* stream);
int accflow_conv_pack_patch16(const float* w, const float* scale, int Cout, int Cin, int KH, int KW,
                              void* wpatch16, float* wscale16, void* stream);

int accflow_conv_pack_split16(const float* w, const float* scale, int Cout, int Cin, int KH, int KW,
                              void* wsplit16, float* wscale16, void* stream);

int accflow_conv_pack_all_f32(const float* w, const float* scale, int Cout, int Cin, int KH, int KW, int C0, int tap_major,
                              int transpose_flip, float* wpack, int* ktab, void* wsplit, void* wpatch, void* wpatch16,
                              float* wscale16, void* wsplit16, void* stream);

long long accflow_conv_multi_pack_elems(int Cout, int nsrc, const int* C, const int* KH, const int* KW);
int accflow_conv_pack_multi16(const float* const* w, const float* scale, int Cout, int nsrc, const int* C, const int* KH,
                              const int* KW, void* wpatch16, float* wscale16, void* stream);

int accflow_conv2d_f32(const accflow_conv_desc* desc, void* stream);
int accflow_conv_stat_slots(const accflow_conv_desc* desc);
int accflow_conv_in_norm_supported(const accflow_conv_desc* desc);
int accflow_conv_plan_query(const accflow_conv_desc* desc, int* out, int n);
int accflow_conv_gru16_supported(void);

int accflow_corr_volume_f32(const float* fmap1, const float* fmap2, float* lvl0, float* lvl1,
                            float* lvl2, float* lvl3, int B, int C, int H8, int W8, void* stream);

long long accflow_corr_volume_ws_bytes(int C, int H8, int W8);
int accflow_corr_volume_split_f32(const float* fmap1, const float* fmap2, float* lvl0, float* lvl1,
                                  float* lvl2, float* lvl3, void* ws, int mode, int B, int C, int H8,
                                  int W8, void* stream);

int accflow_corr_lookup_f32(const float* lvl0, const float* lvl1, const float* lvl2,
                            const float* lvl3, const float* coords, float* out, long long out_bs,
                            int B, int H8, int W8, void* stream);

int accflow_corr_disp_supported(int H8, int W8);
long long accflow_corr_disp_level_elems(int H8, int W8, int level);
int accflow_corr_volume_disp_f32(const float* fmap1, const float* fmap2, float* lvl0, float* lvl1,
                                 float* lvl2, float* lvl3, void* ws, int mode, int* guard, int B, int C,
                                 int H8, int W8, void* stream);
long long accflow_corr_pack_bytes(int C, int H8, int W8);
int accflow_corr_pack_f32(const float* fmaps, void* packs, int mode, int* guard, int F, int C, int H8, int W8,
                          void* stream);
int accflow_corr_volume_disp_packed_f32(const void* packs, int F, const int* idx1, const int* idx2, float* lvl0,
                                        float* lvl1, float* lvl2, float* lvl3, int mode, int* guard, int B, int C, int H8,
                                        int W8, void* stream);
int accflow_corr_disp_pool_f32(const float* lvl0, float* lvl1, float* lvl2, float* lvl3, int B, int H8,
                               int W8, void* stream);
int accflow_corr_lookup_disp_f32(const float* lvl0, const float* lvl1, const float* lvl2,
                                 const float* lvl3, const float* coords, float* out, long long out_bs,
                                 int B, int H8, int W8, void* stream);

int accflow_corr_lookup_disp_s16(const float* lvl0, const float* lvl1, const float* lvl2, const float* lvl3,
                                 const float* coords, void* out16, long long out16_bs, int* guard, int B, int H8,
                                 int W8, void* stream);

long long accflow_corr_alt_pyramid_elems(int C, int H8, int W8);
int accflow_corr_alt_pyramid_f32(const float* fmaps, float* pyr, int F, int C, int H8, int W8, void* stream);
int accflow_corr_lookup_alt_f32(const float* pyr, int F, const int* idx, const float* coords, float* out, long long out_bs,
                                int B, int C, int H8, int W8, void* stream);
int accflow_corr_lookup_alt_s16(const float* pyr, int F, const int* idx, const float* coords, void* out16, long long out16_bs,
                                int* guard, int B, int C, int H8, int W8, void* stream);

int accflow_corr_lookup_convc1_kpad(void);
int accflow_corr_lookup_convc1_s16(const float* lvl0, const float* lvl1, const float* lvl2, const float* lvl3,
                                   const float* coords, const void* wpatch16, const float* wscale16, const float* bias,
                                   void* out16, long long out16_bs, float* out, long long out_bs, int act, int* guard,
                                   int B, int H8, int W8, int Cout, void* stream);

int accflow_convex_upsample_f32(const float* flow, long long flow_bs, const float* mask,
                                long long mask_bs, float* out, int B, int H8, int W8, void* stream);

int accflow_backwarp_f32(const float* img, long long img_bs, const float* flow, long long flow_bs,
                         float* out, long long out_bs, int B, int C, int H, int W, void* stream);

int accflow_compose_flow_f32(const float* step, long long step_bs, const float* acc, long long acc_bs,
                             float* out, long long out_bs, int B, int H, int W, void* stream);

int accflow_get_occ_f32(const float* flow, long long flow_bs, const float* i1, long long i1_bs,
                        const float* i2, long long i2_bs, float* out, long long out_bs, int B, int C,
                        int H, int W, int binary, void* stream);

int accflow_get_occ_s16(const float* flow, long long flow_bs, const float* i1, long long i1_bs, const float* i2,
                        long long i2_bs, void* out16, long long out16_bs, int* guard, int B, int C, int H, int W, int binary,
                        void* stream);

int accflow_downflow8_f32(const float* flow, float* out, int B, int C, int H, int W, void* stream);
int accflow_forward_interpolate_f32(const float* flow, float* out, int B, int H8, int W8, void* stream);

int accflow_instance_norm_f32(const float* x, const float* res, float* out, int B, int C, int HW,
                              float eps, int mode, void* stream);

int accflow_instance_stats_finalize_f32(const float* stats, int slots, float* meanrstd, int B, int C, float eps,
                                        void* stream);
int accflow_instance_norm_apply_f32(const float* x, const float* stats, int slots, float* meanrstd, const float* res,
                                    float* out, int B, int C, int HW, float eps, int mode, void* stream);
int accflow_instance_stats_finalize_sub_f32(const float* stats, int slots, int Ctot, int c0, float* meanrstd, int B, int C,
                                            float eps, void* stream);

int accflow_instance_norm_apply_s16_f32(const float* x, const float* stats, int slots, float* meanrstd, const float* res,
                                        float* out, void* out16, long long out16_bs, int* guard, int B, int C, int HW,
                                        float eps, int mode, void* stream);
int accflow_instance_norm_apply_s16res_f32(const float* x, const float* stats, int slots, float* meanrstd, const void* res16,
                                           long long res16_bs, float* out, void* out16, long long out16_bs, int* guard, int B,
                                           int C, int HW, float eps, void* stream);

int accflow_instance_norm_apply_s16proj_f32(const float* x, const float* stats, int slots, const float* res, long long res_bs,
                                            const float* res_stats, int res_slots, int res_ctot, int res_c0, float* meanrstd,
                                            void* out16, long long out16_bs, int* guard, int B, int C, int HW, float eps,
                                            void* stream);

int accflow_split_tanh_relu_f32(const float* cnet, float* net, long long net_bs, float* inp,
                                long long inp_bs, int B, int hd, int cd, int HW, void* stream);
int accflow_split_tanh_relu_idx_f32(const float* cnet, int n_items, const int* idx, float* net, long long net_bs, float* inp,
                                    long long inp_bs, int B, int hd, int cd, int HW, void* stream);

int accflow_coords_grid_f32(float* coords, const float* flow_init, int B, int H8, int W8,
                            void* stream);

int accflow_flow_from_coords_f32(const float* coords1, float* dst0, long long dst0_bs, float* dst1,
                                 long long dst1_bs, float* stack16, int is_flow, int B, int H8, int W8, void* stream);
int accflow_flow_from_coords_s16(const float* coords1, float* dst0, long long dst0_bs, float* dst1, long long dst1_bs,
                                 void* stack16, long long stack16_bs, void* motion16, long long motion16_bs, int motion_ch,
                                 int* guard, int is_flow, int B, int H8, int W8, void* stream);

int accflow_blend_f32(const float* f1, const float* f2, const float* m, float* out, int B, int C,
                      int HW, void* stream);

int accflow_blend_s16(const float* f1, const float* f2, const float* m, void* out16, long long out16_bs, int* guard, int B, int C,
                      int HW, void* stream);

int accflow_deform_columns_f32(const float* x, long long x_bs, const float* offset, long long offset_bs,
                               const float* dmask, long long dmask_bs, float* cols, int B, int C, int H, int W,
                               int KH, int KW, int padH, int padW, void* stream);

int accflow_deform_columns_s16(const float* x, long long x_bs, const float* offset, long long offset_bs, const float* dmask,
                               long long dmask_bs, int mask_is_logit, void* cols16, long long cols16_bs, int* guard, int B, int C,
                               int H, int W, int KH, int KW, int padH, int padW, void* stream);

int accflow_tap_sum_f32(const float* z, const float* bias, const float* e0, long long e0_bs, float* out,
                        long long out_bs, int B, int Cout, int H, int W, int KH, int KW, int padH, int padW,
                        int act, int epi, void* stream);
int accflow_tap_sum_parts_f32(const float* z, int nparts, long long part_stride, long long z_bs, const float* bias,
                              const float* e0, long long e0_bs, float* out, long long out_bs, int B, int Cout, int H, int W,
                              int KH, int KW, int padH, int padW, int act, int epi, void* stream);

int accflow_activation_f32(float* x, long long x_bs, int B, int C, int HW, int act, void* stream);

int accflow_copy_f32(const float* src, long long src_bs, float* dst, long long dst_bs, int B, int C,
                     int HW, void* stream);

int accflow_gma_attention_f32(const float* qk, float* attn, int B, int D, int P, float scale,
                              void* stream);
int accflow_gma_aggregate_f32(const float* attn, const float* v, const float* fmap,
                              const float* gamma, float* out, long long out_bs, int B, int D, int P,
                              void* stream);

long long accflow_gma_attention_ws_bytes(int D, int H, int W);
long long accflow_gma_attention_s16_ws_bytes(int D, int H, int W);
int accflow_gma_attention_s16(const float* qk, void* attn16, void* ws, int* guard, int B, int D, int H, int W, float scale,
                              void* stream);
long long accflow_gma_aggregate_s16_ws_bytes(int n, int D, int P);
int accflow_gma_aggregate_s16(const void* attn16, const float* v, const float* fmap, long long fmap_bs, const float* gamma,
                              float* out, long long out_bs, void* out16, long long out16_bs, void* ws, int* guard, int n, int D,
                              int H, int W, void* stream);
long long accflow_gma_attention_alt_ws_bytes(int D, int H, int W);
int accflow_gma_attention_alt(const float* qk, void* kpack, void* qpack, float* stats, void* ws, int* guard, int B, int D, int H,
                              int W, float scale, void* stream);
long long accflow_gma_aggregate_alt_ws_bytes(int n, int D, int P);
int accflow_gma_aggregate_alt(const void* kpack, const void* qpack, const float* stats, const float* v, const float* fmap,
                              long long fmap_bs, const float* gamma, float* out, long long out_bs, void* out16, long long out16_bs,
                              void* ws, int* guard, int n, int D, int H, int W, void* stream);
int accflow_gma_attention_t_f32(const float* qk, float* attnT, void* ws, int mode, int B, int D, int H, int W,
                                float scale, void* stream);
long long accflow_gma_aggregate_ws_bytes(int B, int D, int P);
int accflow_gma_aggregate_t_f32(const float* attnT, const float* v, const float* fmap, const float* gamma,
                                float* out, long long out_bs, void* ws, int mode, int* guard, int B, int D, int H, int W,
                                void* stream);

int accflow_act_backward_f32(const float* dy, long long dy_bs, const float* y, long long y_bs, float* dx, long long dx_bs, int B,
                             long long CHW, int act, void* stream);
int accflow_add_f32(float* dst, long long dst_bs, const float* src, long long src_bs, int B, long long CHW, void* stream);
int accflow_l1_grad_f32(const float* pred, const float* gt, float* dpred, long long n, float scale, void* stream);
int accflow_dilate_f32(const float* src, long long src_bs, float* dst, int B, int C, int OH, int OW, int Hd, int Wd, int stride,
                       void* stream);
int accflow_blend_backward_f32(const float* dy, const float* f1, const float* f2, const float* m, float* df1, float* df2,
                               float* dm, int B, int C, int HW, void* stream);
int accflow_convex_upsample_backward_f32(const float* dup, const float* flow, const float* mask, float* dflow, float* dmask,
                                         int B, int H8, int W8, void* stream);
int accflow_conv_wgrad_f32(const float* x, long long x_bs, const float* dy, long long dy_bs, float* dw, float* db, int B, int Cin,
                           int Cout, int H, int W, int KH, int KW, int stride, int padH, int padW, void* stream);
int accflow_deform_conv_backward_f32(const float* x, long long x_bs, const float* offset, long long offset_bs, const float* dmask,
                                     long long dmask_bs, const float* dcols, float* dx, long long dx_bs, float* doffset,
                                     float* ddmask, int B, int C, int H, int W, int KH, int KW, int padH, int padW, void* stream);

int accflow_abi_version(void);
int accflow_conv_desc_bytes(void);
int accflow_conv_src_bytes(void);

#ifdef __cplusplus
}
#endif
#endif
```

Measured before the change: 530.1 frame-pairs/s.

## Fuse mask head, convex upsample and 8x downsample for small-only estimates

```diff
diff --git a/accflow_amd/_lib.py b/accflow_amd/_lib.py
--- a/accflow_amd/_lib.py
+++ b/accflow_amd/_lib.py
@@ -118,10 +118,13 @@
     "accflow_compose_flow_f32": [c_f, c_ll, c_f, c_ll, c_f, c_ll, c_i, c_i, c_i, c_f],
     "accflow_get_occ_f32": [c_f, c_ll, c_f, c_ll, c_f, c_ll, c_f, c_ll, c_i, c_i, c_i, c_i, c_i, c_f],
     "accflow_downflow8_f32": [c_f, c_f, c_i, c_i, c_i, c_i, c_f],
+    "accflow_mask_convex_down8": [c_f, c_ll, c_i, c_f, c_f, c_f, c_ll, c_f, c_ll, c_i, c_i, c_i, c_i, c_f],
     "accflow_forward_interpolate_f32": [c_f, c_f, c_i, c_i, c_i, c_f],
     "accflow_instance_norm_f32": [c_f, c_f, c_f, c_i, c_i, c_i, ctypes.c_float, c_i, c_f],
     "accflow_split_tanh_relu_f32": [c_f, c_f, c_ll, c_f, c_ll, c_i, c_i, c_i, c_i, c_f],
     "accflow_split_tanh_relu_idx_f32": [c_f, c_i, ctypes.POINTER(c_i), c_f, c_ll, c_f, c_ll, c_i, c_i, c_i, c_i, c_f],
+    "accflow_split_tanh_relu_idx_s16": [c_f, c_i, ctypes.POINTER(c_i), c_f, c_ll, c_f, c_ll, c_f, c_ll, c_f, c_ll, c_f, c_i, c_i, c_i,
+                                        c_i, c_f],
     "accflow_coords_grid_f32": [c_f, c_f, c_i, c_i, c_i, c_f],
     "accflow_flow_from_coords_f32": [c_f, c_f, c_ll, c_f, c_ll, c_f, c_i, c_i, c_i, c_i, c_f],
     "accflow_deform_columns_f32": [c_f, c_ll, c_f, c_ll, c_f, c_ll, c_f, c_i, c_i, c_i, c_i, c_i, c_i, c_i, c_i, c_f],
diff --git a/accflow_amd/csrc/misc.hip b/accflow_amd/csrc/misc.hip
--- a/accflow_amd/csrc/misc.hip
+++ b/accflow_amd/csrc/misc.hip
@@ -288,6 +288,40 @@
   if (bad && guard) atomicOr(guard, 1);
 }
 
+__global__ __launch_bounds__(256) void split_tanh_relu_idx_s16_kernel(const float* __restrict__ cnet, split_idx idx,
+                                                                      mu32x4* __restrict__ h16, long long h16_bs,
+                                                                      mu32x4* __restrict__ inp16, long long inp16_bs,
+                                                                      float* __restrict__ net, long long net_bs,
+                                                                      float* __restrict__ inp, long long inp_bs, int* guard, int B,
+                                                                      int hd, int cd, int HW) {
+  const int OH = hd >> 3, O = (hd + cd) >> 3;
+  const long long g = (long long)blockIdx.x * 256 + threadIdx.x;
+  if (g >= (long long)B * O * HW) return;
+  const int pix = (int)(g % HW), o = (int)((g / HW) % O), b = (int)(g / ((long long)HW * O));
+  const float* src = cnet + ((long long)idx.v[b] * (hd + cd) + o * 8) * HW + pix;
+  const bool is_net = o < OH;
+  const int ol = is_net ? o : o - OH;
+  float v[8];
+#pragma unroll
+  for (int j = 0; j < 8; ++j) {
+    const float x = src[(long long)j * HW];
+    v[j] = is_net ? tanhf(x) : fmaxf(x, 0.0f);
+  }
+  float* f32 = is_net ? net : inp;
+  if (f32) {
+    f32 += b * (is_net ? net_bs : inp_bs) + (long long)(ol * 8) * HW + pix;
+#pragma unroll
+    for (int j = 0; j < 8; ++j) f32[(long long)j * HW] = v[j];
+  }
+  mu32x4 hi, lo;
+  bool bad = false;
+  s16_split8(v, hi, lo, bad);
+  mu32x4* d = is_net ? h16 + (b * h16_bs) / 4 : inp16 + (b * inp16_bs) / 4;
+  d[(long long)(ol * 2 + 0) * HW + pix] = hi;
+  d[(long long)(ol * 2 + 1) * HW + pix] = lo;
+  if (bad && guard) atomicOr(guard, 1);
+}
+
 __global__ __launch_bounds__(256) void instance_norm_apply_s16_kernel(const float* __restrict__ x, const float* __restrict__ meanrstd,
                                                                       const float* __restrict__ res, float* __restrict__ out,
                                                                       mu32x4* __restrict__ dst, long long dst_bs, int* guard,
@@ -542,6 +576,27 @@
     const long long n = (long long)nb * (hd + cd) * HW;
     hipLaunchKernelGGL(split_tanh_relu_idx_kernel, dim3(cdiv(n, 256)), dim3(256), 0, as_stream(stream), cnet, a,
                        net + b0 * net_bs, net_bs, inp + b0 * inp_bs, inp_bs, nb, hd, cd, HW);
+  }
+  ACCFLOW_RETURN_LAUNCH_STATUS();
+}
+
+extern "C" int accflow_split_tanh_relu_idx_s16(const float* cnet, int n_items, const int* idx, void* h16, long long h16_bs,
+                                               void* inp16, long long inp16_bs, float* net, long long net_bs, float* inp,
+                                               long long inp_bs, int* guard, int B, int hd, int cd, int HW, void* stream) {
+  if (!cnet || !h16 || !inp16 || n_items <= 0 || B <= 0 || hd <= 0 || cd <= 0 || (hd & 7) || (cd & 7) || HW <= 0) return 1;
+  for (int b = 0; b < B; ++b) {
+    const int s = idx ? idx[b] : b;
+    if (s < 0 || s >= n_items) return 1;
+  }
+  for (int b0 = 0; b0 < B; b0 += 64) {
+    const int nb = B - b0 < 64 ? B - b0 : 64;
+    split_idx a;
+    for (int k = 0; k < 64; ++k) a.v[k] = k < nb ? (idx ? idx[b0 + k] : b0 + k) : 0;
+    const long long n = (long long)nb * ((hd + cd) / 8) * HW;
+    hipLaunchKernelGGL(split_tanh_relu_idx_s16_kernel, dim3(cdiv(n, 256)), dim3(256), 0, as_stream(stream), cnet, a,
+                       reinterpret_cast<mu32x4*>(h16) + (b0 * h16_bs) / 4, h16_bs, reinterpret_cast<mu32x4*>(inp16) + (b0 * inp16_bs) / 4,
+                       inp16_bs, net ? net + b0 * net_bs : nullptr, net_bs, inp ? inp + b0 * inp_bs : nullptr, inp_bs, guard, nb,
+                       hd, cd, HW);
   }
   ACCFLOW_RETURN_LAUNCH_STATUS();
 }
diff --git a/accflow_amd/csrc/sampling.hip b/accflow_amd/csrc/sampling.hip
--- a/accflow_amd/csrc/sampling.hip
+++ b/accflow_amd/csrc/sampling.hip
@@ -1,6 +1,38 @@
 #include "common.h"
 
 namespace {
+
+__device__ __forceinline__ void convex_combine(float (&m)[9], const float (&f0)[9], const float (&f1)[9], float& u0, float& u1) {
+  float mx = -INFINITY;
+#pragma unroll
+  for (int k = 0; k < 9; ++k) mx = fmaxf(mx, m[k]);
+  float s = 0.0f;
+#pragma unroll
+  for (int k = 0; k < 9; ++k) {
+    m[k] = expf(m[k] - mx);
+    s += m[k];
+  }
+  u0 = 0.0f;
+  u1 = 0.0f;
+#pragma unroll
+  for (int k = 0; k < 9; ++k) {
+    const float wk = m[k] / s;
+    u0 += wk * f0[k];
+    u1 += wk * f1[k];
+  }
+}
+
+__device__ __forceinline__ void flow_taps8(const float* __restrict__ fl, int h, int w, int H8, int W8, float (&f0)[9],
+                                           float (&f1)[9]) {
+  const int P = H8 * W8;
+#pragma unroll
+  for (int k = 0; k < 9; ++k) {
+    const int yy = h + k / 3 - 1, xx = w + k % 3 - 1;
+    const bool ok = (unsigned)yy < (unsigned)H8 && (unsigned)xx < (unsigned)W8;
+    f0[k] = ok ? 8.0f * fl[yy * W8 + xx] : 0.0f;
+    f1[k] = ok ? 8.0f * fl[P + yy * W8 + xx] : 0.0f;
+  }
+}
 
 __global__ __launch_bounds__(256) void convex_upsample_kernel(const float* __restrict__ flow, long long flow_bs,
                                                               const float* __restrict__ mask, long long mask_bs,
@@ -12,13 +44,7 @@
   const int h = pix / W8, w = pix - h * W8;
   const float* fl = flow + b * flow_bs;
   float f0[9], f1[9];
-#pragma unroll
-  for (int k = 0; k < 9; ++k) {
-    const int yy = h + k / 3 - 1, xx = w + k % 3 - 1;
-    const bool ok = (unsigned)yy < (unsigned)H8 && (unsigned)xx < (unsigned)W8;
-    f0[k] = ok ? 8.0f * fl[yy * W8 + xx] : 0.0f;
-    f1[k] = ok ? 8.0f * fl[P + yy * W8 + xx] : 0.0f;
-  }
+  flow_taps8(fl, h, w, H8, W8, f0, f1);
   const float* mk = mask + b * mask_bs + pix;
   const int W = 8 * W8;
   float* o0 = out + ((long long)(b * 2 + 0) * (8 * H8) + 8 * h) * W + 8 * w;
@@ -29,27 +55,9 @@
 #pragma unroll
     for (int bb = 0; bb < 8; ++bb) {
       float m[9];
-      float mx = -INFINITY;
-#pragma unroll
-      for (int k = 0; k < 9; ++k) {
-        m[k] = mk[(long long)(k * 64 + a * 8 + bb) * P];
-        mx = fmaxf(mx, m[k]);
-      }
-      float s = 0.0f;
-#pragma unroll
-      for (int k = 0; k < 9; ++k) {
-        m[k] = expf(m[k] - mx);
-        s += m[k];
-      }
-      float u0 = 0.0f, u1 = 0.0f;
-#pragma unroll
-      for (int k = 0; k < 9; ++k) {
-        const float wk = m[k] / s;
-        u0 += wk * f0[k];
-        u1 += wk * f1[k];
-      }
-      r0[bb] = u0;
-      r1[bb] = u1;
+#pragma unroll
+      for (int k = 0; k < 9; ++k) m[k] = mk[(long long)(k * 64 + a * 8 + bb) * P];
+      convex_combine(m, f0, f1, r0[bb], r1[bb]);
     }
     float4* q0 = reinterpret_cast<float4*>(o0 + (long long)a * W);
     float4* q1 = reinterpret_cast<float4*>(o1 + (long long)a * W);
@@ -191,6 +199,24 @@
   if (bad && guard) atomicOr(guard, 1);
 }
 
+struct Down8Axis {
+  int i0, ip;
+  float l;
+};
+__device__ __forceinline__ Down8Axis down8_axis(float scale, int i, int N) {
+  const float s = scale * (float)i;
+  Down8Axis a;
+  a.i0 = (int)s;
+  a.ip = a.i0 < N - 1 ? 1 : 0;
+  a.l = fmaf(scale, (float)i, -(float)a.i0);
+  return a;
+}
+__device__ __forceinline__ float down8_blend(float ly, float lx, float p00, float p01, float p10, float p11) {
+  const float hy = 1.0f - ly, hx = 1.0f - lx;
+  const float v = hy * (hx * p00 + lx * p01) + ly * (hx * p10 + lx * p11);
+  return v / 8.0f;
+}
+
 __global__ __launch_bounds__(256) void downflow8_kernel(const float* __restrict__ flow, float* __restrict__ out,
                                                         int BC, int H, int W) {
   const int H8 = H / 8, W8 = W / 8, P = H8 * W8;
@@ -200,14 +226,132 @@
   const int y = pix / W8, x = pix - y * W8;
   const float sy_scale = H8 > 1 ? (float)(H - 1) / (float)(H8 - 1) : 0.0f;
   const float sx_scale = W8 > 1 ? (float)(W - 1) / (float)(W8 - 1) : 0.0f;
-  const float sy = sy_scale * (float)y, sx = sx_scale * (float)x;
-  const int y0 = (int)sy, x0 = (int)sx;
-  const int yp = y0 < H - 1 ? 1 : 0, xp = x0 < W - 1 ? 1 : 0;
-  const float ly = sy - (float)y0, lx = sx - (float)x0;
-  const float hy = 1.0f - ly, hx = 1.0f - lx;
-  const float* p = flow + (long long)bc * H * W + (long long)y0 * W + x0;
-  const float v = hy * (hx * p[0] + lx * p[xp]) + ly * (hx * p[(long long)yp * W] + lx * p[(long long)yp * W + xp]);
-  out[g] = v / 8.0f;
+  const Down8Axis ay = down8_axis(sy_scale, y, H), ax = down8_axis(sx_scale, x, W);
+  const int xp = ax.ip;
+  const long long yo = (long long)ay.ip * W;
+  const float* p = flow + (long long)bc * H * W + (long long)ay.i0 * W + ax.i0;
+  out[g] = down8_blend(ay.l, ax.l, p[0], p[xp], p[yo], p[yo + xp]);
+}
+
+constexpr int MCD_THREADS = 128, MCD_CCH = 64, MCD_ROWS = 144, MCD_LD = 145, MCD_MAX_SIZE = 2048;
+
+struct McdOctet { mu32x4 a, b; };
+
+template <bool S16IN>
+__device__ __forceinline__ McdOctet mcd_load(const void* __restrict__ hidden, int o, int P, int pix) {
+  McdOctet r;
+  if constexpr (S16IN) {
+    const mu32x4* h = reinterpret_cast<const mu32x4*>(hidden);
+    r.a = h[(long long)(o * 2 + 0) * P + pix];
+    r.b = h[(long long)(o * 2 + 1) * P + pix];
+  } else {
+    const float* h = reinterpret_cast<const float*>(hidden) + (long long)(o * 8) * P + pix;
+#pragma unroll
+    for (int j = 0; j < 4; ++j) {
+      r.a[j] = __float_as_uint(h[(long long)j * P]);
+      r.b[j] = __float_as_uint(h[(long long)(j + 4) * P]);
+    }
+  }
+  return r;
+}
+
+template <bool S16IN>
+__device__ __forceinline__ void mcd_decode(const McdOctet& r, float (&v)[8]) {
+  if constexpr (S16IN) {
+    typedef _Float16 h2 __attribute__((ext_vector_type(2)));
+#pragma unroll
+    for (int j = 0; j < 4; ++j) {
+      const h2 hi = __builtin_bit_cast(h2, (unsigned)r.a[j]), lo = __builtin_bit_cast(h2, (unsigned)r.b[j]);
+      v[2 * j] = ((float)hi[0] + (float)lo[0]) * (1.0f / (float)(1 << ACCFLOW_F16_ASHIFT));
+      v[2 * j + 1] = ((float)hi[1] + (float)lo[1]) * (1.0f / (float)(1 << ACCFLOW_F16_ASHIFT));
+    }
+  } else {
+#pragma unroll
+    for (int j = 0; j < 4; ++j) {
+      v[j] = __uint_as_float(r.a[j]);
+      v[j + 4] = __uint_as_float(r.b[j]);
+    }
+  }
+}
+
+template <bool S16IN>
+__global__ __launch_bounds__(MCD_THREADS) void mask_convex_down8_kernel(const void* __restrict__ hidden, long long hidden_bs,
+                                                                        const float* __restrict__ weight,
+                                                                        const float* __restrict__ bias,
+                                                                        const float* __restrict__ flow, long long flow_bs,
+                                                                        float* __restrict__ out, long long out_bs, int C, int H8,
+                                                                        int W8) {
+  __shared__ float lw[MCD_CCH * MCD_LD];
+  const int P = H8 * W8;
+  const int y = blockIdx.y, b = blockIdx.z;
+  const int x = blockIdx.x * MCD_THREADS + threadIdx.x;
+  const bool live = x < W8;
+  const int xc = live ? x : W8 - 1;
+  const int pix = y * W8 + xc;
+  const int H = 8 * H8, W = 8 * W8;
+  const float sy_scale = H8 > 1 ? (float)(H - 1) / (float)(H8 - 1) : 0.0f;
+  const float sx_scale = W8 > 1 ? (float)(W - 1) / (float)(W8 - 1) : 0.0f;
+  const Down8Axis ay = down8_axis(sy_scale, y, H), ax = down8_axis(sx_scale, xc, W);
+  const int a0 = min(max(ay.i0 - 8 * y, 0), 7), a1 = min(a0 + ay.ip, 7);
+  const int b0 = min(max(ax.i0 - 8 * xc, 0), 7), b1 = min(b0 + ax.ip, 7);
+  const float* lrow[2] = {lw + b0 * 9, lw + b1 * 9};
+  const void* hb = reinterpret_cast<const char*>(hidden) + b * hidden_bs * 4;
+  double acc[2][2][9];
+#pragma unroll
+  for (int ai = 0; ai < 2; ++ai)
+#pragma unroll
+    for (int bi = 0; bi < 2; ++bi)
+#pragma unroll
+      for (int k = 0; k < 9; ++k) acc[ai][bi][k] = 0.0;
+  const int O = C >> 3;
+  McdOctet nxt = mcd_load<S16IN>(hb, 0, P, pix);
+  for (int o = 0; o < O; ++o) {
+    if ((o & (MCD_CCH / 8 - 1)) == 0) {
+      const int c0 = o * 8;
+      __syncthreads();
+      for (int i = threadIdx.x; i < MCD_ROWS * MCD_CCH; i += MCD_THREADS) {
+        const int r = i / MCD_CCH, cc = i - r * MCD_CCH;
+        const int ai = r / 72, rem = r - ai * 72, bb = rem / 9, k = rem - bb * 9;
+        const int ch = k * 64 + (ai ? a1 : a0) * 8 + bb;
+        lw[cc * MCD_LD + r] = weight[(long long)ch * C + c0 + cc];
+      }
+      __syncthreads();
+    }
+    const McdOctet cur = nxt;
+    if (o + 1 < O) nxt = mcd_load<S16IN>(hb, o + 1, P, pix);
+    float v[8];
+    mcd_decode<S16IN>(cur, v);
+    const int cl = (o & (MCD_CCH / 8 - 1)) * 8;
+#pragma unroll
+    for (int ai = 0; ai < 2; ++ai)
+#pragma unroll
+      for (int bi = 0; bi < 2; ++bi)
+#pragma unroll
+        for (int k = 0; k < 9; ++k) {
+          float p = 0.0f;
+#pragma unroll
+          for (int j = 0; j < 8; ++j) p = fmaf(lrow[bi][(cl + j) * MCD_LD + ai * 72 + k], v[j], p);
+          acc[ai][bi][k] += (double)p;
+        }
+  }
+  float f0[9], f1[9];
+  flow_taps8(flow + b * flow_bs, y, xc, H8, W8, f0, f1);
+  float u0[2][2], u1[2][2];
+#pragma unroll
+  for (int ai = 0; ai < 2; ++ai)
+#pragma unroll
+    for (int bi = 0; bi < 2; ++bi) {
+      const int sub = (ai ? a1 : a0) * 8 + (bi ? b1 : b0);
+      float m[9];
+#pragma unroll
+      for (int k = 0; k < 9; ++k) m[k] = (float)(acc[ai][bi][k] + (double)bias[k * 64 + sub]);
+      convex_combine(m, f0, f1, u0[ai][bi], u1[ai][bi]);
+    }
+  if (live) {
+    float* ob = out + b * out_bs;
+    ob[pix] = down8_blend(ay.l, ax.l, u0[0][0], u0[0][1], u0[1][0], u0[1][1]);
+    ob[P + pix] = down8_blend(ay.l, ax.l, u1[0][0], u1[0][1], u1[1][0], u1[1][1]);
+  }
 }
 
 }
@@ -311,6 +455,21 @@
   else
     hipLaunchKernelGGL((get_occ_s16_kernel<false>), dim3(cdiv(np, 256), cdiv(C, 8)), dim3(256), 0, as_stream(stream), flow,
                        flow_bs, i1, i1_bs, i2, i2_bs, d, out16_bs, guard, B, C, H, W);
+  ACCFLOW_RETURN_LAUNCH_STATUS();
+}
+
+extern "C" int accflow_mask_convex_down8(const void* hidden, long long hidden_bs, int hidden_s16, const float* weight,
+                                         const float* bias, const float* flow, long long flow_bs, float* out, long long out_bs,
+                                         int B, int C, int H8, int W8, void* stream) {
+  if (!hidden || !weight || !bias || !flow || !out || B <= 0 || C <= 0 || (C % MCD_CCH) || H8 <= 0 || W8 <= 0) return 1;
+  if (B > 65535 || H8 > MCD_MAX_SIZE || W8 > MCD_MAX_SIZE) return 1;
+  const dim3 grid(cdiv(W8, MCD_THREADS), H8, B);
+  if (hidden_s16)
+    hipLaunchKernelGGL((mask_convex_down8_kernel<true>), grid, dim3(MCD_THREADS), 0, as_stream(stream), hidden, hidden_bs, weight,
+                       bias, flow, flow_bs, out, out_bs, C, H8, W8);
+  else
+    hipLaunchKernelGGL((mask_convex_down8_kernel<false>), grid, dim3(MCD_THREADS), 0, as_stream(stream), hidden, hidden_bs, weight,
+                       bias, flow, flow_bs, out, out_bs, C, H8, W8);
   ACCFLOW_RETURN_LAUNCH_STATUS();
 }
 
diff --git a/accflow_amd/networks/AccFlow_.py b/accflow_amd/networks/AccFlow_.py
--- a/accflow_amd/networks/AccFlow_.py
+++ b/accflow_amd/networks/AccFlow_.py
@@ -45,6 +45,7 @@
     if USE_CHAIN_HOIST == "auto":
         return not getattr(_CHAIN_TLS, "pipelined", False)
     return USE_CHAIN_HOIST == "1" or USE_CHAIN_HOIST is True
+ESTIMATE_SMALL_FUSED = True
 USE_CHAIN_DEFER_UP = os.environ.get("ACCFLOW_CHAIN_DEFER_UP", "1") == "1"
 _CTX_STREAMS = {}
 
@@ -357,6 +358,8 @@
     def estimate_small(self, images, pairs, flow_init=None, iters=None, features=None):
         iters = getattr(self, "ofe_iters", 12) if iters is None else iters
         if hasattr(self.ofe, "estimate_pairs"):
+            if ESTIMATE_SMALL_FUSED:
+                return self.ofe.estimate_pairs(images, pairs, iters=iters, flow_init=flow_init, features=features, small_only=True)
             flows = self.ofe.estimate_pairs(images, pairs, iters=iters, flow_init=flow_init, features=features)
         else:
             flows = self.ofe(torch.cat([images[i] for i, _ in pairs]), torch.cat([images[j] for _, j in pairs]),
diff --git a/accflow_amd/networks/_packs.py b/accflow_amd/networks/_packs.py
--- a/accflow_amd/networks/_packs.py
+++ b/accflow_amd/networks/_packs.py
@@ -94,6 +94,23 @@
         self._store[key] = [sig, pk, _mark_ready(conv.weight.device)]
         return pk
 
+    def plain(self, key, conv, const_scale=1.0):
+        sig = _sig([conv.weight, conv.bias]) + (const_scale,)
+        key = (key, str(conv.weight.device))
+        hit = self._store.get(key)
+        if hit is not None and hit[0] == sig:
+            _wait_ready(hit)
+            return hit[1]
+        with torch.no_grad():
+            co, ci, kh, kw = conv.weight.shape
+            if (kh, kw) != (1, 1):
+                raise ValueError("PackCache.plain: a 1x1 convolution")
+            w = (conv.weight.float().reshape(co, ci) * float(const_scale)).contiguous()
+            b = (conv.bias.float() * float(const_scale)).contiguous() if conv.bias is not None else torch.zeros(
+                co, dtype=torch.float32, device=w.device)
+        self._store[key] = [sig, (w, b), _mark_ready(conv.weight.device)]
+        return self._store[key][1]
+
     def multi(self, key, conv, bn=None, scale=None, scale_dep=None, splits=None, strided=False, in_ranges=None, with_bias=True):
         deps = [conv.weight, conv.bias, scale_dep if scale_dep is not None else (None if callable(scale) else scale)]
         if callable(scale) and scale_dep is None:
diff --git a/accflow_amd/networks/gma/gma.py b/accflow_amd/networks/gma/gma.py
--- a/accflow_amd/networks/gma/gma.py
+++ b/accflow_amd/networks/gma/gma.py
@@ -14,6 +14,7 @@
 
 class RAFTGMA(RAFT):
     KEEP_CONTEXT_RUNS = True
+    CONTEXT_INP_FP32 = True
 
     def __init__(self, args):
         nn.Module.__init__(self)
diff --git a/accflow_amd/networks/gma/update.py b/accflow_amd/networks/gma/update.py
--- a/accflow_amd/networks/gma/update.py
+++ b/accflow_amd/networks/gma/update.py
@@ -38,7 +38,7 @@
         self.aggregate(ws, attention)
         self.gru_step(ws)
         self.flow_delta(ws, coords1=coords1)
-        return self.up_mask(ws) if want_mask else None
+        return self._mask_out(ws, want_mask)
 
     @torch.no_grad()
     @ops.range_guarded
diff --git a/accflow_amd/networks/raft/raft.py b/accflow_amd/networks/raft/raft.py
--- a/accflow_amd/networks/raft/raft.py
+++ b/accflow_amd/networks/raft/raft.py
@@ -34,6 +34,7 @@
 
 class RAFT(nn.Module):
     KEEP_CONTEXT_RUNS = False
+    CONTEXT_INP_FP32 = False
 
     def __init__(self, args):
         super().__init__()
@@ -76,12 +77,16 @@
         self.update_block.prepack()
 
     def _prepare_context(self, ws, cnet_feat, ids=None):
-        if isinstance(cnet_feat, tuple):
+        indexed = isinstance(cnet_feat, tuple)
+        if ws.s16:
+            ws.inp16 = ops.S16.empty(ws.B, self.context_dim, ws.h, ws.w, ws.hx.device)
+            ops.split_tanh_relu_s16(cnet_feat[0] if indexed else cnet_feat, cnet_feat[1] if indexed else None, ws.h16, ws.inp16,
+                                    self.hidden_dim, self.context_dim, net=None if ws.net_in_h16 else ws.net,
+                                    inp=ws.inp if self.CONTEXT_INP_FP32 else None)
+        elif indexed:
             ops.split_tanh_relu_indexed(cnet_feat[0], cnet_feat[1], ws.net, ws.inp, self.hidden_dim, self.context_dim)
         else:
             ops.split_tanh_relu(cnet_feat, ws.net, ws.inp, self.hidden_dim, self.context_dim)
-        if ws.s16:
-            ops.to_s16(ws.net, ws.h16)
 
     def _lookup_and_flow(self, ws, corr_fn, coords1):
         if ws.s16 and corr_fn.supports_s16():
@@ -118,7 +123,8 @@
                     cuts[g] += 1
         return cuts
 
-    def _refine(self, fmap1, fmap2, cnet_feat, iters, flow_init, packed=None, ctx_ids=None, ready=None, return_low=False):
+    def _refine(self, fmap1, fmap2, cnet_feat, iters, flow_init, packed=None, ctx_ids=None, ready=None, return_low=False,
+                small_only=False):
         if iters < 1:
             raise ValueError("iters must be >= 1")
         indexed = isinstance(cnet_feat, tuple)
@@ -134,7 +140,7 @@
         bounds = list(zip(cuts[:-1], cuts[1:]))
         main = torch.cuda.current_stream()
         streams = [main] if n_groups == 1 else _side_streams(dev, n_groups)
-        out_all = torch.empty((B, 2, 8 * h, 8 * w), dtype=torch.float32, device=dev)
+        out_all = torch.empty((B, 2, h, w) if small_only else (B, 2, 8 * h, 8 * w), dtype=torch.float32, device=dev)
         low_all = torch.empty((B, 2, h, w), dtype=torch.float32, device=dev) if return_low else None
         forked = None
         if ctx_ready is not None:
@@ -167,16 +173,21 @@
                 coords1 = ops.coords_grid(b1 - b0, h, w, dev, flow_init=fi)
             state.append((st, corr_fn, ws, coords1))
         masks = [None] * n_groups
+        tail = "hidden" if small_only else True
         for itr in range(iters):
             for g, (st, corr_fn, ws, coords1) in enumerate(state):
                 with torch.cuda.stream(st):
-                    masks[g] = self._iteration(ws, corr_fn, coords1, last=(itr == iters - 1))
+                    masks[g] = self._iteration(ws, corr_fn, coords1, last=(itr == iters - 1) and tail)
         for g, (st, corr_fn, ws, coords1) in enumerate(state):
             with torch.cuda.stream(st):
                 if forked is not None and early:
                     st.wait_event(forked)
                 ops.flow_from_coords(coords1, dst0=ws.flow)
-                ops.convex_upsample(ws.flow, masks[g], out=out_all[bounds[g][0]:bounds[g][1]])
+                if small_only:
+                    mw, mb = self.update_block.mask_weights()
+                    ops.mask_convex_down8(masks[g], mw, mb, ws.flow, out=out_all[bounds[g][0]:bounds[g][1]])
+                else:
+                    ops.convex_upsample(ws.flow, masks[g], out=out_all[bounds[g][0]:bounds[g][1]])
                 if return_low:
                     low_all[bounds[g][0]:bounds[g][1]].copy_(ws.flow)
             if st != main:
@@ -239,7 +250,7 @@
         return feats
 
     @torch.no_grad()
-    def estimate_pairs(self, frames, pairs, iters=12, flow_init=None, features=None, return_low=False):
+    def estimate_pairs(self, frames, pairs, iters=12, flow_init=None, features=None, return_low=False, small_only=False):
         require_cuda(*frames)
         N = frames[0].shape[0]
         feats = self.encode_pairs(frames, pairs, features)
@@ -247,7 +258,7 @@
         home = feats.pop("refine_at_home", None)
         if ready is not None and home is not None and flow_init is None:
             ready = (ready, home[0], home[1])
-        return self._estimate_encoded(frames, pairs, feats, ready, iters, flow_init, return_low)
+        return self._estimate_encoded(frames, pairs, feats, ready, iters, flow_init, return_low, small_only)
 
     @torch.no_grad()
     def estimate_video(self, frames, iters=12, warm_start=True, pairs=None, features=None):
@@ -294,7 +305,7 @@
         self._prepack()
         return feats
 
-    def _estimate_encoded(self, frames, pairs, feats, ready, iters, flow_init, return_low=False):
+    def _estimate_encoded(self, frames, pairs, feats, ready, iters, flow_init, return_low=False, small_only=False):
         N = frames[0].shape[0]
         cb = feats.get("cnet_base")
         if cb is not None and all(i in cb[1] for i, _ in pairs):
@@ -317,7 +328,7 @@
             def refine_alt():
                 pyr = ops.corr_alt_pyramid(fb[0])
                 return self._refine(None, None, cfeat, iters, flow_init, packed=(pyr, idx1, idx2), ctx_ids=ctx_ids,
-                                    return_low=return_low)
+                                    return_low=return_low, small_only=small_only)
 
             return ops.with_range_guard(refine_alt, frames[0].device, name="%s.refine" % type(self).__name__)
         if self._packs_usable(feats, pairs):
@@ -333,12 +344,12 @@
                     cp, ev = ops.corr_pack(fb[0]), None
                     feats["corr_packs"] = cp
                 return self._refine(None, None, cfeat, iters, flow_init, packed=(cp, idx1, idx2), ctx_ids=ctx_ids, ready=ev,
-                                    return_low=return_low)
+                                    return_low=return_low, small_only=small_only)
 
             return ops.with_range_guard(refine_packed, frames[0].device, name="%s.refine" % type(self).__name__)
         fmap1 = torch.cat([feats["fmap"][i] for i, _ in pairs], dim=0)
         fmap2 = torch.cat([feats["fmap"][j] for _, j in pairs], dim=0)
-        return self._refine_guarded(fmap1, fmap2, cfeat, iters, flow_init, ctx_ids=ctx_ids, return_low=return_low)
+        return self._refine_guarded(fmap1, fmap2, cfeat, iters, flow_init, ctx_ids=ctx_ids, return_low=return_low, small_only=small_only)
 
 
 def default_args():
diff --git a/accflow_amd/networks/raft/update.py b/accflow_amd/networks/raft/update.py
--- a/accflow_amd/networks/raft/update.py
+++ b/accflow_amd/networks/raft/update.py
@@ -74,6 +74,7 @@
             self.head = buf(256)
         self.mask = None
         self.gru_pre = None
+        self.inp16 = None
         if self.s16:
             def s(c, zero=False):
                 return ops.S16.empty(B, c, h, w, device, zero=zero)
@@ -150,6 +151,7 @@
             self._gru_packs(s)
         pk.conv("fh1", f.conv1); pk.conv("fh2", f.conv2)
         pk.conv("m0", self.mask[0]); pk.conv("m2", self.mask[2], const_scale=0.25)
+        pk.plain("m2p", self.mask[2], const_scale=0.25)
 
     def motion_encoder(self, ws):
         pk, e = self._packs, self.encoder
@@ -191,7 +193,7 @@
     def gru_context(self, ws):
         B, h, w, hd = ws.B, ws.h, ws.w, ws.hidden
         ws.gru_pre = {}
-        inp = ops.to_s16(ws.inp) if ws.s16 else ws.inp
+        inp = (ws.inp16 if ws.inp16 is not None else ops.to_s16(ws.inp)) if ws.s16 else ws.inp
         p32 = ws.s16 and ws.net_in_h16
         for s in ("1", "2"):
             _, zrc, _, qc = self._gru_packs(s)
@@ -255,11 +257,27 @@
         ops.conv2d(pk.conv("m0", self.mask[0]), ws.net, out=ws.head, act=ops.ACT_RELU)
         return ops.conv2d(pk.conv("m2", self.mask[2], const_scale=0.25), ws.head, out=ws.mask)
 
+    def mask_hidden(self, ws):
+        pk = self._packs
+        if ws.s16:
+            ops.conv2d(pk.conv("m0", self.mask[0]), ws.h16, out16=ws.head16, act=ops.ACT_RELU, fp32_out=False)
+            return ws.head16
+        ops.conv2d(pk.conv("m0", self.mask[0]), ws.net, out=ws.head, act=ops.ACT_RELU)
+        return ws.head
+
+    def mask_weights(self):
+        return self._packs.plain("m2p", self.mask[2], const_scale=0.25)
+
+    def _mask_out(self, ws, want_mask):
+        if want_mask == "hidden":
+            return self.mask_hidden(ws)
+        return self.up_mask(ws) if want_mask else None
+
     def step(self, ws, coords1, want_mask):
         self.motion_encoder(ws)
         self.gru_step(ws)
         self.flow_delta(ws, coords1=coords1)
-        return self.up_mask(ws) if want_mask else None
+        return self._mask_out(ws, want_mask)
 
     @torch.no_grad()
     @ops.range_guarded
diff --git a/accflow_amd/ops.py b/accflow_amd/ops.py
--- a/accflow_amd/ops.py
+++ b/accflow_amd/ops.py
@@ -1385,6 +1385,29 @@
     return out
 
 
+def mask_convex_down8(hidden, weight, bias, flow, out=None):
+    lib = _lib.load()
+    fbs = _plane4(flow, "flow")
+    B, _, h, w = flow.shape
+    s16 = isinstance(hidden, S16)
+    hbs = hidden.bs if s16 else _plane4(hidden, "hidden")
+    C = hidden.shape[1]
+    if tuple(hidden.shape) != (B, C, h, w) or flow.shape[1] != 2:
+        raise RuntimeError("mask_convex_down8: hidden (B,C,h,w) and flow (B,2,h,w) must match")
+    weight, bias = _dense(weight, "weight"), _dense(bias, "bias")
+    if tuple(weight.shape) != (576, C) or tuple(bias.shape) != (576,):
+        raise RuntimeError("mask_convex_down8: weight must be (576, C) and bias (576,)")
+    if out is None:
+        out = torch.empty((B, 2, h, w), dtype=torch.float32, device=flow.device)
+    elif tuple(out.shape) != (B, 2, h, w):
+        raise RuntimeError("mask_convex_down8: out must be (B,2,h,w)")
+    obs = _plane4(out, "out")
+    hp = ctypes.c_void_p(hidden.ptr()) if s16 else _p(hidden)
+    _check(lib.accflow_mask_convex_down8(hp, hbs, int(s16), _p(weight), _p(bias), _p(flow), fbs, _p(out), obs, B, C, h, w,
+                                         _stream()), "accflow_mask_convex_down8")
+    return out
+
+
 def forward_interpolate(flow, out=None):
     lib = _lib.load()
     if not (isinstance(flow, torch.Tensor) and flow.is_cuda and flow.is_floating_point() and flow.dim() in (3, 4)
@@ -1496,6 +1519,26 @@
            "accflow_split_tanh_relu_idx_f32")
 
 
+def split_tanh_relu_s16(cnet_items, idx, h16, inp16, hd, cd, net=None, inp=None):
+    lib = _lib.load()
+    cnet_items = _dense(cnet_items, "cnet")
+    n, _, H, W = cnet_items.shape
+    B = h16.shape[0]
+    if idx is not None and len(idx) != B:
+        raise RuntimeError("split_tanh_relu_s16: one index per output item")
+    if tuple(h16.shape) != (B, hd, H, W) or tuple(inp16.shape) != (B, cd, H, W) or cnet_items.shape[1] != hd + cd:
+        raise RuntimeError("split_tanh_relu_s16: h16 (B,hd,H,W), inp16 (B,cd,H,W), cnet (n,hd+cd,H,W)")
+    for t, c, name in ((net, hd, "net"), (inp, cd, "inp")):
+        if t is not None and tuple(t.shape) != (B, c, H, W):
+            raise RuntimeError("split_tanh_relu_s16: %s must be (B,%d,H,W)" % (name, c))
+    nbs = _plane4(net, "net") if net is not None else 0
+    ibs = _plane4(inp, "inp") if inp is not None else 0
+    arr = (ctypes.c_int * B)(*idx) if idx is not None else None
+    _check(lib.accflow_split_tanh_relu_idx_s16(_p(cnet_items), n, arr, ctypes.c_void_p(h16.ptr()), h16.bs, ctypes.c_void_p(inp16.ptr()),
+                                               inp16.bs, _p(net), nbs, _p(inp), ibs, _p(_guard(cnet_items.device)), B, hd, cd, H * W,
+                                               _stream()), "accflow_split_tanh_relu_idx_s16")
+
+
 def coords_grid(B, H8, W8, device, flow_init=None):
     lib = _lib.load()
     out = torch.empty((B, 2, H8, W8), dtype=torch.float32, device=device)
diff --git a/include/accflow_hip.h b/include/accflow_hip.h
--- a/include/accflow_hip.h
+++ b/include/accflow_hip.h
@@ -181,6 +181,9 @@
                         void* stream);
 
 int accflow_downflow8_f32(const float* flow, float* out, int B, int C, int H, int W, void* stream);
+int accflow_mask_convex_down8(const void* hidden, long long hidden_bs, int hidden_s16, const float* weight, const float* bias,
+                              const float* flow, long long flow_bs, float* out, long long out_bs, int B, int C, int H8, int W8,
+                              void* stream);
 int accflow_forward_interpolate_f32(const float* flow, float* out, int B, int H8, int W8, void* stream);
 
 int accflow_instance_norm_f32(const float* x, const float* res, float* out, int B, int C, int HW,
@@ -209,6 +212,9 @@
                                 long long inp_bs, int B, int hd, int cd, int HW, void* stream);
 int accflow_split_tanh_relu_idx_f32(const float* cnet, int n_items, const int* idx, float* net, long long net_bs, float* inp,
                                     long long inp_bs, int B, int hd, int cd, int HW, void* stream);
+int accflow_split_tanh_relu_idx_s16(const float* cnet, int n_items, const int* idx, void* h16, long long h16_bs, void* inp16,
+                                    long long inp16_bs, float* net, long long net_bs, float* inp, long long inp_bs, int* guard,
+                                    int B, int hd, int cd, int HW, void* stream);
 
 int accflow_coords_grid_f32(float* coords, const float* flow_init, int B, int H8, int W8,
                             void* stream);
```

Result: no change. 533.3 frame-pairs/s, median of 6 (+0.6%).
